# hpcde/spmv-acc

Hardware: AMD Instinct MI355X
Metric: CSR SpMV GFLOP/s (fp64, int32 indices; achieved HBM GB/s in roofline) (higher is better)
Workload: dtype f64

## Files before the change

include/spmv_acc.h:

```cpp
#ifndef SPMV_ACC_C_ABI_H
#define SPMV_ACC_C_ABI_H

#ifdef __cplusplus
extern "C" {
#endif

enum spmv_acc_strategy {
  SPMV_ACC_DEFAULT = 0,
  SPMV_ACC_ADAPTIVE = 1,
  SPMV_ACC_THREAD_ROW = 2,
  SPMV_ACC_WF_ROW = 3,
  SPMV_ACC_BLOCK_ROW_ORDINARY = 4,
  SPMV_ACC_LIGHT = 5,
  SPMV_ACC_VECTOR_ROW = 6,
  SPMV_ACC_LINE_ENHANCE = 7,
  SPMV_ACC_LINE = 8,
  SPMV_ACC_FLAT = 9,
  SPMV_ACC_ADAPTIVE_PLUS = 10
};
int spmv_acc_set_strategy(const char *name);
int spmv_acc_set_strategy_id(int strategy);
int spmv_acc_get_strategy(void);
const char *spmv_acc_strategy_name(int strategy);
int spmv_acc_parse_strategy(const char *name);
// ... 29 lines not shown

int spmv_acc_adaptive_plus_analyze(int m, int min_nnz_per_block, int threads_per_block, int vec_size,
                                   const int *h_rowptr, int *h_break_points, int bp_cap,
                                   int *h_first_block_of_row);
int spmv_acc_adaptive_plus_analyze_device(int m, int min_nnz_per_block, int threads_per_block, int vec_size,
                                          const int *d_rowptr, int *d_break_points, int bp_cap,
                                          int *d_first_block_of_row);
int spmv_acc_adaptive_plus_vec(int m, int nnz);

int spmv_acc_adaptive_branch(int m, int rp_quarter, int rp_half, int rp_three_quarter, int rp_last);

int spmv_acc_partition_rows(int m, int parts, int mode, const int *h_rowptr, int *row_begin);

int spmv_acc_sharded_spmv(void *nccl_comm, int strategy, double alpha, double beta, int m_local, int m_pad, int n, int nnz_local,
                          const int *h_rowptr, const int *d_rowptr, const int *d_colindex, const double *d_value, const double *dx,
                          double *dy_local, double *dy_full);

typedef struct spmv_acc_shard *spmv_acc_shard_t;
int spmv_acc_shard_create(spmv_acc_shard_t *out, void *nccl_comm, int strategy, int m_local, int m_pad, int n, int nnz_local,
                          const int *d_rowptr, const int *d_colindex, const double *d_value, int pipeline);
int spmv_acc_shard_step(spmv_acc_shard_t shard, double alpha, double beta, const double *dx, const double *dy_in_local,
                        double *dy_full);
int spmv_acc_shard_prepare(spmv_acc_shard_t shard, double beta, const double *dx);
int spmv_acc_shard_pipeline(spmv_acc_shard_t shard);
int spmv_acc_shard_destroy(spmv_acc_shard_t shard);
int spmv_acc_rccl_comm_init_all(void **comms, int ndev, const int *devices);
int spmv_acc_rccl_comm_destroy(void *comm);

int spmv_acc_stage_csr(int m, int n, int nnz, const int *h_rowptr, const int *h_colindex, const double *h_value,
                       const double *h_x, const double *h_y, int **d_rowptr, int **d_colindex, double **d_value,
                       double **d_x, double **d_y);
int spmv_acc_free_device(void *p);

int spmv_acc_prepare(int strategy, int m, int n, int nnz, const int *h_rowptr, const int *d_rowptr, const int *d_colindex,
                     const double *d_value, const double *dx, float *ms_out);
int spmv_acc_prepare_beta(int strategy, double beta, int m, int n, int nnz, const int *h_rowptr, const int *d_rowptr,
                          const int *d_colindex, const double *d_value, const double *dx, float *ms_out);

void spmv_acc_set_tune_cache(const char *path);

int spmv_acc_refresh_values(const int *d_rowptr);

double spmv_acc_last_prepare_us(void);

void spmv_acc_release_plans(const int *d_rowptr);
int spmv_acc_cached_plans(void);
int spmv_acc_check_plans(void);
int spmv_acc_query_plan(const int *d_rowptr, int m, int *out);
int spmv_acc_query_plan_beta0(const int *d_rowptr, int m);
int spmv_acc_query_plan_slab_passes(const int *d_rowptr, int m);
int spmv_acc_query_plan_settled(const int *d_rowptr, int m);
int spmv_acc_query_plan_col16(const int *d_rowptr, int m);
int spmv_acc_query_plan_col_bits(const int *d_rowptr, int m);
enum spmv_acc_kernel {
  SPMV_ACC_KERNEL_ROWBLOCK = 0,
  SPMV_ACC_KERNEL_ROWBLOCK_PLUS = 1,
  SPMV_ACC_KERNEL_FLAT_TILE = 2,
  SPMV_ACC_KERNEL_SLAB_PASSES = 3,
  SPMV_ACC_KERNEL_VECTOR_TILE = 4, SPMV_ACC_KERNEL_VECTOR_ROW = 5, SPMV_ACC_KERNEL_WAVE_ROW = 6, SPMV_ACC_KERNEL_LIGHT = 7,
  SPMV_ACC_KERNEL_BLOCK_ROW = 8, SPMV_ACC_KERNEL_COL_SLABS = 9, SPMV_ACC_KERNEL_SCALE_ONLY = 10
};
int spmv_acc_query_plan_last_kernel(const int *d_rowptr, int m);

void spmv_acc_set_stream(void *hip_stream);
void *spmv_acc_get_stream(void);

int spmv_acc_last_error(void);
const char *spmv_acc_last_error_string(void);
void spmv_acc_clear_error(void);
enum spmv_acc_error {
  SPMV_ACC_OK = 0,
  SPMV_ACC_ERR_UNSUPPORTED_TRANS = 1,
  SPMV_ACC_ERR_BAD_ARGUMENT = 2,
  SPMV_ACC_ERR_HIP = 3,
  SPMV_ACC_ERR_TOO_LARGE = 4,
  SPMV_ACC_ERR_UNKNOWN_STRATEGY = 5,
  SPMV_ACC_ERR_NO_DEVICE = 6
};

int spmv_acc_time_spmv(int strategy, int iters, double alpha, double beta, int m, int n, int nnz,
                       const int *h_rowptr, const int *d_rowptr, const int *d_colindex, const double *d_value,
                       const double *dx, double *dy, const double *d_y0, float *ms_out);

int spmv_acc_time_spmv_events(int strategy, int iters, double alpha, double beta, int m, int n, int nnz,
                              const int *h_rowptr, const int *d_rowptr, const int *d_colindex, const double *d_value,
                              const double *dx, double *dy, const double *d_y0, float *ms_out, unsigned event_flags);

int spmv_acc_time_spmv_cold(int strategy, int iters, double alpha, double beta, int m, int n, int nnz,
                            const int *h_rowptr, const int *d_rowptr, const int *d_colindex, const double *d_value,
                            const double *dx, double *dy, const double *d_y0, void *d_flush, long long flush_bytes, float *ms_out);

int spmv_acc_time_spmv_total(int strategy, int iters, double alpha, double beta, int m, int n, int nnz,
                             const int *h_rowptr, const int *d_rowptr, const int *d_colindex, const double *d_value,
                             const double *dx, double *dy, float *total_ms_out);
int spmv_acc_time_spmv_kernels(int strategy, int iters, double alpha, double beta, int m, int n, int nnz,
                               const int *h_rowptr, const int *d_rowptr, const int *d_colindex, const double *d_value,
                               const double *dx, double *dy, const double *d_y0, float *event_ms_out, float *kernel_ms_out, int *launches_out);
int spmv_acc_time_spmv_region(int strategy, int iters, double alpha, double beta, int m, int n, int nnz,
                              const int *h_rowptr, const int *d_rowptr, const int *d_colindex, const double *d_value,
                              const double *dx, double *dy, float *total_ms_out);
double spmv_acc_copy_ceiling_gbs(void *d_dst, const void *d_src, long long bytes, int reps);

int spmv_acc_set_tunable(const char *name, int value);
int spmv_acc_get_tunable(const char *name);
void spmv_acc_reset_tunables(void);

// ... 8 lines not shown
```

spmv_acc_amd/__init__.py:

```python
from __future__ import annotations

import ctypes
import os
from typing import Optional, Sequence

_HERE = os.path.dirname(os.path.abspath(__file__))
LIB_PATH = os.path.join(_HERE, "lib", "libspmv_acc.so")

STRATEGIES = (
    "default", "adaptive", "thread_row", "wf_row", "block_row_ordinary", "light",
    "vector_row", "line_enhance", "line", "flat", "adaptive_plus",
)
HOT_STRATEGIES = ("default", "adaptive", "flat", "line_enhance", "line", "vector_row", "adaptive_plus")

_c_int_p = ctypes.POINTER(ctypes.c_int)
_c_double_p = ctypes.POINTER(ctypes.c_double)

C_ABI_SYMBOLS = (
    "sparse_spmv", "spmv_acc_csr_spmv", "spmv_acc_csr_spmv_strategy", "spmv_acc_set_strategy",
    "spmv_acc_set_strategy_id", "spmv_acc_get_strategy", "spmv_acc_strategy_name", "spmv_acc_parse_strategy",
    "spmv_acc_break_points", "spmv_acc_break_points_len", "spmv_acc_adaptive_plus_analyze",
    "spmv_acc_adaptive_plus_vec", "spmv_acc_adaptive_branch", "spmv_acc_partition_rows", "spmv_acc_stage_csr",
    "spmv_acc_free_device", "spmv_acc_release_plans", "spmv_acc_cached_plans", "spmv_acc_query_plan",
    "spmv_acc_set_stream", "spmv_acc_get_stream", "spmv_acc_last_error", "spmv_acc_last_error_string",
    "spmv_acc_clear_error", "spmv_acc_time_spmv", "spmv_acc_version", "spmv_acc_set_tunable",
    "spmv_acc_get_tunable", "spmv_acc_reset_tunables", "spmv_acc_time_spmv_total", "spmv_acc_copy_ceiling_gbs", "spmv_acc_adaptive_plus_analyze_device", "spmv_acc_prepare",
    "spmv_acc_last_prepare_us", "spmv_acc_sharded_spmv", "spmv_acc_shard_prepare", "spmv_acc_csr_spmv_chunks", "spmv_acc_query_plan_settled", "spmv_acc_query_plan_col16", "spmv_acc_query_plan_col_bits", "spmv_acc_time_spmv_cold", "spmv_acc_csr_spmv_oop", "spmv_acc_check_plans",
    "spmv_acc_query_plan_beta0", "spmv_acc_query_plan_slab_passes", "spmv_acc_shard_create", "spmv_acc_shard_step", "spmv_acc_shard_pipeline",
    "spmv_acc_shard_destroy", "spmv_acc_rccl_comm_init_all", "spmv_acc_rccl_comm_destroy", "spmv_acc_set_tune_cache",
    "spmv_acc_prepare_beta", "spmv_acc_time_spmv_events", "spmv_acc_refresh_values", "spmv_acc_time_spmv_region", "spmv_acc_query_plan_last_kernel", "spmv_acc_time_spmv_kernels",
    "spmv_acc_csr_spmm",
)

_lib = None


class SpmvAccError(RuntimeError):
    pass


def load_library(path: Optional[str] = None) -> ctypes.CDLL:
    global _lib
    if _lib is not None and path is None:
        return _lib
    p = path or LIB_PATH
    if not os.path.exists(p):
        raise SpmvAccError(
            f"{p} not found: the HIP extension is not built. Run `python -c 'import __graft_entry__ as g; g.build()'` "
            "or `make -C spmv_acc_amd/csrc`. There is no CPU fallback."
        )
    try:
        import torch
    except ImportError:
        pass
    lib = ctypes.CDLL(p)
    vp, ci, cd = ctypes.c_void_p, ctypes.c_int, ctypes.c_double
    lib.sparse_spmv.argtypes = [ci, cd, cd, ci, ci, vp, vp, vp, vp, vp]
    lib.sparse_spmv.restype = None
    lib.spmv_acc_csr_spmv.argtypes = [ci, cd, cd, ci, ci, ci, vp, vp, vp, vp, vp, vp]
    lib.spmv_acc_csr_spmv.restype = None
    lib.spmv_acc_csr_spmv_strategy.argtypes = [ci, ci, cd, cd, ci, ci, ci, vp, vp, vp, vp, vp, vp]
    lib.spmv_acc_csr_spmv_strategy.restype = None
    lib.spmv_acc_set_strategy.argtypes = [ctypes.c_char_p]
    lib.spmv_acc_set_strategy_id.argtypes = [ci]
    lib.spmv_acc_strategy_name.argtypes = [ci]
    lib.spmv_acc_strategy_name.restype = ctypes.c_char_p
    lib.spmv_acc_parse_strategy.argtypes = [ctypes.c_char_p]
    lib.spmv_acc_break_points.argtypes = [vp, ci, ci, ci, vp, ci]
    lib.spmv_acc_break_points_len.argtypes = [ci, ci]
    lib.spmv_acc_adaptive_plus_analyze.argtypes = [ci, ci, ci, ci, vp, vp, ci, vp]
    lib.spmv_acc_adaptive_plus_vec.argtypes = [ci, ci]
    lib.spmv_acc_adaptive_plus_analyze_device.argtypes = [ci, ci, ci, ci, vp, vp, ci, vp]
    lib.spmv_acc_adaptive_branch.argtypes = [ci, ci, ci, ci, ci]
    lib.spmv_acc_partition_rows.argtypes = [ci, ci, ci, vp, vp]
    lib.spmv_acc_stage_csr.argtypes = [ci, ci, ci, vp, vp, vp, vp, vp] + [ctypes.POINTER(vp)] * 5
    lib.spmv_acc_free_device.argtypes = [vp]
    lib.spmv_acc_prepare.argtypes = [ci, ci, ci, ci, vp, vp, vp, vp, vp, ctypes.POINTER(ctypes.c_float)]
    lib.spmv_acc_release_plans.argtypes = [vp]
    lib.spmv_acc_release_plans.restype = None
    lib.spmv_acc_query_plan.argtypes = [vp, ci, vp]
    lib.spmv_acc_set_stream.argtypes = [vp]
    lib.spmv_acc_set_stream.restype = None
    lib.spmv_acc_get_stream.restype = vp
    lib.spmv_acc_last_error_string.restype = ctypes.c_char_p
    lib.spmv_acc_clear_error.restype = None
    lib.spmv_acc_time_spmv.argtypes = [ci, ci, cd, cd, ci, ci, ci, vp, vp, vp, vp, vp, vp, vp, vp]
    lib.spmv_acc_time_spmv_events.argtypes = [ci, ci, cd, cd, ci, ci, ci, vp, vp, vp, vp, vp, vp, vp, vp, ctypes.c_uint]
    lib.spmv_acc_time_spmv_cold.argtypes = [ci, ci, cd, cd, ci, ci, ci, vp, vp, vp, vp, vp, vp, vp, vp, ctypes.c_longlong, vp]
    lib.spmv_acc_version.restype = ctypes.c_char_p
    lib.spmv_acc_set_tunable.argtypes = [ctypes.c_char_p, ci]
    lib.spmv_acc_get_tunable.argtypes = [ctypes.c_char_p]
    lib.spmv_acc_reset_tunables.restype = None
    lib.spmv_acc_time_spmv_total.argtypes = [ci, ci, cd, cd, ci, ci, ci, vp, vp, vp, vp, vp, vp, vp]
    lib.spmv_acc_time_spmv_kernels.argtypes = [ci, ci, cd, cd, ci, ci, ci, vp, vp, vp, vp, vp, vp, vp, vp, vp, vp]
    lib.spmv_acc_time_spmv_region.argtypes = [ci, ci, cd, cd, ci, ci, ci, vp, vp, vp, vp, vp, vp, vp]
    lib.spmv_acc_copy_ceiling_gbs.argtypes = [vp, vp, ctypes.c_longlong, ci]
    lib.spmv_acc_copy_ceiling_gbs.restype = cd
    lib.spmv_acc_last_prepare_us.restype = cd
    lib.spmv_acc_sharded_spmv.argtypes = [vp, ci, cd, cd, ci, ci, ci, ci, vp, vp, vp, vp, vp, vp, vp]
    lib.spmv_acc_csr_spmv_oop.argtypes = [ci, ci, cd, cd, ci, ci, ci, vp, vp, vp, vp, vp, vp, vp]
    lib.spmv_acc_csr_spmv_oop.restype = None
    lib.spmv_acc_query_plan_beta0.argtypes = [vp, ci]
    lib.spmv_acc_query_plan_slab_passes.argtypes = [vp, ci]
    lib.spmv_acc_query_plan_settled.argtypes = [vp, ci]
    lib.spmv_acc_query_plan_col16.argtypes = [vp, ci]
    lib.spmv_acc_query_plan_col_bits.argtypes = [vp, ci]
    lib.spmv_acc_query_plan_last_kernel.argtypes = [vp, ci]
    lib.spmv_acc_shard_create.argtypes = [ctypes.POINTER(vp), vp, ci, ci, ci, ci, ci, vp, vp, vp, ci]
    lib.spmv_acc_shard_step.argtypes = [vp, cd, cd, vp, vp, vp]
    lib.spmv_acc_shard_pipeline.argtypes = [vp]
    lib.spmv_acc_shard_destroy.argtypes = [vp]
    lib.spmv_acc_rccl_comm_init_all.argtypes = [ctypes.POINTER(vp), ci, vp]
    lib.spmv_acc_rccl_comm_destroy.argtypes = [vp]
    lib.spmv_acc_set_tune_cache.argtypes = [ctypes.c_char_p]
    lib.spmv_acc_set_tune_cache.restype = None
    lib.spmv_acc_refresh_values.argtypes = [vp]
    lib.spmv_acc_prepare_beta.argtypes = [ci, cd, ci, ci, ci, vp, vp, vp, vp, vp, ctypes.POINTER(ctypes.c_float)]
    lib.spmv_acc_shard_prepare.argtypes = [vp, cd, vp]
    lib.spmv_acc_csr_spmv_chunks.argtypes = [ci, cd, cd, ci, ci, vp, vp, vp, vp, vp, vp, vp, vp, vp, vp]
    ll = ctypes.c_longlong
    lib.spmv_acc_csr_spmm.argtypes = [ci, ci, cd, cd, ci, ci, ci, vp, vp, vp, vp, vp, ll, vp, ll]
    lib.spmv_acc_csr_spmm.restype = ci
    if path is None:
        _lib = lib
    return lib


def strategy_id(name_or_id) -> int:
    if isinstance(name_or_id, int):
        return name_or_id
    s = load_library().spmv_acc_parse_strategy(str(name_or_id).encode())
    if s < 0:
        raise SpmvAccError(f"unknown KERNEL_STRATEGY {name_or_id!r}")
    return s


def _check(lib) -> None:
    code = lib.spmv_acc_last_error()
    if code not in (0, 1):
        msg = lib.spmv_acc_last_error_string().decode()
        lib.spmv_acc_clear_error()
        raise SpmvAccError(f"spmv_acc error {code}: {msg}")


def _ptr(t) -> int:
    if t is None:
        return 0
    if isinstance(t, int):
        return t
    if hasattr(t, "data_ptr"):
        return t.data_ptr()
    return t.ctypes.data


def _require_cuda(*tensors) -> None:
    for t in tensors:
        if t is not None and hasattr(t, "is_cuda") and not t.is_cuda:
            raise SpmvAccError("device pointers required: tensor is not on the GPU (no CPU fallback)")

# ... 241 lines not shown
    args = (strategy_id(strategy), iters, alpha, beta, m, n, nnz, None, _ptr(rowptr), _ptr(colindex), _ptr(value), _ptr(x), _ptr(y),
            ctypes.addressof(out))
    fn = lib.spmv_acc_time_spmv_region

    def run() -> float:
        rc = fn(*args)
        if rc != 0:
            raise SpmvAccError(f"time_spmv_region failed ({rc}): {lib.spmv_acc_last_error_string().decode()}")
        return float(out.value)

    return run


def copy_ceiling_gbs(dst, src, reps: int = 5) -> float:
    lib = load_library()
    _require_cuda(dst, src)
    nbytes = (src.numel() * src.element_size()) // 16 * 16
    return float(lib.spmv_acc_copy_ceiling_gbs(_ptr(dst), _ptr(src), nbytes, reps))


def release_plans(rowptr=None) -> None:
    load_library().spmv_acc_release_plans(_ptr(rowptr))


def set_tune_cache(path: Optional[str]) -> None:
    load_library().spmv_acc_set_tune_cache(path.encode() if path else None)


def refresh_values(rowptr) -> int:
    return int(load_library().spmv_acc_refresh_values(_ptr(rowptr)))


def check_plans() -> int:
    return int(load_library().spmv_acc_check_plans())


KERNEL_NAMES = {0: "rowblock", 1: "rowblock_plus", 2: "flat_tile", 3: "slab_passes", 4: "vector_tile", 5: "vector_row", 6: "wave_row", 7: "light",
                8: "block_row", 9: "col_slabs", 10: "scale_only"}


def query_plan(rowptr, m: int):
    import numpy as np

    out = np.zeros(9, dtype=np.int32)
    found = load_library().spmv_acc_query_plan(_ptr(rowptr), m, _ptr(out))
    if not found:
        return None
    keys = ("nnz", "adaptive_branch", "vec", "flat_tiles", "plus_blocks", "aligned16", "stream_policy", "flat_fixup", "adaptive_family")
    info = dict(zip(keys, (int(v) for v in out)))
    info["slab_passes"] = max(0, int(load_library().spmv_acc_query_plan_slab_passes(_ptr(rowptr), m)))
    info["settled"] = int(load_library().spmv_acc_query_plan_settled(_ptr(rowptr), m)) == 1
    info["col16"] = int(load_library().spmv_acc_query_plan_col16(_ptr(rowptr), m))
    info["col_bits"] = int(load_library().spmv_acc_query_plan_col_bits(_ptr(rowptr), m))
    info["last_kernel"] = KERNEL_NAMES.get(int(load_library().spmv_acc_query_plan_last_kernel(_ptr(rowptr), m)), "none")
    return info


def set_strategy(name: str) -> None:
    lib = load_library()
    if lib.spmv_acc_set_strategy(name.encode()) != 0:
        lib.spmv_acc_clear_error()
        raise SpmvAccError(f"unknown KERNEL_STRATEGY {name!r}")


def get_strategy() -> str:
    lib = load_library()
    return lib.spmv_acc_strategy_name(lib.spmv_acc_get_strategy()).decode()
```

spmv_acc_amd/csrc/c_api.cpp:

```cpp
#include <hip/hip_runtime.h>

#include <dlfcn.h>

#include <algorithm>
#include <cstdlib>
#include <cstring>
#include <mutex>
#include <vector>

#include "../../include/spmv_acc.h"
#include "engine.hpp"

#include <string>
#include <cstdint>

using namespace spmv_acc;

namespace {
struct PinTable {
  std::mutex mu;
  struct Range { uintptr_t lo, hi; int refs; };
  std::vector<Range> ranges;
  static constexpr uintptr_t kPage = 4096;
  bool pin(void *p, size_t bytes) {
// ... 306 lines not shown
  ok = ok && stage_one(st, h_value, static_cast<size_t>(nnz), d_value);
  ok = ok && stage_one(st, h_x, static_cast<size_t>(n), d_x);
  ok = ok && stage_one(st, h_y, static_cast<size_t>(m), d_y);
  ok = ok && hipStreamSynchronize(st.copy) == hipSuccess;
  if (!ok) {
    const hipError_t e = hipGetLastError();
    set_error(kErrHip, std::string("spmv_acc_stage_csr: ") + hipGetErrorString(e));
    return kErrHip;
  }
  return kOk;
}

int spmv_acc_free_device(void *p) {
  if (!p) return kOk;
  return hipFree(p) == hipSuccess ? kOk : kErrHip;
}

void spmv_acc_release_plans(const int *d_rowptr) { release_plans(d_rowptr); }
int spmv_acc_cached_plans(void) { return cached_plan_count(); }
int spmv_acc_check_plans(void) { return check_plans(); }
int spmv_acc_query_plan(const int *d_rowptr, int m, int *out) {
  PlanInfo info;
  if (!out || !query_plan(d_rowptr, m, &info)) return 0;
  out[0] = info.nnz;
  out[1] = info.adaptive_branch;
  out[2] = info.vec;
  out[3] = info.flat_tiles;
  out[4] = info.plus_blocks;
  out[5] = info.aligned16;
  out[6] = info.stream_policy;
  out[7] = info.flat_fixup;
  out[8] = info.adaptive_family;
  return 1;
}
int spmv_acc_query_plan_beta0(const int *d_rowptr, int m) {
  PlanInfo info;
  return query_plan(d_rowptr, m, &info) ? info.adaptive_family_beta0 : -2;
}
int spmv_acc_query_plan_slab_passes(const int *d_rowptr, int m) {
  PlanInfo info;
  return query_plan(d_rowptr, m, &info) ? info.slab_passes : -2;
}
int spmv_acc_query_plan_last_kernel(const int *d_rowptr, int m) {
  PlanInfo info;
  return query_plan(d_rowptr, m, &info) ? info.last_kernel : -2;
}
int spmv_acc_query_plan_col16(const int *d_rowptr, int m) {
  PlanInfo info;
  return query_plan(d_rowptr, m, &info) ? info.col16 : -2;
}
int spmv_acc_query_plan_col_bits(const int *d_rowptr, int m) {
  PlanInfo info;
  return query_plan(d_rowptr, m, &info) ? info.col_bits : -2;
}
int spmv_acc_query_plan_settled(const int *d_rowptr, int m) {
  PlanInfo info;
  return query_plan(d_rowptr, m, &info) ? info.settled : -2;
}

void spmv_acc_set_stream(void *hip_stream) { set_stream(static_cast<hipStream_t>(hip_stream)); }
void *spmv_acc_get_stream(void) { return static_cast<void *>(get_stream()); }

int spmv_acc_set_tunable(const char *name, int value) { return name ? set_tunable(name, value) : -1; }
int spmv_acc_get_tunable(const char *name) { return name ? get_tunable(name) : -1; }
void spmv_acc_reset_tunables(void) { reset_tunables(); }

double spmv_acc_last_prepare_us(void) { return last_prepare_us(); }

int spmv_acc_last_error(void) { return last_error(); }
const char *spmv_acc_last_error_string(void) { return last_error_string(); }
void spmv_acc_clear_error(void) { clear_error(); }

void spmv_acc_set_tune_cache(const char *path) { set_tune_cache(path); }
int spmv_acc_refresh_values(const int *d_rowptr) { return refresh_values(d_rowptr); }

int spmv_acc_prepare(int strategy, int m, int n, int nnz, const int *h_rowptr, const int *d_rowptr, const int *d_colindex,
                     const double *d_value, const double *dx, float *ms_out) {
  return spmv_acc_prepare_beta(strategy, 1.0, m, n, nnz, h_rowptr, d_rowptr, d_colindex, d_value, dx, ms_out);
}

int spmv_acc_prepare_beta(int strategy, double beta, int m, int n, int nnz, const int *h_rowptr, const int *d_rowptr,
                          const int *d_colindex, const double *d_value, const double *dx, float *ms_out) {
  if (m <= 0) return kOk;
  hipStream_t st = get_stream();
  double *scratch = nullptr;
  if (hipMalloc(reinterpret_cast<void **>(&scratch), sizeof(double) * static_cast<size_t>(m)) != hipSuccess) {
    set_error(kErrHip, "spmv_acc_prepare: hipMalloc failed");
    return kErrHip;
  }
  hipEvent_t e0 = nullptr, e1 = nullptr;
  const bool timed = ms_out && hipEventCreate(&e0) == hipSuccess && hipEventCreate(&e1) == hipSuccess;
  clear_error();
  if (timed) (void)hipEventRecord(e0, st);
  (void)hipMemsetAsync(scratch, 0, sizeof(double) * static_cast<size_t>(m), st);
  {
    UnboundedTuningScope unbounded;
    for (int round = 0; round < 6; ++round) {
      run_spmv(strategy, 0, 1.0, beta != 0.0 ? 1.0 : 0.0, m, n, nnz, h_rowptr, d_rowptr, d_colindex, d_value, dx, scratch);
      if (last_error() != kOk || last_prepare_us() <= 0.0) break;
    }
  }
  if (timed) (void)hipEventRecord(e1, st);
  int rc = hipStreamSynchronize(st) == hipSuccess ? kOk : kErrHip;
  if (timed && rc == kOk && hipEventElapsedTime(ms_out, e0, e1) != hipSuccess) rc = kErrHip;
  if (e0) (void)hipEventDestroy(e0);
  if (e1) (void)hipEventDestroy(e1);
// ... 256 lines not shown
```

spmv_acc_amd/csrc/dispatch.cpp:

```cpp
#include "engine_internal.hpp"

namespace spmv_acc {
using namespace detail;

namespace detail {

constexpr int kFlatMaxTileRows = 16384;

thread_local int t_strict_name = -1;

bool run_flat(hipStream_t st, Plan &p, double alpha, double beta, const double *x, double *y) {
  if (!ensure_flat(p, st)) return false;
  const bool strict = t_strict_name == kFlat;
  if (p.flat.max_tile_rows > kFlatMaxTileRows && tun(kT_rowblock_guard) && !strict) {
    return run_rowblock(st, p, nullptr, alpha, beta, x, y, false, 0);
  }
  p.A.cold = nullptr;
  p.flat.col16 = nullptr;
  if (!autotune_policy(p, kFamFlat, st, [&](int pol, double *ys) { launch_flat_with(st, p, pol, 1.0, trial_beta(), x, ys); })) return false;
  if (!autotune_flat_mode(p, st, x)) return false;
  if (!autotune_flat_geometry(p, st, x)) return false;
  if (!autotune_hint(p, kFamFlat, st, [&](double *ys) { launch_flat_with(st, p, policy_for(p, kFamFlat), 1.0, trial_beta(), x, ys); })) return false;
  const Col16 *c16 = nullptr;
  if (p.flat.stride == kThreads * kNnzPerThread && !flat_segment_sum() &&
      !autotune_col16(p, kFamFlat, st, [&](const Col16 *c, double *ys) {
        p.flat.col16 = c;
        launch_flat_with(st, p, policy_for(p, kFamFlat), 1.0, trial_beta(), x, ys);
      }, &c16))
    return false;
  p.flat.col16 = c16;
  const int rb_mode = tun(kT_flat_rowblock);
  const bool tile_pinned = tun(kT_flat_finish) >= 0 || tun(kT_flat_npt) >= 0 || tun(kT_flat_early) >= 0;
  if (rb_mode != 0 && (rb_mode > 0 || !tile_pinned) && !flat_segment_sum() && tun(kT_col16) <= 0 &&
      !t_coarse_tuning && !strict) {
    if (rb_mode > 0) {
      int vec = 1, rpb = kThreads;
      pick_rowblock_shape(p.A.m, p.A.count(), rowblock_target_for(p), &vec, &rpb);
      if (t_capturing ? (p.rowblock_ok == 1 && p.rowblock_rpb == rpb) : (probe_rowblock(p, rpb, st) && p.rowblock_ok == 1))
        return run_rowblock(st, p, nullptr, alpha, beta, x, y, false, 0);
    } else if (p.flat_rowblock_choice < 0 && !t_capturing && !by_rule()) {
      int vec = 1, rpb = kThreads;
      pick_rowblock_shape(p.A.m, p.A.count(), rowblock_target_for(p), &vec, &rpb);
      if (!probe_rowblock(p, rpb, st)) return false;
      p.flat_rowblock_choice = 0;
      if (p.rowblock_ok == 1) {
        TimingPhase ph(st, p.A.m);
        float ms2[2] = {0.f, 0.f};
        bool ok = ph.ok && run_rowblock(st, p, nullptr, 1.0, trial_beta(), x, ph.y, false);
        ok = ok && ph.in_turns(2, [&](int c) {
          if (c == 0) launch_flat_with(st, p, policy_for(p, kFamFlat), 1.0, trial_beta(), x, ph.y);
          else (void)run_rowblock(st, p, nullptr, 1.0, trial_beta(), x, ph.y, false);
        }, ranking_rounds(), ms2);
        if (!ok) return false;
        const float ms_flat = ms2[0], ms_rb = ms2[1];
        p.flat_rowblock_choice = ms_rb < 0.985f * ms_flat ? 1 : 0;
        tune_log("m %d nnz %d flat on balanced rows: tile kernel %.2f us, row blocks %.2f us -> %s", p.A.m, p.A.nnz, ms_flat * 1e3f, ms_rb * 1e3f,
                 p.flat_rowblock_choice ? "row blocks" : "tile kernel");
      }
    }
    if (rb_mode < 0 && p.flat_rowblock_choice == 1) return run_rowblock(st, p, nullptr, alpha, beta, x, y, false, 0);
  }
  launch_flat_with(st, p, policy_for(p, kFamFlat), alpha, beta, x, y);
  p.last_kernel = kKernelFlatTile;
  p.last_c16 = c16 && p.flat.stride == kThreads * kNnzPerThread && p.A.cold == nullptr ? c16->rec_ints : 0;
  p.last_col_bits = p.last_c16 > 0 ? c16->bits : 0;
  return true;
}

bool validate_plan(Plan &p, hipStream_t st) {
  if (p.invalid < 0) {
    if (!plan_work_allowed("validating the matrix")) return false;
    ++t_plan_work;
    int *d_flags = nullptr;
    int h = -1;
    if (!hip_ok(hipMalloc(reinterpret_cast<void **>(&d_flags), sizeof(int)), "hipMalloc validate")) return false;
    if (hip_ok(hipMemsetAsync(d_flags, 0, sizeof(int), st), "memset validate")) {
      launch_validate_csr(st, p.A, d_flags);
      if (!hip_ok(hipMemcpyAsync(&h, d_flags, sizeof(int), hipMemcpyDeviceToHost, st), "read validate") ||
          !hip_ok(hipStreamSynchronize(st), "sync validate"))
        h = -1;
    }
    (void)hipFree(d_flags);
    if (h < 0) return false;
    p.invalid = h;
  }
  if (p.invalid != 0) {
    std::string what = "matrix failed validation:";
    if (p.invalid & 1) what += " rowptr decreases or is negative;";
    if (p.invalid & 2) what += " rowptr[m] != nnz;";
    if (p.invalid & 4) what += " column index outside [0, n);";
    set_error(kErrBadArgument, what);
    return false;
  }
  return true;
}

bool launch_full_guard(Plan &p, hipStream_t st) {
  if (!p.A.guard || !p.A.stale) return true;
  if (!p.have_rp_digest) {
    if (!plan_work_allowed("the full row-pointer digest (guard_full)")) return false;
    ++t_plan_work;
    const size_t words = static_cast<size_t>(Plan::kDigestSlots) * kDigestMaxParts + 1;
    if (!p.d_digest_acc && !hip_ok(hipMalloc(reinterpret_cast<void **>(&p.d_digest_acc), sizeof(unsigned long long) * words), "hipMalloc digest"))
      return false;
    unsigned long long *out = p.d_digest_acc + words - 1;
    launch_rowptr_digest(st, p.A.rp, p.A.m, p.d_digest_acc);
    launch_rowptr_verdict(st, p.d_digest_acc, p.A.m, 0, nullptr, out);
    unsigned long long h = 0;
    if (!hip_ok(hipMemcpyAsync(&h, out, sizeof(h), hipMemcpyDeviceToHost, st), "read digest") || !hip_ok(hipStreamSynchronize(st), "sync digest"))
      return false;
    p.rp_digest = h;
    p.have_rp_digest = true;
  }
  unsigned long long *part = p.d_digest_acc + static_cast<size_t>(p.digest_turn++ % Plan::kDigestSlots) * kDigestMaxParts;
  launch_rowptr_digest(st, p.A.rp, p.A.m, part);
  launch_rowptr_verdict(st, part, p.A.m, p.rp_digest, p.A.stale, nullptr);
  return true;
}
// ... 96 lines not shown
      }))
    return false;
  if (tun(kT_rowblock_target) <= 0 && p.rb_target == 0 && p.stream_policy[kFamRowblock][t_beta_class] >= 0 && !t_capturing && !t_coarse_tuning &&
      !t_no_policy_timing && !by_rule()) {
    int v2[2], r2[2];
    const int cand[2] = {kRowblockTargetRule, kRowblockTargetAlt};
    for (int c = 0; c < 2; ++c) shape_for(cand[c], &v2[c], &r2[c]);
    if (v2[0] == v2[1] && r2[0] == r2[1]) {
      p.rb_target = cand[0];
    } else {
      TimingPhase ph(st, p.A.m);
      bool ok = ph.ok;
      bool skip[2] = {false, false};
      float ms[2] = {1e30f, 1e30f};
      const int pol = policy_for(p, kFamRowblock);
      for (int c = 0; ok && c < 2; ++c) {
        vec = v2[c];
        rpb = r2[c];
        if (tun(kT_rowblock_guard)) {
          ok = probe_rowblock(p, rpb, st);
          skip[c] = ok && p.rowblock_ok == 0;
        }
      }
      for (int round = 0; ok && round < ranking_rounds(); ++round) {
        for (int c = 0; ok && c < 2; ++c) {
          if (skip[c]) continue;
          vec = v2[c];
          rpb = r2[c];
          ok = setup();
          float t = 0.f;
          ok = ok && ph.time([&] {
            const int zz = next_reverse(p) ? 64 : 0;
            launch_rowblock_stream(st, p.A, vec, rpb, base_flags | (pol << 4) | zz, 1.0, trial_beta(), x, ph.y, dg, cache_ends);
          }, &t);
          if (ok && t < ms[c]) ms[c] = t;
        }
      }
      if (!ok) return false;
      p.rb_target = (!skip[1] && (skip[0] || ms[1] < 0.985f * ms[0])) ? cand[1] : cand[0];
      tune_log("m %d nnz %d row blocks: %d products per block %.2f us, %d products %.2f us -> %d", p.A.m, p.A.nnz, cand[0], ms[0] * 1e3f, cand[1], ms[1] * 1e3f,
               p.rb_target);
    }
    shape_for(rowblock_target_for(p), &vec, &rpb);
    if (tun(kT_rowblock_guard) && !probe_rowblock(p, rpb, st)) return false;
    if (!setup()) return false;
  }
  if (!autotune_hint(p, kFamRowblock, st, [&](double *ys) {
        const int zz = next_reverse(p) ? 64 : 0;
        launch_rowblock_stream(st, p.A, vec, rpb, base_flags | (policy_for(p, kFamRowblock) << 4) | zz, 1.0, trial_beta(), x, ys, dg, cache_ends);
      }))
    return false;
  const Col16 *c16 = nullptr;
  if (!autotune_col16(p, kFamRowblock, st, [&](const Col16 *c, double *ys) {
        const int zz = next_reverse(p) ? 64 : 0;
        launch_rowblock_stream(st, p.A, vec, rpb, base_flags | (policy_for(p, kFamRowblock) << 4) | zz, 1.0, trial_beta(), x, ys, dg, cache_ends, c);
      }, &c16))
    return false;
  const int zz = next_reverse(p) ? 64 : 0;
  launch_rowblock_stream(st, p.A, vec, rpb, base_flags | (policy_for(p, kFamRowblock) << 4) | zz, alpha, beta, x, y, dg, cache_ends, c16);
  p.last_kernel = kKernelRowblock;
  p.last_c16 = c16 && p.A.cold == nullptr ? c16->rec_ints : 0;
  p.last_col_bits = p.last_c16 > 0 ? c16->bits : 0;
  return true;
}

bool run_plus_prepare(Plan &p, const int *h_rowptr, hipStream_t st, const double *x) {
  auto launch = [&](int pol, double *ys) {
    launch_plus(st, p.A, p.d_pbp, p.d_pfbr, p.d_pblk, p.plus_blocks, p.plus_has_long, tun(kT_xcd_chunk), pol,
                p.d_ppartial, 1.0, trial_beta(), x, ys, next_reverse(p));
  };
  const int forced = tun(kT_plus_min_nnz);
  if (forced > 0) {
    return ensure_plus(p, h_rowptr, st, forced > 0 ? forced : kPlusMinNnz) && autotune_policy(p, kFamPlus, st, launch);
  }
  if (tun(kT_deterministic)) {
    int vec = 1, rpb = kThreads;
    pick_rowblock_shape(p.A.m, p.A.count(), rowblock_target_for(p), &vec, &rpb);
    return probe_rowblock(p, rpb, st) && ensure_plus(p, h_rowptr, st, p.rowblock_ok == 0 ? kPlusMinNnz : 1536);
  }
  if (p.plus_tuned_min > 0) return ensure_plus(p, h_rowptr, st, p.plus_tuned_min) && autotune_policy(p, kFamPlus, st, launch);
  if (t_capturing) return (p.plus_blocks >= 0 || ensure_plus(p, h_rowptr, st, 1536)) && autotune_policy(p, kFamPlus, st, launch);
  if (t_coarse_tuning || defer_tuning())
    return ensure_plus(p, h_rowptr, st, p.rowblock_ok == 0 ? kPlusMinNnz : 1536) && autotune_policy(p, kFamPlus, st, launch);
  if (!ensure_plus(p, h_rowptr, st, 1536) || !autotune_policy(p, kFamPlus, st, launch)) return false;
  TimingPhase ph(st, p.A.m);
  bool ok = ph.ok;
  const int candidates[3] = {1536, 1920, kPlusMinNnz};
  float best = 1e30f;
  int best_min = kPlusMinNnz;
  for (int c = 0; ok && c < 3; ++c) {
    ok = ensure_plus(p, h_rowptr, st, candidates[c]);
    if (!ok) break;
    float ms = 0.f;
    ok = ph.time([&] { launch(policy_for(p, kFamPlus), ph.y); }, &ms);
    if (ok) tune_log("m %d nnz %d beta class %d row-block-plus: MIN_NNZ_PER_BLOCK %d -> %.2f us (kept for both classes)", p.A.m, p.A.nnz, t_beta_class, candidates[c], ms * 1e3f);
    if (ok && ms < best) {
      best = ms;
      best_min = candidates[c];
    }
  }
  if (!ok) return false;
  p.plus_tuned_min = best_min;
  return ensure_plus(p, h_rowptr, st, best_min);
}

thread_local bool t_in_slab = false;
bool ensure_segments(Plan &p, int S, hipStream_t st);
thread_local bool t_in_segment_timing = false;
static bool decide_whole_pass_hint(hipStream_t st, Plan &p, const double *x) {
  const int s = p.seg_slabs - 1;
  if (p.seg_rest_below <= 0 || p.seg_entries[s] == 0 || tun(kT_gather_hint) == 0 || static_cast<long long>(p.A.n) * 8 >= (1LL << 32)) return true;
  if (p.hint_state < 0 && !t_capturing && !ensure_hint(p, st)) return false;
  if (p.hint_state != 1 || !p.d_cold) return true;
  if (p.seg_whole_hint >= 0 || t_capturing || by_rule()) return true;
  TimingPhase ph(st, p.A.m, false);
// ... 292 lines not shown
      return 0;
    }
  }
  *p.h_values_changed = 0;
  launch_value_samples(st, p.A.v, p.A.ci, p.A.nnz0, p.A.count() - 1, p.value_samples, p.d_value_samples, p.h_values_changed);
  if (!hip_ok(hipStreamSynchronize(st), "compare the value samples")) return 0;
  if (*p.h_values_changed & 2) {
    tune_log("m %d nnz %d: the caller's column indices changed under the slab-major copy: the copy is dropped, the run-list passes serve", p.A.m, p.A.nnz);
    p.free_slabs();
    p.slab_copy_choice = 0;
    return 0;
  }
  if (*p.h_values_changed) {
    launch_slab_scatter(st, p.A, p.slab_width, p.slab_count, p.d_slab_rp, p.d_slab_off, p.d_slab_ci, p.d_slab_v, true);
    launch_value_samples(st, p.A.v, p.A.ci, p.A.nnz0, p.A.count() - 1, p.value_samples, p.d_value_samples, nullptr);
    ++p.values_refreshed;
    tune_log("m %d nnz %d: the caller's values changed under the slab-major copy: refreshed (%u so far)", p.A.m, p.A.nnz, p.values_refreshed);
  }
  return S;
}

namespace {
thread_local bool t_early_clock = false;
thread_local std::chrono::steady_clock::time_point t_early_began;

void run_spmv_call(int strategy, int trans, double alpha, double beta, int m, int n, int nnz, const int *h_rowptr,
                   const int *d_rowptr, const int *d_colindex, const double *d_value, const double *dx, double *dy,
                   const double *dy_in);
}

void run_spmv(int strategy, int trans, double alpha, double beta, int m, int n, int nnz, const int *h_rowptr,
              const int *d_rowptr, const int *d_colindex, const double *d_value, const double *dx, double *dy,
              const double *dy_in) {
  apply_env_tunables();
  bool early = rule_until_settled() && !t_in_slab && !t_rule_twin && t_unbounded_tuning == 0 && m > 0 && d_rowptr && dy && strategy >= 0 &&
               strategy < kStrategyCount && strategy < 32 && tun(kT_col_slabs) < 2;
  const bool capturing = early && stream_capturing(t_stream);
  if (early) early = !plan_settled_for(d_rowptr, d_colindex, d_value, m, n, strategy, beta != 0.0 ? 1 : 0);
  if (!early) {
    run_spmv_call(strategy, trans, alpha, beta, m, n, nnz, h_rowptr, d_rowptr, d_colindex, d_value, dx, dy, dy_in);
    return;
  }
  if (capturing && !rule_twin_exists(d_rowptr, d_colindex, d_value, m, n)) {
    run_spmv_call(strategy, trans, alpha, beta, m, n, nnz, h_rowptr, d_rowptr, d_colindex, d_value, dx, dy, dy_in);
    return;
  }
  if (capturing) {
    ScopedSet twin(t_rule_twin, true);
    run_spmv_call(strategy, trans, alpha, beta, m, n, nnz, h_rowptr, d_rowptr, d_colindex, d_value, dx, dy, dy_in);
    return;
  }
  const auto began = std::chrono::steady_clock::now();
  const int err_before = last_error_code_only();
  int served_kernel = -1, served_c16 = 0, served_col_bits = 0;
  {
    ScopedSet twin(t_rule_twin, true);
    run_spmv_call(strategy, trans, alpha, beta, m, n, nnz, h_rowptr, d_rowptr, d_colindex, d_value, dx, dy, dy_in);
    if (const std::shared_ptr<Plan> tp = t_last_plan.lock()) {
      served_kernel = tp->last_kernel;
      served_c16 = tp->last_c16;
      served_col_bits = tp->last_col_bits;
    }
  }
  if (last_error_code_only() != err_before && last_error_code_only() != kOk && last_error_code_only() != kErrUnsupportedTrans) return;
  const double twin_prepare_us = t_last_prepare_us;
  double *scratch = tune_scratch(static_cast<size_t>(m));
  if (!scratch) {
    clear_error();
    return;
  }
  (void)hipMemsetAsync(scratch, 0, sizeof(double) * static_cast<size_t>(m), t_stream);
  t_early_began = began;
  {
    ScopedSet early_clock(t_early_clock, true);
    run_spmv_call(strategy, 0, alpha, beta, m, n, nnz, h_rowptr, d_rowptr, d_colindex, d_value, dx, scratch, nullptr);
  }
  t_last_prepare_us += twin_prepare_us;
  if (const std::shared_ptr<Plan> p = t_last_plan.lock()) {
    std::lock_guard<std::mutex> plan_lock(p->mu);
    const int cls = beta != 0.0 ? 1 : 0;
    if (!((p->settled_for[cls] >> strategy) & 1u)) {
      p->last_kernel = served_kernel;
      p->last_c16 = served_c16;
      p->last_col_bits = served_col_bits;
    }
  }
  if (plan_settled_for(d_rowptr, d_colindex, d_value, m, n, strategy, beta != 0.0 ? 1 : 0)) drop_rule_twin(d_rowptr, d_colindex, d_value, m, n);
}

namespace {
void run_spmv_call(int strategy, int trans, double alpha, double beta, int m, int n, int nnz, const int *h_rowptr,
                   const int *d_rowptr, const int *d_colindex, const double *d_value, const double *dx, double *dy,
                   const double *dy_in) {
  const int strategy_named = strategy;
  if (trans != 0) {
    set_error(kErrUnsupportedTrans, "only operation_none is supported; computed y = alpha*A*x + beta*y");
  }
  apply_env_tunables();
  if (m <= 0) return;
  if (m > INT_MAX - (1 << 16)) {
    set_error(kErrTooLarge, "row count does not leave room for block arithmetic in int32; shard the matrix");
    return;
  }
  if (!d_rowptr || !dy || (n > 0 && !dx)) {
    set_error(kErrBadArgument, "null rowptr / x / y");
    return;
  }
  if (dy_in == dy) dy_in = nullptr;
  if (dy_in && beta != 0.0) {
    const uintptr_t a = reinterpret_cast<uintptr_t>(dy_in), b = reinterpret_cast<uintptr_t>(dy), bytes = sizeof(double) * static_cast<uintptr_t>(m);
    if (a < b + bytes && b < a + bytes) {
      set_error(kErrBadArgument, "y_in and y_out overlap without being the same vector");
      return;
    }
  }
  hipStream_t st = t_stream;
  note_stream_use();
  t_capturing = stream_capturing(st);
  if (strategy < 0 || strategy >= kStrategyCount) {
    set_error(kErrUnknownStrategy, "unknown strategy id");
    return;
  }
  const std::shared_ptr<Plan> p = get_plan(m, n, nnz, h_rowptr, d_rowptr, d_colindex, d_value);
  if (!p) return;
  t_last_plan = p;
  struct ScratchScope {
    bool outer;
    ~ScratchScope() {
      if (outer) release_tune_scratch();
    }
  } scratch_scope{!t_in_slab};
  std::lock_guard<std::mutex> plan_lock(p->mu);
  t_beta_class = beta != 0.0 ? 1 : 0;
  struct BudgetScope {
    Plan &p;
    bool outer;
    int strategy, cls;
    ~BudgetScope() {
      if (!outer) return;
      if (t_first_trial_ms > 0.f) p.trial_ms = t_first_trial_ms;
      p.tuning_open = t_tuning_deferred;
      if (!t_tuning_deferred && strategy >= 0 && strategy < 32) p.settled_for[cls] |= 1u << strategy;
      t_budget_spmvs = 0.0;
      t_budget_ms = -1.0;
    }
  } budget_scope{*p, !t_in_slab, strategy_named, beta != 0.0 ? 1 : 0};
  if (!t_in_slab) {
    t_call_began = (t_early_clock && p->calls == 0) ? t_early_began : std::chrono::steady_clock::now();
    t_tuning_deferred = false;
    t_first_trial_ms = 0.f;
    const int allowance = p->calls == 0 ? tun(kT_first_call_budget) : tun(kT_later_call_budget);
    t_budget_spmvs = (t_unbounded_tuning > 0 || t_capturing || allowance <= 0) ? 0.0 : static_cast<double>(allowance);
    t_budget_ms = (t_budget_spmvs > 0.0 && p->trial_ms > 0.0) ? t_budget_spmvs * p->trial_ms : -1.0;
  }
  struct PrepareClock {
    unsigned work0;
    std::chrono::steady_clock::time_point t0;
    ~PrepareClock() {
      t_last_prepare_us =
          t_plan_work != work0 ? std::chrono::duration<double, std::micro>(std::chrono::steady_clock::now() - t0).count() : 0.0;
    }
  } prepare_clock{t_plan_work, std::chrono::steady_clock::now()};
  if (p->calls++ == 0) ++t_plan_work;
  (void)hipGetLastError();
  if (p->launched && p->last_stream != st && !t_capturing && !t_in_slab) {
    if (!p->order_event && hipEventCreateWithFlags(&p->order_event, hipEventDisableTiming) != hipSuccess) p->order_event = nullptr;
    if (p->order_event && hipEventRecord(p->order_event, p->last_stream) == hipSuccess) (void)hipStreamWaitEvent(st, p->order_event, 0);
    (void)hipGetLastError();
  }
  p->last_stream = st;
  p->launched = true;
  if (t_capturing) p->captured = true;
  struct YinScope {
    CsrDev &A;
    ~YinScope() { A.yin = nullptr; }
  } yin_scope{p->A};
  p->A.yin = beta != 0.0 ? dy_in : nullptr;
  p->last_c16 = 0;
  p->last_col_bits = 0;

  if (p->A.count() == 0) {
    launch_scale_y(st, m, beta, dy, p->A.yin);
    p->last_kernel = kKernelScaleOnly;
    return;
  }
  ScopedSet strict_scope(t_strict_name, t_in_slab ? t_strict_name : (tun(kT_strict_strategy) ? strategy : -1));
  if (!d_colindex || !d_value) {
    set_error(kErrBadArgument, "null colindex / value with nnz > 0");
    return;
  }
  if (tun(kT_validate) && !validate_plan(*p, st)) return;
  if (tun(kT_guard_full) && !t_in_slab && !launch_full_guard(*p, st)) return;

  int copy_slabs = (tun(kT_col_slabs) >= 2 && !t_in_slab) ? (tun(kT_col_slabs) > 64 ? 64 : tun(kT_col_slabs)) : 0;
  if (!copy_slabs && tun(kT_col_slabs) < 0 && !t_in_slab) copy_slabs = slab_copy_auto(*p, strategy, st, n, dx);
  if (copy_slabs) {
    if (!run_col_slabs(*p, copy_slabs, strategy, st, alpha, beta, m, n, dx, dy)) return;
    t_last_plan = p;
    t_beta_class = beta != 0.0 ? 1 : 0;
    if (t_plan_work != prepare_clock.work0 && p->tune_key) tune_store(*p);
    return;
  }

  if (tun(kT_slab_segments) >= 1 && !t_in_slab && !(t_strict_name == kLineEnhance || t_strict_name == kLine || t_strict_name == kFlat)) {
    const int S = tun(kT_slab_segments) == 1 ? seg_auto_slabs(n) : tun(kT_slab_segments) > 16 ? 16 : tun(kT_slab_segments);
    if (last_error_code_only() == kOk && !t_capturing && !ensure_segments(*p, S, st)) {
      (void)hipGetLastError();
      tune_log("m %d nnz %d: slab_segments: the run lists could not be built (%s), ordinary path", m, p->A.nnz, last_error_string());
      clear_error();
      p->free_segments();
      p->seg_state = 0;
    }
    if (p->seg_state == 1) {
      run_segments(st, *p, alpha, beta, dx, dy);
      if (t_plan_work != prepare_clock.work0 && p->tune_key) tune_store(*p);
      return;
    }
  }


  const long long avg = static_cast<long long>(p->A.count()) / m;
  auto resident_blocks = [&]() {
    int cus = 0;
    if (hipDeviceGetAttribute(&cus, hipDeviceAttributeMultiprocessorCount, p->device) != hipSuccess || cus <= 0) cus = 256;
    (void)hipGetLastError();
    return cus * 8;
  };
  if (strategy == kLight) {
    if (!p->d_light_counter) {
      if (!plan_work_allowed("LIGHT's row counter")) return;
      ++t_plan_work;
      if (!hip_ok(hipMalloc(reinterpret_cast<void **>(&p->d_light_counter), 2 * sizeof(unsigned)), "hipMalloc light counter") ||
// ... 103 lines not shown
```

spmv_acc_amd/csrc/engine.hpp:

```cpp
#pragma once

#include <hip/hip_runtime_api.h>

#include <string>
#include <vector>

#include "kernels.hpp"

namespace spmv_acc {

enum Strategy {
  kDefault = 0,
  kAdaptive = 1,
  kThreadRow = 2,
  kWfRow = 3,
  kBlockRowOrdinary = 4,
  kLight = 5,
  kVectorRow = 6,
  kLineEnhance = 7,
  kLine = 8,
  kFlat = 9,
  kAdaptivePlus = 10,
  kStrategyCount = 11
};
// ... 33 lines not shown
int active_strategy();
int set_active_strategy(int s);

struct FlatSegmentSumScope {
  FlatSegmentSumScope();
  ~FlatSegmentSumScope();
  bool prev;
};

struct RowptrSamples {
  int q1 = 0;
  int half = 0;
  int q3 = 0;
  int last = 0;
};

int adaptive_branch(int m, const RowptrSamples &s);

int plus_analyze_host(int m, int min_nnz_per_block, int threads_per_block, int vec_size, const int *host_row_ptr,
                      std::vector<int> &break_points, std::vector<int> &first_block_of_row);
int plus_analyze_device(int m, int min_nnz_per_block, int threads_per_block, int vec_size, const int *d_rowptr,
                        int *d_break_points, int bp_cap, int *d_first_block_of_row);
int plus_pick_vec(int m, int nnz);
int plus_pick_vec_tuned(int m, int nnz, int min_nnz);

void run_spmv(int strategy, int trans, double alpha, double beta, int m, int n, int nnz, const int *h_rowptr,
              const int *d_rowptr, const int *d_colindex, const double *d_value, const double *dx, double *dy,
              const double *dy_in = nullptr);

int run_spmm(int layout, int k, double alpha, double beta, int m, int n, int nnz, const int *h_rowptr, const int *d_rowptr, const int *d_colindex,
             const double *d_value, const double *dX, long long ldx, double *dY, long long ldy);
void release_plans(const int *d_rowptr, int m_only = -1);
void kernel_clock_begin();
void kernel_clock_set(bool on);
void kernel_clock_release();
size_t kernel_clock_used();
bool kernel_clock_failed();
hipEvent_t kernel_clock_event(size_t i);

struct PlanInfo {
  int nnz = 0;
  int adaptive_branch = 0;
  int vec = 0;
  int flat_tiles = 0;
  int plus_blocks = 0;
  int aligned16 = 0;
  int stream_policy = -1;
  int flat_fixup = -1;
  int adaptive_family = -1;
  int adaptive_family_beta0 = -1;
  int slab_passes = 0;
  int last_kernel = -1;
  int col16 = -1;
  int col_bits = -1;
  int settled = 0;
};
bool query_plan(const int *d_rowptr, int m, PlanInfo *out);
unsigned plan_work_count();
int cached_plan_count();
void set_tune_cache(const char *path);
int refresh_values(const int *d_rowptr);
int check_plans();

}
```

spmv_acc_amd/csrc/engine_internal.hpp:

```cpp
#pragma once

#include "engine.hpp"

#include <hip/hip_runtime.h>

#include <algorithm>
#include <atomic>
#include <chrono>
#include <climits>
#include <cstdarg>
#include <cstdio>
#include <cstdint>
#include <cstdlib>
#include <cstring>
#include <deque>
#include <map>
#include <memory>
#include <mutex>
#include <string>
#include <tuple>

#include <vector>

#include "kernels.hpp"
// ... 16 lines not shown
  return capturing;
}
template <typename T> struct ScopedSet {
  T &ref;
  const T old;
  ScopedSet(T &r, T value) : ref(r), old(r) { ref = value; }
  ~ScopedSet() { ref = old; }
  ScopedSet(const ScopedSet &) = delete;
  ScopedSet &operator=(const ScopedSet &) = delete;
};
struct Tunable {
  const char *name;
  int def;
  int val;
};
enum TunableId {
  kT_xcd_chunk, kT_rowblock_vec, kT_rowblock_target, kT_stream_plain, 
  kT_rowblock_guard, kT_adaptive_timed, kT_adaptive_split, 
  kT_plus_min_nnz, kT_plus_host_analysis, kT_flat_finish, kT_flat_npt, kT_validate, kT_rowlen, kT_flat_early, kT_vector_tile, kT_col16, kT_vector_width, kT_zigzag, kT_cache_ends_mb, kT_flat_reduce, kT_gather_hint, kT_hint_budget_kb, kT_deterministic, kT_col_slabs, kT_flat_rowblock, kT_guard_full, kT_slab_segments, kT_first_call_budget, kT_later_call_budget, kT_slab_whole_below, kT_strict_strategy, kT_slab_kb, kT_hint_min_x_mb, kT_max_grid_blocks, kT_flat_small_nnz_k, kTunableCount
};
extern Tunable g_tunables[];
void apply_env_tunables();
extern thread_local bool t_rule_twin;
inline int tun(TunableId id) {
  if (id == kT_deterministic) return (t_rule_twin || g_tunables[id].val > 0) ? 1 : 0;
  return g_tunables[id].val;
}
inline bool rule_until_settled() { return g_tunables[kT_deterministic].val == 0; }
bool quarters_uneven(const RowptrSamples &s);
int classic_vec(long long avg);
int tile_vec(long long avg);

int guard_acquire(int device, const int **d_guard, int **h_flag);
void guard_release(int device, int slot, bool launched, hipStream_t last_stream);
enum Family { kFamRowblock = 0, kFamPlus = 1, kFamFlat = 2, kFamVector = 3, kFamilyCount = 4 };
enum LastKernel { kKernelRowblock = 0, kKernelPlus = 1, kKernelFlatTile = 2, kKernelSlabPasses = 3, kKernelVectorTile = 4, kKernelVectorRow = 5,
                  kKernelWaveRow = 6, kKernelLight = 7, kKernelBlockRow = 8, kKernelColSlabs = 9, kKernelScaleOnly = 10 };
extern thread_local int t_strict_name;

typedef std::tuple<int, const void *, const void *, const void *, int, int, int> PlanKey;

struct Plan {
  int device = 0;
  PlanKey key;
  hipStream_t last_stream = nullptr;
  hipEvent_t order_event = nullptr;
  bool launched = false;
  unsigned long long last_use = 0;
  std::mutex mu;
  unsigned long long calls = 0;
  unsigned launches = 0;
  double trial_ms = 0.0;
  int last_c16 = -1;
  int last_col_bits = -1;
  int last_kernel = -1;
  bool tuning_open = true;
  bool captured = false;
  unsigned settled_for[2] = {0, 0};
  CsrDev A;
  int guard_slot = -1;
  bool have_samples = false;
  RowptrSamples samples;
  int stream_policy[kFamilyCount][2] = {{-1, -1}, {-1, -1}, {-1, -1}, {-1, -1}};
  int invalid = -1;
  int rowblock_ok = -1;
  int rowblock_rpb = 0;
  int rb_target = 0;
  int max_block_nnz = 0;
  bool rowblock_uneven = false;
  int adaptive_family[2] = {-1, -1};
  float adaptive_ms[2][3] = {{1e30f, 1e30f, 1e30f}, {1e30f, 1e30f, 1e30f}};
  bool adaptive_provisional[2] = {false, false};
  bool adaptive_skipped[2][3] = {{false, false, false}, {false, false, false}};
  RowDigest digest;
  int flat_tiles = -1;
  FlatPlan flat;
  Col16 col16;
  int c16_use[kFamilyCount] = {-1, -1, -1, -1};
  int flat_npt_choice = 0;
  bool flat_geometry_tuned = false;
  int flat_rowblock_choice = -1;
  bool flat_early_choice = false;
  int flat_mode_choice[2] = {-1, -1};
  unsigned long long tune_key = 0;
  unsigned *d_light_counter = nullptr;
  static constexpr int kDigestSlots = 8;
  bool have_rp_digest = false;
  unsigned long long rp_digest = 0;
  unsigned long long *d_digest_acc = nullptr;
  unsigned digest_turn = 0;
  int slab_count = 0;
  int slab_width = 0;
  int slab_copy_choice = -1;
  unsigned long long *d_value_samples = nullptr;
  int *h_values_changed = nullptr;
  int value_samples = 0;
  unsigned values_refreshed = 0;
  long long *d_slab_off = nullptr;
  std::vector<int *> slab_rowid, slab_crp;
  std::vector<int> slab_rows;
  double *d_slab_ys = nullptr;
  int *d_slab_rp = nullptr;
  int *d_slab_ci = nullptr;
  double *d_slab_v = nullptr;
  std::vector<long long> slab_off;
  int plus_blocks = -1;
  int plus_vec = 0;
  int plus_min = 0;
  int plus_tuned_min = 0;
  bool plus_has_long = false;
  int hint_state = -1;
  unsigned char *d_cold = nullptr;
  double hint_hot_share = 0.0;
  int hint_use[kFamilyCount] = {-1, -1, -1, -1};
  int *d_pbp = nullptr;
  int *d_pfbr = nullptr;
  double *d_ppartial = nullptr;
  void *d_pblk = nullptr;
  int spmm_state = -1;
  SpmmLong spmm;
  void free_spmm() {
    for (void *q : {static_cast<void *>(spmm.rows), static_cast<void *>(spmm.first), static_cast<void *>(spmm.piece), static_cast<void *>(spmm.partial)})
      if (q) (void)hipFree(q);
    spmm = SpmmLong();
    spmm_state = -1;
  }

  ~Plan() {
    free_device();
    guard_release(device, guard_slot, launched, last_stream);
  }
  bool is_stale() const { return A.stale && __atomic_load_n(A.stale, __ATOMIC_RELAXED) != 0; }
  void free_col16() {
    if (col16.d16) (void)hipFree(col16.d16);
    if (col16.d8) (void)hipFree(col16.d8);
    if (col16.rec) (void)hipFree(col16.rec);
    if (col16.ovf) (void)hipFree(col16.ovf);
    if (col16.ci_guard) (void)hipFree(col16.ci_guard);
    col16 = Col16();
  }
  void free_digest() {
    if (digest.lens) (void)hipFree(digest.lens);
    if (digest.base) (void)hipFree(digest.base);
    digest = RowDigest();
  }
  void free_slabs();
  int seg_state = -1, seg_slabs = 0;
  int seg_choice = -1;
  bool seg_early_tried = false;
  std::vector<int *> seg_row, seg_begin, seg_vptr, seg_blk, seg_cut;
  std::vector<int> seg_entries, seg_blocks, seg_pieces;
  double *d_seg_ys = nullptr;
  int seg_rest_below = 0;
  int seg_whole_hint = -1;
  void free_segments() {
    seg_rest_below = 0;
    seg_whole_hint = -1;
    for (auto *list : {&seg_row, &seg_begin, &seg_vptr, &seg_blk, &seg_cut}) {
      for (int *q : *list)
        if (q) (void)hipFree(q);
      list->clear();
    }
    seg_entries.clear();
    seg_blocks.clear();
    seg_pieces.clear();
    if (d_seg_ys) (void)hipFree(d_seg_ys);
    d_seg_ys = nullptr;
    seg_state = -1;
    seg_slabs = 0;
  }
  void free_device() {
    if (order_event) (void)hipEventDestroy(order_event);
    order_event = nullptr;
    free_slabs();
    free_segments();
    if (d_light_counter) (void)hipFree(d_light_counter);
    d_light_counter = nullptr;
    if (d_digest_acc) (void)hipFree(d_digest_acc);
    d_digest_acc = nullptr;
    if (d_cold) (void)hipFree(d_cold);
    d_cold = nullptr;
    hint_state = -1;
    free_flat();
    free_digest();
    free_col16();
    free_spmm();
    if (d_pbp) (void)hipFree(d_pbp);
    if (d_pfbr) (void)hipFree(d_pfbr);
    if (d_ppartial) (void)hipFree(d_ppartial);
    if (d_pblk) (void)hipFree(d_pblk);
    d_pblk = nullptr;
    d_ppartial = nullptr;
    d_pbp = d_pfbr = nullptr;
  }
  static void free_flat_plan(FlatPlan &F) {
    if (F.bp) (void)hipFree(F.bp);
    if (F.head) (void)hipFree(F.head);
    if (F.tail) (void)hipFree(F.tail);
    if (F.tail_row) (void)hipFree(F.tail_row);
    if (F.tail_end) (void)hipFree(F.tail_end);
    if (F.digest) (void)hipFree(F.digest);
    F = FlatPlan();
  }
  void free_flat() {
    free_flat_plan(flat);
    flat_tiles = -1;
  }
};

struct TuneRecord {
  int v[26];
  bool operator==(const TuneRecord &o) const { return std::memcmp(v, o.v, sizeof(v)) == 0; }
};
constexpr int kTuneFields = 26;
bool tune_cache_enabled();
void tune_adopt(Plan &p);
void tune_store(const Plan &p);
extern std::map<PlanKey, std::shared_ptr<Plan>> g_plans;
extern thread_local std::weak_ptr<Plan> t_last_plan;
extern thread_local bool t_capturing;
bool plan_work_allowed(const char *what);
bool plan_settled_for(const int *rp, const int *ci, const double *v, int m, int n, int strategy, int cls);
void drop_rule_twin(const int *rp, const int *ci, const double *v, int m, int n);
bool rule_twin_exists(const int *rp, const int *ci, const double *v, int m, int n);
const int *host_view(const int *h);
bool fetch_samples(Plan &p, const int *h_rowptr);
std::shared_ptr<Plan> get_plan(int m, int n, int nnz, const int *h_rowptr, const int *rp, const int *ci, const double *v);
bool report_stale_last_plan();
void drain_deferred_locked();

extern thread_local bool t_flat_segment_sum;
inline bool flat_segment_sum() { return (t_flat_segment_sum || tun(kT_flat_reduce) == 1) && tun(kT_col16) <= 0; }
extern thread_local int t_beta_class;
inline double trial_beta() { return t_beta_class ? 1.0 : 0.0; }
extern thread_local bool t_coarse_tuning;
extern thread_local bool t_no_policy_timing;
extern thread_local bool t_in_slab;
inline bool next_reverse(Plan &p) { return tun(kT_zigzag) && (p.launches++ & 1u); }
constexpr int kRowblockTargetRule = 1800, kRowblockTargetAlt = 1500;
inline int rowblock_target_for(const Plan &p) { return tun(kT_rowblock_target) > 0 ? tun(kT_rowblock_target) : (p.rb_target > 0 ? p.rb_target : kRowblockTargetRule); }
constexpr int kFlatSmallNnz = 24 << 20;
inline long long flat_small_nnz() { return static_cast<long long>(tun(kT_flat_small_nnz_k)) << 10; }
int policy_for(const Plan &p, int fam);
bool tune_log_enabled();
void tune_log(const char *fmt, ...);
double *tune_scratch(size_t len);
void release_tune_scratch();
bool build_flat_plan(const CsrDev &A, int stride, hipStream_t stream, FlatPlan &F);
int flat_stride_for(const Plan &p);
bool ensure_flat(Plan &p, hipStream_t stream);
int analyze_on_device(hipStream_t st, const int *d_rowptr, int m, int min_nnz, int threads, int vec, int **d_bp, int **d_fbr);
bool ensure_plus(Plan &p, const int *h_rowptr, hipStream_t stream, int min_nnz);
bool ensure_col16(Plan &p, hipStream_t st);
bool ensure_hint(Plan &p, hipStream_t st);
bool ensure_slabs(Plan &p, int S, hipStream_t st);
bool ensure_segments(Plan &p, int S_cols, hipStream_t st);
void launch_flat_plan(hipStream_t st, const CsrDev &A, FlatPlan &F, int policy, double alpha, double beta, const double *x, double *y, bool reverse);
void launch_flat_with(hipStream_t st, Plan &p, int policy, double alpha, double beta, const double *x, double *y);
bool autotune_flat_mode(Plan &p, hipStream_t st, const double *x);
bool autotune_flat_geometry(Plan &p, hipStream_t st, const double *x);

extern thread_local std::chrono::steady_clock::time_point t_call_began;
extern thread_local double t_budget_spmvs;
extern thread_local double t_budget_ms;
extern thread_local bool t_tuning_deferred;
extern thread_local float t_first_trial_ms;
extern thread_local int t_unbounded_tuning;
inline bool defer_tuning() {
  if (t_budget_spmvs <= 0.0 || t_budget_ms < 0.0) return false;
  const double spent = std::chrono::duration<double, std::milli>(std::chrono::steady_clock::now() - t_call_began).count();
  if (spent < 0.5 * t_budget_ms) return false;
  t_tuning_deferred = true;
  return true;
}
inline bool by_rule() { return tun(kT_deterministic) != 0 || defer_tuning(); }
inline double budget_spent_fraction() {
  if (t_budget_spmvs <= 0.0 || t_budget_ms <= 0.0) return 0.0;
  return std::chrono::duration<double, std::milli>(std::chrono::steady_clock::now() - t_call_began).count() / t_budget_ms;
}

struct TuneTimer {
  static constexpr int kMaxTimed = 5;
  hipEvent_t e0 = nullptr, e1 = nullptr;
  hipEvent_t per[2 * kMaxTimed] = {};
  void *reset_ptr = nullptr;
  size_t reset_bytes = 0;
  bool ok = false;
  TuneTimer() {
    ok = hip_ok(hipEventCreate(&e0), "event") && hip_ok(hipEventCreate(&e1), "event");
    for (auto &e : per) ok = ok && hip_ok(hipEventCreate(&e), "event");
  }
  ~TuneTimer() {
    if (e0) (void)hipEventDestroy(e0);
    if (e1) (void)hipEventDestroy(e1);
    for (auto &e : per)
      if (e) (void)hipEventDestroy(e);
  }
  template <typename F> bool time(hipStream_t st, F &&fn, float *ms_per_launch, int at_least = 1) {
    if (!ok) return false;
    float first = 0.f;
    (void)hipEventRecord(e0, st);
    fn();
    (void)hipEventRecord(e1, st);
    if (!hip_ok(hipEventSynchronize(e1), "sync tune") || !hip_ok(hipEventElapsedTime(&first, e0, e1), "elapsed tune")) return false;
    if (t_first_trial_ms <= 0.f) t_first_trial_ms = first;
    if (t_budget_spmvs > 0.0 && t_budget_ms < 0.0) t_budget_ms = t_budget_spmvs * static_cast<double>(first);
// ... 88 lines not shown
      if (p.stream_policy[f][cls] >= 0) return true;
  }
  TimingPhase ph(st, p.A.m);
  bool ok = ph.ok;
  const int candidates[3] = {kStreamPolicyNt, kStreamPolicyDefault, kStreamPolicyValueDefault};
  float best = 1e30f;
  int best_policy = kStreamPolicyNt;
  for (int c = 0; ok && c < 3; ++c) {
    float ms = 0.f;
    ok = ph.time([&] { launch(candidates[c], ph.y); }, &ms);
    if (ok) tune_log("m %d nnz %d family %d beta class %d: stream policy %d -> %.2f us", p.A.m, p.A.nnz, fam, cls, candidates[c], ms * 1e3f);
    if (ok && ms < best) {
      best = ms;
      best_policy = candidates[c];
    }
  }
  if (ok) tune_log("m %d nnz %d family %d: keeps stream policy %d", p.A.m, p.A.nnz, fam, best_policy);
  if (ok) p.stream_policy[fam][cls] = best_policy;
  return ok;
}

template <class Launch> bool autotune_hint(Plan &p, int fam, hipStream_t st, Launch launch) {
  p.A.cold = nullptr;
  const int mode = tun(kT_gather_hint);
  if (mode == 0) return true;
  if ((p.hint_state < 0 || (mode < 0 && p.hint_state == 1 && p.hint_use[fam] < 0)) && stream_capturing(st)) return true;
  if (!ensure_hint(p, st)) return false;
  if (p.hint_state != 1) return true;
  if (mode > 0 || tun(kT_deterministic)) {
    p.A.cold = p.d_cold;
    return true;
  }
  if (p.hint_use[fam] < 0 && defer_tuning()) return true;
  if (p.hint_use[fam] < 0) {
    TimingPhase ph(st, p.A.m);
    bool ok = ph.ok;
    float ms[2] = {0.f, 0.f};
    for (int h = 0; ok && h < 2; ++h) {
      p.A.cold = h ? p.d_cold : nullptr;
      ok = ph.time([&] { launch(ph.y); }, &ms[h]);
    }
    p.A.cold = nullptr;
    if (!ok) return false;
    p.hint_use[fam] = ms[1] < 0.98f * ms[0] ? 1 : 0;
    tune_log("m %d nnz %d family %d beta class %d gather hints: plain %.2f us, hinted %.2f us -> %s (kept for both classes)", p.A.m, p.A.nnz, fam,
             t_beta_class, ms[0] * 1e3f, ms[1] * 1e3f, p.hint_use[fam] ? "hinted" : "plain");
  }
  p.A.cold = p.hint_use[fam] == 1 ? p.d_cold : nullptr;
  return true;
}

template <class Launch> bool autotune_col16(Plan &p, int fam, hipStream_t st, Launch launch, const Col16 **out) {
  *out = nullptr;
  const int mode = tun(kT_col16);
  if (mode == 0 || p.A.cold != nullptr || p.col16.state == 0) return true;
  if (mode < 0 && (tun(kT_deterministic) || p.c16_use[fam] == 0)) return true;
  const bool undecided = p.col16.state < 0 || (mode < 0 && p.c16_use[fam] < 0);
  if (undecided) {
    if (t_capturing || (mode < 0 && (t_coarse_tuning || t_no_policy_timing || defer_tuning())) || stream_capturing(st)) return true;
  }
  if (!ensure_col16(p, st)) return false;
  if (p.col16.state != 1) return true;
  if (mode < 0 && p.c16_use[fam] < 0) {
    TimingPhase ph(st, p.A.m);
    float ms[2] = {0.f, 0.f};
    if (!ph.ok || !ph.in_turns(2, [&](int c) { launch(c ? &p.col16 : nullptr, ph.y); }, ranking_rounds(), ms)) return false;
    p.c16_use[fam] = ms[1] < 0.985f * ms[0] ? 1 : 0;
    tune_log("m %d nnz %d family %d beta class %d 16-bit columns (%d ints per chunk record, %lld escapes, %lld in overflow): colindex %.2f us, encoding %.2f us -> %s",
             p.A.m, p.A.nnz, fam, t_beta_class, p.col16.rec_ints, p.col16.escapes, p.col16.overflow, ms[0] * 1e3f, ms[1] * 1e3f,
             p.c16_use[fam] ? "encoding" : "colindex");
  }
  if (mode > 0 || p.c16_use[fam] == 1) *out = &p.col16;
  return true;
}

bool validate_plan(Plan &p, hipStream_t st);
bool launch_full_guard(Plan &p, hipStream_t st);
bool probe_rowblock(Plan &p, int rpb, hipStream_t st);
bool ensure_digest(Plan &p, int rpb, hipStream_t st);
bool run_flat(hipStream_t st, Plan &p, double alpha, double beta, const double *x, double *y);
bool run_rowblock(hipStream_t st, Plan &p, const int *h_rowptr, double alpha, double beta, const double *x, double *y,
                  bool allow_uneven_switch = false, int lanes_per_row = 0);
bool run_plus(hipStream_t st, Plan &p, const int *h_rowptr, double alpha, double beta, const double *x, double *y);
void run_segments(hipStream_t st, Plan &p, double alpha, double beta, const double *x, double *y);
int seg_auto_slabs(int n);

}
}
```

spmv_acc_amd/csrc/k_col16.hip:

```cpp
#include <climits>

#include <rocprim/device/device_scan.hpp>

#include "device_utils.hpp"
#include "kernels.hpp"

namespace spmv_acc {
namespace {

using namespace dev;

constexpr int kChunk = kCol16Chunk;

template <int BITS> struct CodeWidth;
template <> struct CodeWidth<16> {
  typedef unsigned short T;
  static constexpr int half = 32767;
};
template <> struct CodeWidth<8> {
  typedef unsigned char T;
  static constexpr int half = 127;
};

template <int BITS>
// ... 19 lines not shown
    if (esc > 0) atomicAdd(stats, static_cast<unsigned long long>(esc));
    if (esc > 12) atomicAdd(stats + 1, 1ull);
    if (esc > 28) atomicAdd(stats + 2, 1ull);
    if (esc > 60) atomicAdd(stats + 3, 1ull);
  }
}

__device__ __forceinline__ void chunk_stats(const int *__restrict__ ci, int nnz, int chunk0, int nchunks, int c, int *__restrict__ base,
                                            int *__restrict__ esc_count, unsigned long long *stats) {
  const int lane = threadIdx.x & (kWave - 1);
  const long long j0 = (static_cast<long long>(chunk0) + c) * kChunk + 4 * lane;
  int col[4];
#pragma unroll
  for (int e = 0; e < 4; ++e) col[e] = (j0 + e < nnz) ? ci[j0 + e] : INT_MAX;
  int lo0 = col[0] < col[1] ? col[0] : col[1], hi0 = col[0] < col[1] ? col[1] : col[0];
  int lo1 = col[2] < col[3] ? col[2] : col[3], hi1 = col[2] < col[3] ? col[3] : col[2];
  const int smallest = lo0 < lo1 ? lo0 : lo1;
  int second = lo0 < lo1 ? (hi0 < lo1 ? hi0 : lo1) : (hi1 < lo0 ? hi1 : lo0);
  const int mine = second != INT_MAX ? second : smallest;
  int rank = 0;
  for (int l = 0; l < kWave; ++l) {
    const int other = __shfl(mine, l, kWave);
    rank += (other < mine || (other == mine && l < lane)) ? 1 : 0;
  }
  const int valid = __popcll(__ballot(mine != INT_MAX));
  const int want = valid > 0 ? (valid - 1) / 2 : 0;
  const unsigned long long holder = __ballot(rank == want);
  const int src = holder ? __ffsll(static_cast<long long>(holder)) - 1 : 0;
  const int median = __shfl(mine, src, kWave);
  chunk_base<16>(col, median, valid == 0, lane, c, base, esc_count, stats);
  chunk_base<8>(col, median, valid == 0, lane, c, base + nchunks + 1, esc_count + nchunks + 1, stats + 4);
}

__global__ __launch_bounds__(kThreads) void col16_base_kernel(const int *__restrict__ ci, int nnz, int chunk0, int nchunks,
                                                              int *__restrict__ base, int *__restrict__ esc_count,
                                                              unsigned long long *__restrict__ stats) {
  __shared__ unsigned long long tally[8];
  if (threadIdx.x < 8) tally[threadIdx.x] = 0;
  __syncthreads();
  const long long c_ll = static_cast<long long>(blockIdx.x) * (kThreads / kWave) + threadIdx.x / kWave;
  if (c_ll < nchunks) chunk_stats(ci, nnz, chunk0, nchunks, static_cast<int>(c_ll), base, esc_count, tally);
  __syncthreads();
  if (threadIdx.x < 8 && tally[threadIdx.x] != 0) atomicAdd(stats + threadIdx.x, tally[threadIdx.x]);
}

__global__ __launch_bounds__(kThreads) void col16_overflow_kernel(int *__restrict__ cnt, int nchunks, int E) {
  const long long c = static_cast<long long>(blockIdx.x) * kThreads + threadIdx.x;
  if (c < nchunks) {
    const int over = cnt[c] - E;
    cnt[c] = over > 0 ? over : 0;
  }
}

template <int BITS>
__global__ __launch_bounds__(kThreads) void col16_encode_kernel(const int *__restrict__ ci, int nnz, int chunk0, int nchunks,
                                                                const int *__restrict__ base, const int *__restrict__ ovf_start,
                                                                int R, typename CodeWidth<BITS>::T *__restrict__ codes,
                                                                int *__restrict__ rec, int *__restrict__ ovf) {
  typedef typename CodeWidth<BITS>::T Code;
  constexpr int ESC = 2 * CodeWidth<BITS>::half + 1;
  const int lane = threadIdx.x & (kWave - 1);
  const long long c_ll = static_cast<long long>(blockIdx.x) * (kThreads / kWave) + threadIdx.x / kWave;
  if (c_ll >= nchunks) return;
  const int c = static_cast<int>(c_ll);
  const long long j0 = (static_cast<long long>(chunk0) + c) * kChunk + 4 * lane;
  const int bs = base[c];
  const int E = R - 4;
  int col[4];
  bool is_esc[4];
  int mine = 0;
#pragma unroll
  for (int e = 0; e < 4; ++e) {
    col[e] = (j0 + e < nnz) ? ci[j0 + e] : bs;
    const long long d = static_cast<long long>(col[e]) - bs;
    is_esc[e] = d < 0 || d >= ESC;
    mine += is_esc[e] ? 1 : 0;
  }
  int incl = mine;
#pragma unroll
  for (int o = 1; o < kWave; o <<= 1) {
    const int up = __shfl_up(incl, o, kWave);
    if (lane >= o) incl += up;
  }
  const int total = __shfl(incl, kWave - 1, kWave);
  int pos = incl - mine;
  int *r = rec + static_cast<size_t>(c) * R;
  const int o0 = ovf_start[c];
  Code out[4];
#pragma unroll
  for (int e = 0; e < 4; ++e) {
    out[e] = static_cast<Code>(ESC);
    if (is_esc[e]) {
      if (pos < E) r[4 + pos] = col[e];
      else ovf[o0 + pos - E] = col[e];
      ++pos;
    } else {
      out[e] = static_cast<Code>(col[e] - bs);
    }
  }
  Code *dst = codes + static_cast<size_t>(c) * kChunk + 4 * lane;
#pragma unroll
  for (int e = 0; e < 4; ++e) dst[e] = out[e];
  if (lane == 0) {
    r[0] = bs;
    r[1] = total;
    r[2] = o0;
  }
}

__global__ __launch_bounds__(kWave) void col16_guard_kernel(const int *__restrict__ ci, int lo, int span, int *__restrict__ out) {
  out[threadIdx.x] = ci[lo + static_cast<int>(static_cast<long long>(threadIdx.x) * span / (kWave - 1))];
}

}

size_t col16_scan_bytes(int nchunks) {
  size_t bytes = 0;
  (void)rocprim::exclusive_scan(nullptr, bytes, static_cast<int *>(nullptr), static_cast<int *>(nullptr), 0,
                                static_cast<size_t>(nchunks) + 1, rocprim::plus<int>());
  return bytes;
}

void launch_col16_base(hipStream_t stream, const int *ci, int nnz, int chunk0, int nchunks, int *base, int *esc_count,
                       unsigned long long *stats) {
  if (nchunks <= 0) return;
  const int waves_per_block = kThreads / kWave;
  SPMV_ACC_LAUNCH(col16_base_kernel, dim3((nchunks + waves_per_block - 1) / waves_per_block), dim3(kThreads), 0, stream, ci, nnz,
                     chunk0, nchunks, base, esc_count, stats);
}

void launch_col16_overflow(hipStream_t stream, int *cnt, int nchunks, int E) {
  if (nchunks <= 0) return;
  SPMV_ACC_LAUNCH(col16_overflow_kernel, dim3((nchunks + kThreads - 1) / kThreads), dim3(kThreads), 0, stream, cnt, nchunks, E);
}

bool launch_col16_scan(hipStream_t stream, int nchunks, const int *esc_count, int *esc_start, void *tmp, size_t tmp_bytes) {
  return rocprim::exclusive_scan(tmp, tmp_bytes, esc_count, esc_start, 0, static_cast<size_t>(nchunks) + 1, rocprim::plus<int>(),
                                 stream) == hipSuccess;
}

void launch_col16_encode(hipStream_t stream, const int *ci, int nnz, int chunk0, int nchunks, const int *base, const int *ovf_start,
                         int R, int bits, void *codes, int *rec, int *ovf) {
  if (nchunks <= 0) return;
  const int waves_per_block = kThreads / kWave;
  const dim3 grid((nchunks + waves_per_block - 1) / waves_per_block);
  if (bits == 8)
    SPMV_ACC_LAUNCH(col16_encode_kernel<8>, grid, dim3(kThreads), 0, stream, ci, nnz, chunk0, nchunks, base, ovf_start, R,
                       static_cast<unsigned char *>(codes), rec, ovf);
  else
    SPMV_ACC_LAUNCH(col16_encode_kernel<16>, grid, dim3(kThreads), 0, stream, ci, nnz, chunk0, nchunks, base, ovf_start, R,
                       static_cast<unsigned short *>(codes), rec, ovf);
}

void launch_col16_guard(hipStream_t stream, const int *ci, int lo, int span, int *out) {
  SPMV_ACC_LAUNCH(col16_guard_kernel, dim3(1), dim3(kWave), 0, stream, ci, lo, span, out);
}

}
```

spmv_acc_amd/csrc/k_flat.hip:

```cpp
#include "device_utils.hpp"
#include "kernels.hpp"
#include "tile_stage.hpp"

namespace spmv_acc {
namespace {

using namespace dev;

__global__ __launch_bounds__(256) void break_points_kernel(const int *__restrict__ rp, int m, int nnz, int stride, int tile0,
                                                           int *__restrict__ bp, int bp_len) {
  const int j = blockIdx.x * 256 + threadIdx.x;
  if (j >= bp_len) return;
  const long long target = (static_cast<long long>(j) + tile0) * stride;
  int out = 0;
  if (j > 0 && target <= nnz) {
    int lo = 0, hi = m;
    while (lo < hi) {
      const int mid = lo + (hi - lo) / 2;
      if (rp[mid] < target) lo = mid + 1; else hi = mid;
    }
    out = (rp[lo] == target) ? lo : (lo > 0 ? lo - 1 : 0);
  }
  bp[j] = out;
}

__device__ __forceinline__ int tile_end_excl(const int *__restrict__ rp, const int *__restrict__ bp, int t, int ntiles,
                                             int m, int t1) {
  if (t == ntiles - 1) return m;
  int e = bp[t + 1];
  e = e < m ? e : m;
  return (e < m && rp[e] < t1) ? e + 1 : e;
}

template <int NPT, bool NTC, bool NTV, bool EARLY, bool C16 = false, bool SEGSUM = false, bool HINT = false>
__global__ __launch_bounds__(kThreads) __attribute__((amdgpu_waves_per_eu(EARLY || NPT > 8 ? 1 : 7, 8))) void flat_tile_kernel(int m, int nnz, int ntiles, double alpha, double beta,
                                                             const int *__restrict__ rp, const int *__restrict__ bp,
                                                             const int *__restrict__ ci,
                                                             const double *__restrict__ v,
                                                             const double *__restrict__ x, double *y, const double *yin,
                                                             double *__restrict__ head, double *__restrict__ tail,
                                                             int *__restrict__ tail_row, int *__restrict__ tail_end,
                                                             int xcd_chunk, int reach, int tile0,
                                                             const int *__restrict__ guard, int *__restrict__ stale,
                                                             Col16Dev c16, int reverse, int cache_ends,
                                                             const int4v *__restrict__ dig, const unsigned char *__restrict__ cold) {
  check_plan_guard(rp, m, guard, stale);
  constexpr int STRIDE = kThreads * NPT;
  static_assert(STRIDE / 64 <= kTileSpans, "TileSpans must hold every >= 64-product span of one tile");
  __shared__ __attribute__((aligned(16))) double lds[STRIDE];
  __shared__ double sh_tail_sum, sh_tail_yold;
  __shared__ int sh_tail_row;
  __shared__ TileSpans spans;
  if (threadIdx.x == 0) {
    sh_tail_row = -1;
    spans.n = 0;
  }
  int t = (reverse & 1) ? zigzag_block(blockIdx.x, ntiles) : static_cast<int>(blockIdx.x);
  if (xcd_chunk > 0) t = xcd_chunked_block(t, ntiles, xcd_chunk);
  const int t0 = (t + tile0) * STRIDE;
  const int t1 = (nnz - t0 > STRIDE) ? t0 + STRIDE : nnz;

  StreamRegs<EARLY ? NPT : 4> early_regs;
  const bool early = EARLY && xcd_chunk >= 0 && stage_fast_ok(t1, nnz);
  if (EARLY && early) stage_issue<kThreads, EARLY ? NPT : 4, NTC, NTV>(early_regs, t0, t1, ci, v);

  const int4v rec = dig[t];
  const int first = rec.x;
  const int end_excl = rec.y;
  const int nrows = end_excl - first;
  int w = 1;
  while (!SEGSUM && w < 64 && nrows * (w * 2) <= kThreads) w <<= 1;
  const int lane = threadIdx.x & (w - 1);
  const int vec_id = threadIdx.x / w;
  const int vecs = kThreads / w;
  const bool live0 = vec_id < nrows;
  int a0 = 0, b0 = 0;
  if (live0) {
    a0 = rp[first + vec_id];
    b0 = rp[first + vec_id + 1];
  }
  const bool early_y = beta != 0.0;
  double y_old0 = 0.0;
  if (early_y && live0 && lane == 0) y_old0 = yin[first + vec_id];

  constexpr int FIN_STEPS = kFlatFinish / kWave;
  int fin_c[FIN_STEPS];
  double fin_v[FIN_STEPS];
  bool fin = false;
  if (reach > 0 && nrows > 0 && t < ntiles - 1 && threadIdx.x < kWave) {
    const int la = rec.z, lb = rec.w;
    fin = la >= t0 && lb > t1 && lb - t1 <= reach;
    if (fin) {
#pragma unroll
      for (int k = 0; k < FIN_STEPS; ++k) {
        const int j = t1 + static_cast<int>(threadIdx.x) + k * kWave;
        fin_c[k] = j < lb ? load_stream(ci + j) : -1;
        fin_v[k] = j < lb ? load_stream(v + j) : 0.0;
      }
    }
  }

  if (C16) check_ci_guard(ci, c16, stale);
  if (C16 && stage_fast_ok(t1, nnz))
    stage_products_c16<kThreads, NPT, NTC, NTV>(lds, t0, t0, t1, c16, v, x);
  else if (EARLY && early) stage_finish<kThreads, EARLY ? NPT : 4>(lds, early_regs, x);
  else if (NTC && NTV && cache_ends > 0 && (t < cache_ends || t >= ntiles - cache_ends))
    stage_products<kThreads, NPT, false, false, HINT>(lds, t0, t1, nnz, ci, v, x, xcd_chunk >= 0, cold, (reverse & 2) != 0);
  else stage_products<kThreads, NPT, NTC, NTV, HINT>(lds, t0, t1, nnz, ci, v, x, xcd_chunk >= 0, cold, (reverse & 2) != 0);

  double fin_extra = 0.0;
  if (fin) {
#pragma unroll
    for (int k = 0; k < FIN_STEPS; ++k)
      if (fin_c[k] >= 0) fin_extra += fin_v[k] * x[fin_c[k]];
  }

  __shared__ unsigned char seg_head[SEGSUM ? STRIDE : 1];
  __shared__ double seg_wave_sum[kThreads / kWave];
  __shared__ int seg_wave_flag[kThreads / kWave];
  if (SEGSUM) {
#pragma unroll
    for (int e = 0; e < NPT; ++e) seg_head[NPT * threadIdx.x + e] = 0;
  }

  __syncthreads();

  if (SEGSUM) {
    if (threadIdx.x == 0) seg_head[0] = 1;
    for (int base = 0; base < nrows; base += kThreads) {
      const int i = base + static_cast<int>(threadIdx.x);
      if (i < nrows) {
        const int a = (base == 0) ? a0 : rp[first + i];
        const int b = (base == 0) ? b0 : rp[first + i + 1];
        if (a >= t0 && a < t1 && b > a) seg_head[a - t0] = 1;
      }
    }
    __syncthreads();
    const int c0 = NPT * static_cast<int>(threadIdx.x);
    double run = 0.0;
    int first_head = NPT;
#pragma unroll
    for (int e = 0; e < NPT; ++e) {
      if (seg_head[c0 + e]) {
        run = 0.0;
        first_head = first_head == NPT ? e : first_head;
      }
      run += lds[c0 + e];
      lds[c0 + e] = run;
    }
    double sv = run;
    int sf = first_head < NPT ? 1 : 0;
    const int wl = threadIdx.x & (kWave - 1);
#pragma unroll
    for (int d = 1; d < kWave; d <<= 1) {
      const double pv = __shfl_up(sv, d, kWave);
      const int pf = __shfl_up(sf, d, kWave);
      if (wl >= d && !sf) {
// ... 95 lines not shown
  if (t >= ntiles) return;
  const int t0 = (t + tile0) * stride;
  const int t1 = (nnz - t0 > stride) ? t0 + stride : nnz;
  int first = bp[t];
  first = first < m ? first : m;
  const int end_excl = tile_end_excl(rp, bp, t, ntiles, m, t1);
  if (end_excl <= first) return;
  atomicMax(flag + 1, end_excl - first);
  if (t == ntiles - 1) return;
  const int r = end_excl - 1;
  if (rp[r] >= t0 && rp[r + 1] - t1 > kFlatFinish) *flag = 1;
}

__global__ __launch_bounds__(256) void flat_fixup_kernel(int ntiles, int stride, int tile0, double alpha, double beta,
                                                         const double *__restrict__ head,
                                                         const double *__restrict__ tail,
                                                         const int *__restrict__ tail_row,
                                                         const int *__restrict__ tail_end, double *y, const double *yin) {
  const int t = blockIdx.x * 256 + threadIdx.x;
  int r = -1;
  if (t < ntiles - 1) r = tail_row[t];
  int k0 = 0, k1 = 0;
  double s = 0.0;
  if (r >= 0) {
    const long long b = tail_end[t];
    k0 = t + 1;
    k1 = static_cast<int>((b + stride - 1) / stride) - tile0;
    k1 = k1 < ntiles ? k1 : ntiles;
    s = tail[t];
  }
  s += wave_range_sum(head, k0, k1);
  if (r >= 0) store_y(y, yin, r, alpha, beta, s);
}

}

void launch_break_points_from(hipStream_t stream, const int *rp, int m, int nnz, int stride, int tile0, int *bp, int bp_len) {
  if (bp_len <= 0) return;
  SPMV_ACC_LAUNCH(break_points_kernel, dim3((bp_len + 255) / 256), dim3(256), 0, stream, rp, m, nnz, stride, tile0, bp,
                     bp_len);
}
void launch_break_points(hipStream_t stream, const int *rp, int m, int nnz, int stride, int *bp, int bp_len) {
  launch_break_points_from(stream, rp, m, nnz, stride, 0, bp, bp_len);
}

namespace {
template <int NPT, bool NTC, bool NTV>
void launch_flat_variant(hipStream_t stream, const CsrDev &A, const FlatPlan &P, double alpha, double beta, const double *x,
                         double *y) {
  const Col16Dev none = {};
  if (P.early_stream)
    SPMV_ACC_LAUNCH((flat_tile_kernel<NPT, NTC, NTV, true>), dim3(P.ntiles), dim3(kThreads), 0, stream, A.m, A.nnz,
                       P.ntiles, alpha, beta, A.rp, P.bp, A.ci, A.v, x, y, A.yin ? A.yin : y, P.head, P.tail, P.tail_row, P.tail_end,
                       P.xcd_chunk, P.needs_fixup ? 0 : kFlatFinish, P.tile0, A.guard, A.stale, none, (P.reverse ? 1 : 0) | (x32_ok(A) ? 2 : 0), P.cache_ends, static_cast<const int4v *>(P.digest), nullptr);
  else
    SPMV_ACC_LAUNCH((flat_tile_kernel<NPT, NTC, NTV, false>), dim3(P.ntiles), dim3(kThreads), 0, stream, A.m, A.nnz,
                       P.ntiles, alpha, beta, A.rp, P.bp, A.ci, A.v, x, y, A.yin ? A.yin : y, P.head, P.tail, P.tail_row, P.tail_end,
                       P.xcd_chunk, P.needs_fixup ? 0 : kFlatFinish, P.tile0, A.guard, A.stale, none, (P.reverse ? 1 : 0) | (x32_ok(A) ? 2 : 0), P.cache_ends, static_cast<const int4v *>(P.digest), nullptr);
}
template <bool NTC, bool NTV>
void launch_flat_segsum(hipStream_t stream, const CsrDev &A, const FlatPlan &P, double alpha, double beta, const double *x,
                        double *y) {
  const Col16Dev none = {};
  SPMV_ACC_LAUNCH((flat_tile_kernel<kNnzPerThread, NTC, NTV, false, false, true>), dim3(P.ntiles), dim3(kThreads), 0, stream, A.m,
                     A.nnz, P.ntiles, alpha, beta, A.rp, P.bp, A.ci, A.v, x, y, A.yin ? A.yin : y, P.head, P.tail, P.tail_row, P.tail_end,
                     P.xcd_chunk, P.needs_fixup ? 0 : kFlatFinish, P.tile0, A.guard, A.stale, none, (P.reverse ? 1 : 0) | (x32_ok(A) ? 2 : 0), P.cache_ends,
                     static_cast<const int4v *>(P.digest), nullptr);
}
template <bool NTC, bool NTV>
void launch_flat_hint(hipStream_t stream, const CsrDev &A, const FlatPlan &P, double alpha, double beta, const double *x, double *y) {
  const Col16Dev none = {};
  SPMV_ACC_LAUNCH((flat_tile_kernel<kNnzPerThread, NTC, NTV, false, false, false, true>), dim3(P.ntiles), dim3(kThreads), 0, stream, A.m,
                     A.nnz, P.ntiles, alpha, beta, A.rp, P.bp, A.ci, A.v, x, y, A.yin ? A.yin : y, P.head, P.tail, P.tail_row, P.tail_end,
                     P.xcd_chunk, P.needs_fixup ? 0 : kFlatFinish, P.tile0, A.guard, A.stale, none, (P.reverse ? 1 : 0) | (x32_ok(A) ? 2 : 0), P.cache_ends,
                     static_cast<const int4v *>(P.digest), A.cold);
}
template <bool NTC, bool NTV>
void launch_flat_col16(hipStream_t stream, const CsrDev &A, const FlatPlan &P, double alpha, double beta, const double *x,
                       double *y) {
  const Col16Dev c = col16_dev(*P.col16, A);
  SPMV_ACC_LAUNCH((flat_tile_kernel<kNnzPerThread, NTC, NTV, false, true>), dim3(P.ntiles), dim3(kThreads), 0, stream, A.m,
                     A.nnz, P.ntiles, alpha, beta, A.rp, P.bp, A.ci, A.v, x, y, A.yin ? A.yin : y, P.head, P.tail, P.tail_row, P.tail_end,
                     P.xcd_chunk, P.needs_fixup ? 0 : kFlatFinish, P.tile0, A.guard, A.stale, c, (P.reverse ? 1 : 0) | 2, P.cache_ends, static_cast<const int4v *>(P.digest), nullptr);
}
template <int NPT>
void launch_flat_policy(hipStream_t stream, const CsrDev &A, const FlatPlan &P, double alpha, double beta, const double *x,
                        double *y) {
  switch (P.stream_policy & 3) {
  case 1: launch_flat_variant<NPT, false, false>(stream, A, P, alpha, beta, x, y); break;
  case 2: launch_flat_variant<NPT, false, true>(stream, A, P, alpha, beta, x, y); break;
  case 3: launch_flat_variant<NPT, true, false>(stream, A, P, alpha, beta, x, y); break;
  default: launch_flat_variant<NPT, true, true>(stream, A, P, alpha, beta, x, y); break;
  }
}
}

void launch_flat_digest(hipStream_t stream, const CsrDev &A, const FlatPlan &P) {
  if (P.ntiles <= 0) return;
  SPMV_ACC_LAUNCH(flat_digest_kernel, dim3((P.ntiles + 255) / 256), dim3(256), 0, stream, A.rp, P.bp, P.ntiles, A.m, A.nnz, P.stride,
                     P.tile0, static_cast<int4v *>(P.digest));
}

void launch_flat_needs_fixup(hipStream_t stream, const CsrDev &A, const FlatPlan &P, int *d_flag) {
  if (P.ntiles <= 0) return;
  SPMV_ACC_LAUNCH(flat_needs_fixup_kernel, dim3((P.ntiles + 255) / 256), dim3(256), 0, stream, A.rp, P.bp, P.ntiles,
                     A.m, A.nnz, P.stride, P.tile0, d_flag);
}

void launch_flat(hipStream_t stream, const CsrDev &A, const FlatPlan &P, double alpha, double beta, const double *x,
                 double *y) {
  if (P.ntiles <= 0) return;
  const int npt = P.stride / kThreads;
  if (P.segment_sum && npt == kNnzPerThread) {
    switch (P.stream_policy & 3) {
    case 1: launch_flat_segsum<false, false>(stream, A, P, alpha, beta, x, y); break;
    case 2: launch_flat_segsum<false, true>(stream, A, P, alpha, beta, x, y); break;
    case 3: launch_flat_segsum<true, false>(stream, A, P, alpha, beta, x, y); break;
    default: launch_flat_segsum<true, true>(stream, A, P, alpha, beta, x, y); break;
    }
  } else if (A.cold != nullptr && !P.col16 && !P.early_stream && npt == kNnzPerThread) {
    switch (P.stream_policy & 3) {
    case 1: launch_flat_hint<false, false>(stream, A, P, alpha, beta, x, y); break;
    case 2: launch_flat_hint<false, true>(stream, A, P, alpha, beta, x, y); break;
    case 3: launch_flat_hint<true, false>(stream, A, P, alpha, beta, x, y); break;
    default: launch_flat_hint<true, true>(stream, A, P, alpha, beta, x, y); break;
    }
  } else if (P.col16 && P.col16->state == 1 && x32_ok(A) && npt == kNnzPerThread) {
    switch (P.stream_policy & 3) {
    case 1: launch_flat_col16<false, false>(stream, A, P, alpha, beta, x, y); break;
    case 2: launch_flat_col16<false, true>(stream, A, P, alpha, beta, x, y); break;
    case 3: launch_flat_col16<true, false>(stream, A, P, alpha, beta, x, y); break;
    default: launch_flat_col16<true, true>(stream, A, P, alpha, beta, x, y); break;
    }
  } else if (npt == 4) launch_flat_policy<4>(stream, A, P, alpha, beta, x, y);
  else if (npt == 16) launch_flat_policy<16>(stream, A, P, alpha, beta, x, y);
  else launch_flat_policy<8>(stream, A, P, alpha, beta, x, y);
// ... 8 lines not shown
```

spmv_acc_amd/csrc/k_rowblock.hip:

```cpp
#include "device_utils.hpp"
#include "kernels.hpp"
#include "tile_stage.hpp"

namespace spmv_acc {
namespace {

using namespace dev;

template <int CTRL> __device__ __forceinline__ int dpp_shr_or_zero(int v) {
  return __builtin_amdgcn_update_dpp(0, v, CTRL, 0xF, 0xF, false);
}
__device__ __forceinline__ int wave_inclusive_scan(int v) {
  v += dpp_shr_or_zero<0x111>(v);
  v += dpp_shr_or_zero<0x112>(v);
  v += dpp_shr_or_zero<0x114>(v);
  v += dpp_shr_or_zero<0x118>(v);
  const int t0 = __builtin_amdgcn_readlane(v, 15), t1 = __builtin_amdgcn_readlane(v, 31), t2 = __builtin_amdgcn_readlane(v, 47);
  const int r = (threadIdx.x & (kWave - 1)) >> 4;
  return v + (r > 0 ? t0 : 0) + (r > 1 ? t1 : 0) + (r > 2 ? t2 : 0);
}

template <int VEC, bool NTC, bool NTV, bool LENS, bool HINT = false, bool C16 = false>
__global__ __launch_bounds__(kThreads) void rowblock_stream_kernel(int m, int nnz, int nblocks, int rpb, int flags,
                                                                   double alpha, double beta,
                                                                   const int *__restrict__ rp,
                                                                   const int *__restrict__ ci,
                                                                   const double *__restrict__ v,
                                                                   const double *__restrict__ x,
                                                                   double *y, const double *yin,
                                                                   const int *__restrict__ guard,
                                                                   int *__restrict__ stale,
                                                                   const unsigned char *__restrict__ lens,
                                                                   const int *__restrict__ base, int cache_ends,
                                                                   const unsigned char *__restrict__ cold, Col16Dev c16) {
  check_plan_guard(rp, m, guard, stale);
  if (C16) check_ci_guard(ci, c16, stale);
  __shared__ int wave_tot[kThreads / kWave];
  __shared__ __attribute__((aligned(16))) double lds[kTile];
  __shared__ TileSpans2K spans;
  if (threadIdx.x == 0) spans.n = 0;

  int b = blockIdx.x;
  if (flags & 64) b = zigzag_block(b, nblocks);
  if (flags & 4) b = xcd_chunked_block(b, nblocks, flags >> 8);

  const long long base_ll = static_cast<long long>(b) * rpb;
  const int row_base = static_cast<int>(base_ll);
  const int row_end = (base_ll + rpb < m) ? row_base + rpb : m;
  int s0, s1;
  bool from_lens = false;
  if (LENS) {
    const int b0 = base[b];
    s0 = b0 & 0x7fffffff;
    s1 = base[b + 1] & 0x7fffffff;
    from_lens = b0 >= 0;
  } else {
    s0 = rp[row_base];
    s1 = rp[row_end];
  }

  const int lane = threadIdx.x % VEC;
  const int row = row_base + threadIdx.x / VEC;
  const bool live = row < row_end;
  int r0 = 0, r1 = 0, len = 0;
  if (LENS && from_lens) {
    if (live) len = lens[row];
  } else if (live) {
    r0 = rp[row];
    r1 = rp[row + 1];
  }
  const bool writer = live && lane == 0;
  double y_old = 0.0;
  if (beta != 0.0 && writer) y_old = yin[row];

  double acc = 0.0;
  int incl = 0;
  const int lo4 = s0 & ~3;
  const int off0 = (C16 && lo4 < s1) ? (s0 & ~(kCol16Chunk - 1)) : lo4;
  const bool c16_ok = C16 && stage_fast_ok(s1, nnz);
  for (int off = off0; off < s1; off += kTile) {
    const bool cached_end = NTC && NTV && cache_ends > 0 && (b < cache_ends || b >= nblocks - cache_ends);
    if (C16 && c16_ok) {
      if (cached_end) stage_products_c16<kThreads, kNnzPerThread, false, false>(lds, off, lo4 > off ? lo4 : off, s1, c16, v, x);
      else stage_products_c16<kThreads, kNnzPerThread, NTC, NTV>(lds, off, lo4 > off ? lo4 : off, s1, c16, v, x);
    } else if (cached_end)
      stage_products<kThreads, kNnzPerThread, false, false, HINT>(lds, off, s1, nnz, ci, v, x, true, cold, (flags & 128) != 0);
    else
      stage_products<kThreads, kNnzPerThread, NTC, NTV, HINT>(lds, off, s1, nnz, ci, v, x, true, cold, (flags & 128) != 0);
    if (LENS && from_lens && off == off0) {
      incl = wave_inclusive_scan(lane == 0 ? len : 0);
      if ((threadIdx.x & (kWave - 1)) == kWave - 1) wave_tot[threadIdx.x / kWave] = incl;
    }
    __syncthreads();
    if (LENS && from_lens && off == off0) {
      const int w = threadIdx.x / kWave;
      int before = s0;
#pragma unroll
      for (int k = 0; k < kThreads / kWave - 1; ++k) before += (k < w) ? wave_tot[k] : 0;
      r1 = before + incl;
      r0 = r1 - len;
    }
    const int lo = (r0 > off ? r0 : off) - off;
    const int hi = (r1 < off + kTile ? r1 : off + kTile) - off;
    acc += tile_row_sum<kThreads>(lds, spans, lo, hi > lo ? hi : lo, lane, VEC);
    if (off + kTile < s1) __syncthreads();
  }
  acc = group_sum<VEC>(acc);
  if (writer) {
    __builtin_nontemporal_store(beta == 0.0 ? alpha * acc : alpha * acc + beta * y_old, y + row);
  }
}

__global__ __launch_bounds__(256) void max_block_nnz_kernel(const int *__restrict__ rp, int m, int rpb, int nblocks,
                                                            int avg_block, int *__restrict__ out) {
  const int b = blockIdx.x * 256 + threadIdx.x;
  int v = 0;
  bool off = false;
  if (b < nblocks) {
    const long long lo = static_cast<long long>(b) * rpb;
    const long long hi = lo + rpb < m ? lo + rpb : m;
    v = rp[hi] - rp[lo];
    const long long d = static_cast<long long>(v) - avg_block;
    off = hi - lo == rpb && (20 * (d < 0 ? -d : d) > 7LL * avg_block || v > kTile);
  }
  const unsigned long long votes = __ballot(off);
#pragma unroll
  for (int o = 32; o > 0; o >>= 1) {
    const int other = __shfl_xor(v, o, 64);
    v = other > v ? other : v;
  }
  if ((threadIdx.x & 63) == 0) {
    if (v > 0) atomicMax(out, v);
    if (votes) atomicAdd(out + 1, __popcll(votes));
  }
}

__global__ __launch_bounds__(256) void row_digest_base_kernel(const int *__restrict__ rp, int m, int rpb, int nblocks,
                                                              int *__restrict__ base) {
  const int b = blockIdx.x * 256 + threadIdx.x;
  if (b > nblocks) return;
  const long long r = static_cast<long long>(b) * rpb;
  base[b] = rp[r < m ? r : m];
}
__global__ __launch_bounds__(256) void row_digest_lens_kernel(const int *__restrict__ rp, int m, int rpb,
                                                              unsigned char *__restrict__ lens, int *__restrict__ base) {
  const long long r = static_cast<long long>(blockIdx.x) * 256 + threadIdx.x;
  if (r >= m) return;
  const int len = rp[r + 1] - rp[r];
  lens[r] = static_cast<unsigned char>(len < 255 ? (len > 0 ? len : 0) : 255);
  if (len > 255 || len < 0) atomicOr(base + r / rpb, static_cast<int>(0x80000000u));
}

template <int VEC, bool NC, bool NV, bool LN, bool H, bool C>
void launch_rb_instance(hipStream_t stream, const CsrDev &A, const RowDigest *D, const Col16Dev &c16, int nblocks, int rpb, int flags,
                        double alpha, double beta, const double *x, double *y, int cache_ends) {
  SPMV_ACC_LAUNCH((rowblock_stream_kernel<VEC, NC, NV, LN, H, C>), dim3(nblocks), dim3(kThreads), 0, stream, A.m, A.nnz, nblocks, rpb, flags,
                     alpha, beta, A.rp, A.ci, A.v, x, y, A.yin ? A.yin : y, A.guard, A.stale,
                     LN ? D->lens : static_cast<const unsigned char *>(nullptr), LN ? D->base : static_cast<const int *>(nullptr), cache_ends,
                     H ? A.cold : static_cast<const unsigned char *>(nullptr), c16);
}

template <int VEC, bool NC, bool NV>
void launch_policy(hipStream_t stream, const CsrDev &A, const RowDigest *D, const Col16 *C, int nblocks, int rpb, int flags, double alpha,
                   double beta, const double *x, double *y, int cache_ends) {
  const bool lens = VEC <= 2 && D && D->lens;
  const bool c16 = C && C->state == 1 && A.cold == nullptr && x32_ok(A);
  const Col16Dev cd = c16 ? col16_dev(*C, A) : Col16Dev{};
#define SPMV_ACC_RB(LN, H, CC) launch_rb_instance<VEC, NC, NV, LN, H, CC>(stream, A, D, cd, nblocks, rpb, flags, alpha, beta, x, y, cache_ends)
  if constexpr (VEC <= 2) {
    if (lens) {
      if (c16) SPMV_ACC_RB(true, false, true);
      else if (A.cold) SPMV_ACC_RB(true, true, false);
      else SPMV_ACC_RB(true, false, false);
      return;
    }
  }
  if (c16) SPMV_ACC_RB(false, false, true);
  else if (A.cold) SPMV_ACC_RB(false, true, false);
  else SPMV_ACC_RB(false, false, false);
#undef SPMV_ACC_RB
}

template <int VEC>
void launch_vec(hipStream_t stream, const CsrDev &A, const RowDigest *D, const Col16 *C, int rpb, int xcd, double alpha, double beta,
                const double *x, double *y, int cache_ends) {
  if (rpb < 1 || rpb > kThreads / VEC) rpb = kThreads / VEC;
  if (D && D->rpb != rpb) D = nullptr;
  const int nblocks = static_cast<int>((static_cast<long long>(A.m) + rpb - 1) / rpb);
  if (nblocks == 0) return;
  const int remap = (xcd & ~0xb) | (x32_ok(A) ? 128 : 0);
  switch ((xcd >> 4) & 3) {
  case 1: launch_policy<VEC, false, false>(stream, A, D, C, nblocks, rpb, remap, alpha, beta, x, y, cache_ends); break;
  case 2: launch_policy<VEC, false, true>(stream, A, D, C, nblocks, rpb, remap, alpha, beta, x, y, cache_ends); break;
  case 3: launch_policy<VEC, true, false>(stream, A, D, C, nblocks, rpb, remap, alpha, beta, x, y, cache_ends); break;
  default: launch_policy<VEC, true, true>(stream, A, D, C, nblocks, rpb, remap, alpha, beta, x, y, cache_ends); break;
  }
}

}

void launch_max_block_nnz(hipStream_t stream, const int *rp, int m, int rows_per_block, int avg_block, int *d_out) {
  const int nblocks = static_cast<int>((static_cast<long long>(m) + rows_per_block - 1) / rows_per_block);
  if (nblocks <= 0) return;
  SPMV_ACC_LAUNCH(max_block_nnz_kernel, dim3((nblocks + 255) / 256), dim3(256), 0, stream, rp, m, rows_per_block,
                     nblocks, avg_block, d_out);
}

void launch_row_digest(hipStream_t stream, const int *rp, int m, int rows_per_block, unsigned char *lens, int *base) {
  if (m <= 0 || rows_per_block <= 0) return;
  const int nblocks = static_cast<int>((static_cast<long long>(m) + rows_per_block - 1) / rows_per_block);
  SPMV_ACC_LAUNCH(row_digest_base_kernel, dim3((nblocks + 1 + 255) / 256), dim3(256), 0, stream, rp, m, rows_per_block, nblocks,
                     base);
  SPMV_ACC_LAUNCH(row_digest_lens_kernel, dim3(static_cast<unsigned>((static_cast<long long>(m) + 255) / 256)), dim3(256), 0,
                     stream, rp, m, rows_per_block, lens, base);
}

void launch_rowblock_stream(hipStream_t stream, const CsrDev &A, int vec, int rows_per_block, int xcd_remap,
                            double alpha, double beta, const double *x, double *y, const RowDigest *digest, int cache_ends,
                            const Col16 *col16) {
  switch (vec) {
// ... 23 lines not shown
```

spmv_acc_amd/csrc/kernels.hpp:

```cpp
#pragma once

#include <hip/hip_runtime_api.h>
#include <hip/hip_ext.h>

namespace spmv_acc {

bool kernel_clock_next(hipEvent_t *start, hipEvent_t *stop);
#define SPMV_ACC_LAUNCH(kernel, grid, block, shmem, stream, ...)                                                                  \
  do {                                                                                                                           \
    hipEvent_t kc_e0_ = nullptr, kc_e1_ = nullptr;                                                                               \
    if (::spmv_acc::kernel_clock_next(&kc_e0_, &kc_e1_))                                                                         \
      hipExtLaunchKernelGGL(kernel, grid, block, shmem, stream, kc_e0_, kc_e1_, 0, __VA_ARGS__);                                 \
    else                                                                                                                         \
      hipLaunchKernelGGL(kernel, grid, block, shmem, stream, __VA_ARGS__);                                                       \
  } while (0)

struct CsrDev {
  int m = 0;
  int n = 0;
  int nnz = 0;
  int nnz0 = 0;
  int count() const { return nnz - nnz0; }
  const int *rp = nullptr;
  const int *ci = nullptr;
// ... 37 lines not shown

constexpr int kThreads = 256;
constexpr int kMaxGridBlocks = 8388593;
int max_grid_blocks();
constexpr int kNnzPerThread = 8;
constexpr int kTile = kThreads * kNnzPerThread;
constexpr int kVectorTarget = 1900;
constexpr int kPlusThreads = 256;
constexpr int kPlusR = 2;
constexpr int kPlusMinNnz = 2 * kPlusR * kPlusThreads;
constexpr int kPlusLongChunk = 2 * kPlusMinNnz;

void launch_vector_row(hipStream_t stream, const CsrDev &A, int row_split, int w0, int w1, double alpha, double beta,
                       const double *x, double *y, bool single_row_groups = false);

void launch_vector_tile(hipStream_t stream, const CsrDev &A, int row_split, int w0, int w1, double avg0, double avg1,
                        int target_products, int xcd_chunk, int stream_policy, double alpha, double beta, const double *x,
                        double *y, bool reverse = false);

void launch_light(hipStream_t stream, const CsrDev &A, int w, int grid_blocks, unsigned *counter, double alpha, double beta, const double *x,
                  double *y);
void launch_block_row(hipStream_t stream, const CsrDev &A, int grid_blocks, double alpha, double beta, const double *x, double *y);

void launch_wave_row(hipStream_t stream, const CsrDev &A, double alpha, double beta, const double *x, double *y);

struct RowDigest {
  int rpb = 0;
  unsigned char *lens = nullptr;
  int *base = nullptr;
};
struct Col16;
void launch_rowblock_stream(hipStream_t stream, const CsrDev &A, int vec, int rows_per_block, int flags,
                            double alpha, double beta, const double *x, double *y, const RowDigest *digest = nullptr,
                            int cache_ends = 0, const Col16 *col16 = nullptr);
void launch_row_digest(hipStream_t stream, const int *rp, int m, int rows_per_block, unsigned char *lens, int *base);
void pick_rowblock_shape(int m, int nnz, int target_products, int *vec, int *rows_per_block);

void launch_max_block_nnz(hipStream_t stream, const int *rp, int m, int rows_per_block, int avg_block, int *d_out);
constexpr int kRowblockMaxRounds = 8;

void launch_break_points(hipStream_t stream, const int *rp, int m, int nnz, int stride, int *bp, int bp_len);

constexpr int kCol16Chunk = 256;
struct Col16 {
  int state = -1;
  int chunk0 = 0;
  int nchunks = 0;
  int rec_ints = 0;
  int bits = 0;
  unsigned short *d16 = nullptr;
  unsigned char *d8 = nullptr;
  int *rec = nullptr;
  int *ovf = nullptr;
  int *ci_guard = nullptr;
  long long escapes = 0;
  long long overflow = 0;
  size_t bytes = 0;
};
struct Col16Dev {
  const unsigned short *d16;
  const unsigned char *d8;
  const int *rec;
  const int *ovf;
  const int *ci_guard;
  int rec_ints;
  int guard_lo, guard_span;
};
inline Col16Dev col16_dev(const Col16 &C, const CsrDev &A) {
  Col16Dev d;
  d.d16 = C.d16 ? C.d16 - static_cast<long long>(C.chunk0) * kCol16Chunk : nullptr;
  d.d8 = C.d8 ? C.d8 - static_cast<long long>(C.chunk0) * kCol16Chunk : nullptr;
  d.rec = C.rec - static_cast<long long>(C.chunk0) * C.rec_ints;
  d.ovf = C.ovf;
  d.ci_guard = C.ci_guard;
  d.rec_ints = C.rec_ints;
  d.guard_lo = A.nnz0;
  d.guard_span = A.count() > 0 ? A.count() - 1 : 0;
  return d;
}
constexpr int kHintLineShift = 4;
constexpr int kHintBins = 4096;
constexpr int kHintSamples = 8 << 20;
void launch_hint_census(hipStream_t stream, const int *ci, int nnz, int ncols, int stride, int samples, unsigned *counts);
void launch_hint_hist(hipStream_t stream, const unsigned *counts, int nlines, unsigned *hist_lines, unsigned long long *hist_hits);
void launch_hint_bits(hipStream_t stream, const int *ci, int nnz, int ncols, const unsigned *counts, unsigned threshold, unsigned char *bits);

size_t col16_scan_bytes(int nchunks);
void launch_col16_base(hipStream_t stream, const int *ci, int nnz, int chunk0, int nchunks, int *base, int *esc_count, unsigned long long *stats);
void launch_col16_overflow(hipStream_t stream, int *cnt, int nchunks, int E);
bool launch_col16_scan(hipStream_t stream, int nchunks, const int *esc_count, int *esc_start, void *tmp, size_t tmp_bytes);
void launch_col16_encode(hipStream_t stream, const int *ci, int nnz, int chunk0, int nchunks, const int *base, const int *ovf_start, int R,
                         int bits, void *codes, int *rec, int *ovf);
void launch_col16_guard(hipStream_t stream, const int *ci, int lo, int span, int *out);

struct FlatPlan {
  int stride = 0;
  int ntiles = 0;
  int tile0 = 0;
  int *bp = nullptr;
  double *head = nullptr;
  double *tail = nullptr;
  int *tail_row = nullptr;
  int *tail_end = nullptr;
  void *digest = nullptr;
  int xcd_chunk = 0;
  int stream_policy = 0;
  bool can_finish = false;
  bool needs_fixup = true;
  int max_tile_rows = 0;
  bool early_stream = false;
  bool reverse = false;
  int cache_ends = 0;
  bool segment_sum = false;
  const Col16 *col16 = nullptr;
  bool mode_tuned[2] = {false, false};
  bool tuned_fixup[2] = {true, true};
};
constexpr int kFlatFinish = 128;
void launch_break_points_from(hipStream_t stream, const int *rp, int m, int nnz, int stride, int tile0, int *bp, int bp_len);
void launch_flat_digest(hipStream_t stream, const CsrDev &A, const FlatPlan &P);
void launch_flat_needs_fixup(hipStream_t stream, const CsrDev &A, const FlatPlan &P, int *d_flag);
void launch_flat(hipStream_t stream, const CsrDev &A, const FlatPlan &P, double alpha, double beta, const double *x,
                 double *y);

void launch_plus_digest(hipStream_t stream, const CsrDev &A, const int *bp, const int *fbr, int nblocks, int long_chunk, void *blk,
                        int *d_has_long);
void launch_plus(hipStream_t stream, const CsrDev &A, const int *bp, const int *fbr, const void *blk, int nblocks,
                 bool has_long_rows, int xcd_chunk, int stream_policy, double *partial, double alpha, double beta,
                 const double *x, double *y, bool reverse = false);

size_t plus_analyze_device_workspace_bytes(int m);
bool plus_analyze_device_count(hipStream_t stream, const int *rp, int m, int min_nnz, int threads_per_block,
                               int vec_size, void *workspace, int *d_total);
void plus_analyze_device_emit(hipStream_t stream, const int *rp, int m, int min_nnz, const void *workspace, int *d_bp,
                              int *d_fbr);

void launch_slab_count(hipStream_t stream, const CsrDev &A, int width, int S, int *cnt);
void launch_slab_scatter(hipStream_t stream, const CsrDev &A, int width, int S, const int *rps, const long long *off, int *ci_out,
                         double *v_out, bool values_only = false);
void launch_slab_flags(hipStream_t stream, const int *rps, int m, int *flags);
void launch_slab_compact(hipStream_t stream, const int *rps, const int *pos, int m, int *rowid, int *crp);
void launch_slab_merge(hipStream_t stream, int ms, const int *rowid, const double *ys, double *y);
void launch_value_samples(hipStream_t stream, const double *v, const int *ci, long long lo, long long span, int count, unsigned long long *saved, int *changed);
constexpr int kValueSamples = 65536;
constexpr int kSlabCopyAfterCalls = 32;
// ... 23 lines not shown
```

spmv_acc_amd/csrc/plan.cpp:

```cpp
#include "engine_internal.hpp"

namespace spmv_acc {
using namespace detail;

namespace detail {

constexpr int kGuardSlots = 4096;
struct GuardPool {
  int *d_guard = nullptr;
  int *h_flags = nullptr;
  std::deque<std::pair<int, hipEvent_t>> free_slots;
  bool failed = false;
};
std::mutex g_guard_mu;
std::map<int, GuardPool> g_guard_pools;

int guard_acquire(int device, const int **d_guard, int **h_flag) {
  std::lock_guard<std::mutex> lk(g_guard_mu);
  GuardPool &P = g_guard_pools[device];
  if (P.failed) return -1;
  if (!P.d_guard) {
    if (hipMalloc(reinterpret_cast<void **>(&P.d_guard), sizeof(int) * kGuardSlots * kGuardSamples) != hipSuccess ||
        hipHostMalloc(reinterpret_cast<void **>(&P.h_flags), sizeof(int) * kGuardSlots,
                      hipHostMallocCoherent | hipHostMallocMapped | hipHostMallocPortable) != hipSuccess) {
// ... 428 lines not shown
  std::vector<PlanKey> gone;
  for (auto &kv : g_plans) {
    if (!kv.second->is_stale()) continue;
    PlanKey k = kv.first;
    std::get<6>(k) = 0;
    if (std::find(gone.begin(), gone.end(), k) == gone.end()) gone.push_back(k);
  }
  for (const PlanKey &k : gone) {
    erase_with_sibling_locked(k);
    ++dropped;
  }
  if (dropped) set_error(kErrBadArgument, kStaleText);
  return dropped;
}


void release_plans(const int *d_rowptr, int m_only) {
  std::lock_guard<std::mutex> lk(g_mu);
  for (auto it = g_plans.begin(); it != g_plans.end();) {
    if (!d_rowptr || (std::get<1>(it->first) == d_rowptr && (m_only < 0 || std::get<4>(it->first) == m_only))) {
      it = g_plans.erase(it);
    } else {
      ++it;
    }
  }
  drain_deferred_locked();
}

bool query_plan(const int *d_rowptr, int m, PlanInfo *out) {
  std::lock_guard<std::mutex> lk(g_mu);
  for (auto &kv : g_plans) {
    if (std::get<1>(kv.first) == d_rowptr && std::get<4>(kv.first) == m && std::get<6>(kv.first) == 0) {
      const Plan &p = *kv.second;
      out->nnz = p.A.nnz;
      out->adaptive_branch = p.have_samples ? adaptive_branch(m, p.samples) : 0;
      int rb_vec = 1, rb_rows = kThreads;
      pick_rowblock_shape(m, p.A.count(), rowblock_target_for(p), &rb_vec, &rb_rows);
      out->vec = rb_vec;
      out->flat_tiles = p.flat_tiles;
      out->plus_blocks = p.plus_blocks;
      out->aligned16 = p.A.aligned16 ? 1 : 0;
      const int afam = p.adaptive_family[1] >= 0 ? p.adaptive_family[1] : p.adaptive_family[0];
      int fam = afam;
      for (int f = 0; fam < 0 && f < kFamilyCount; ++f)
        if (p.stream_policy[f][1] >= 0 || p.stream_policy[f][0] >= 0) fam = f;
      out->stream_policy = fam < 0 ? -1 : (p.stream_policy[fam][1] >= 0 ? p.stream_policy[fam][1] : p.stream_policy[fam][0]);
      out->flat_fixup = p.flat_tiles > 0 ? (p.flat.needs_fixup ? 1 : 0) : -1;
      out->adaptive_family = afam;
      out->adaptive_family_beta0 = p.adaptive_family[0];
      out->settled = p.calls > 0 && !p.tuning_open ? 1 : 0;
      out->last_kernel = p.last_kernel;
      out->col16 = p.last_c16;
      out->col_bits = p.last_col_bits;
      out->slab_passes = p.seg_state == 1 && (tun(kT_slab_segments) >= 1 || (tun(kT_slab_segments) < 0 && p.seg_choice == 1)) ? p.seg_slabs - (p.seg_rest_below > 0 ? 1 : 0) : 0;
      return true;
    }
  }
  return false;
}

int cached_plan_count() {
  std::lock_guard<std::mutex> lk(g_mu);
  int n = 0;
  for (auto &kv : g_plans) n += std::get<6>(kv.first) == 0 ? 1 : 0;
  return n;
}

namespace detail {
bool plan_settled_for(const int *rp, const int *ci, const double *v, int m, int n, int strategy, int cls) {
  int dev = 0;
  if (hipGetDevice(&dev) != hipSuccess) return true;
  std::lock_guard<std::mutex> lk(g_mu);
  auto it = g_plans.find(PlanKey(dev, rp, ci, v, m, n, 0));
  if (it == g_plans.end()) return false;
  const Plan &p = *it->second;
  return strategy >= 0 && strategy < 32 && ((p.settled_for[cls & 1] >> strategy) & 1u);
}

bool rule_twin_exists(const int *rp, const int *ci, const double *v, int m, int n) {
  int dev = 0;
  if (hipGetDevice(&dev) != hipSuccess) return false;
  std::lock_guard<std::mutex> lk(g_mu);
  return g_plans.find(PlanKey(dev, rp, ci, v, m, n, 1)) != g_plans.end();
}

void drop_rule_twin(const int *rp, const int *ci, const double *v, int m, int n) {
  int dev = 0;
  if (hipGetDevice(&dev) != hipSuccess) return;
  std::lock_guard<std::mutex> lk(g_mu);
  auto it = g_plans.find(PlanKey(dev, rp, ci, v, m, n, 1));
  if (it != g_plans.end() && !it->second->captured) g_plans.erase(it);
}
}

}
```

spmv_acc_amd/csrc/tile_stage.hpp:

```cpp
#pragma once

#include "device_utils.hpp"
#include "kernels.hpp"

namespace spmv_acc {
namespace dev {

template <int THREADS, int NPT, bool NTC, bool NTV, bool HINT>
__device__ __forceinline__ void stage_products_all(double *__restrict__ lds, int a0, int hi, const int *__restrict__ ci,
                                                   const double *__restrict__ v, const double *__restrict__ x,
                                                   const unsigned char *__restrict__ cold) {
  constexpr int K = NPT / 4;
  int4v c[K];
  double2v va[K], vb[K];
  unsigned nib[K];
#pragma unroll
  for (int k = 0; k < K; ++k) {
    const int j = a0 + 4 * (threadIdx.x + k * THREADS);
    const int jc = (j < hi) ? j : a0;
    c[k] = load_stream_i4<NTC>(ci + jc);
    va[k] = load_stream_d2<NTV>(v + jc);
    vb[k] = load_stream_d2<NTV>(v + jc + 2);
    if (HINT) nib[k] = static_cast<unsigned>(cold[jc >> 3]) >> (jc & 4);
  }
// ... 137 lines not shown
      xg[k][0] = x[R.c[k].x];
      xg[k][1] = x[R.c[k].y];
      xg[k][2] = x[R.c[k].z];
      xg[k][3] = x[R.c[k].w];
    }
  }
#pragma unroll
  for (int k = 0; k < K; ++k) {
    if (R.has[k]) {
      const int g = threadIdx.x + k * THREADS;
      double2v p0, p1;
      p0.x = R.va[k].x * xg[k][0];
      p0.y = R.va[k].y * xg[k][1];
      p1.x = R.vb[k].x * xg[k][2];
      p1.y = R.vb[k].y * xg[k][3];
      double2v *dst = reinterpret_cast<double2v *>(lds + 4 * g);
      dst[0] = p0;
      dst[1] = p1;
    }
  }
}

typedef unsigned int uint2v __attribute__((ext_vector_type(2)));
typedef uint2v uint2v_a2 __attribute__((aligned(2)));

template <int BITS> struct Codes4;
template <> struct Codes4<16> {
  static constexpr int escape = 0xFFFF;
  uint2v d;
  template <bool NT> __device__ __forceinline__ void load(const Col16Dev &C, int j) {
    const uint2v_a2 *p = reinterpret_cast<const uint2v_a2 *>(C.d16 + j);
    d = NT ? __builtin_nontemporal_load(p) : *p;
  }
  __device__ __forceinline__ void split(int (&dq)[4]) const {
    dq[0] = static_cast<int>(d.x & 0xFFFFu);
    dq[1] = static_cast<int>(d.x >> 16);
    dq[2] = static_cast<int>(d.y & 0xFFFFu);
    dq[3] = static_cast<int>(d.y >> 16);
  }
};
template <> struct Codes4<8> {
  static constexpr int escape = 0xFF;
  unsigned d;
  template <bool NT> __device__ __forceinline__ void load(const Col16Dev &C, int j) {
    const unsigned *p = reinterpret_cast<const unsigned *>(C.d8 + j);
    d = NT ? __builtin_nontemporal_load(p) : *p;
  }
  __device__ __forceinline__ void split(int (&dq)[4]) const {
#pragma unroll
    for (int q = 0; q < 4; ++q) dq[q] = static_cast<int>((d >> (8 * q)) & 0xFFu);
  }
};

template <int BITS>
__device__ __forceinline__ void c16_decode(int (&c)[4], const Codes4<BITS> &d, int rv, int R, int lane, const int *__restrict__ ovf) {
  constexpr int ESC = Codes4<BITS>::escape;
  const int bs = __builtin_amdgcn_readlane(rv, 0);
  const int nesc = __builtin_amdgcn_readlane(rv, 1);
  int dq[4];
  d.split(dq);
#pragma unroll
  for (int q = 0; q < 4; ++q) c[q] = bs + dq[q];
  if (nesc > 0) {
    const int E = R - 4;
    const unsigned long long lt = (1ull << lane) - 1ull;
    const bool e[4] = {dq[0] == ESC, dq[1] == ESC, dq[2] == ESC, dq[3] == ESC};
    const unsigned long long slot[4] = {__ballot(e[0]), __ballot(e[1]), __ballot(e[2]), __ballot(e[3])};
    int r = __popcll(slot[0] & lt) + __popcll(slot[1] & lt) + __popcll(slot[2] & lt) + __popcll(slot[3] & lt);
#pragma unroll
    for (int q = 0; q < 4; ++q) {
      if (slot[q]) {
        const int got = __shfl(rv, (4 + r) & (kWave - 1), kWave);
        if (e[q]) c[q] = r < E ? got : ovf[__builtin_amdgcn_readlane(rv, 2) + r - E];
      }
      r += e[q] ? 1 : 0;
    }
  }
}

template <int THREADS, int NPT, bool NTC, bool NTV, int BITS>
__device__ __forceinline__ void stage_products_c16_all(double *__restrict__ lds, int a0, int lo4, int hi, const Col16Dev &C,
                                                       const double *__restrict__ v, const double *__restrict__ x) {
  constexpr int K = NPT / 4;
  Codes4<BITS> d[K];
  double2v va[K], vb[K];
  int rv[K];
  const int lane = threadIdx.x & (kWave - 1);
  const int R = C.rec_ints;
  const int rl = lane < R ? lane : 0;
#pragma unroll
  for (int k = 0; k < K; ++k) {
    const int wave_j = __builtin_amdgcn_readfirstlane(a0 + 4 * ((threadIdx.x & ~(kWave - 1)) + k * THREADS));
    rv[k] = C.rec[static_cast<long long>(wave_j >> 8) * R + rl];
  }
#pragma unroll
  for (int k = 0; k < K; ++k) d[k].template load<NTC>(C, a0 + 4 * (threadIdx.x + k * THREADS));
#pragma unroll
  for (int k = 0; k < K; ++k) {
    const int j = a0 + 4 * (threadIdx.x + k * THREADS);
    const int jv = (j >= lo4 && j < hi) ? j : lo4;
    va[k] = load_stream_d2<NTV>(v + jv);
    vb[k] = load_stream_d2<NTV>(v + jv + 2);
  }
  double xg[K][4];
#pragma unroll
  for (int k = 0; k < K; ++k) {
    const int j = a0 + 4 * (threadIdx.x + k * THREADS);
    int c[4];
    c16_decode(c, d[k], rv[k], R, lane, C.ovf);
    const bool mine = j >= lo4 && j < hi;
    const int bs = __builtin_amdgcn_readlane(rv[k], 0);
#pragma unroll
    for (int q = 0; q < 4; ++q) xg[k][q] = gather_u32(x, mine ? c[q] : bs);
  }
#pragma unroll
  for (int k = 0; k < K; ++k) {
    const int g = threadIdx.x + k * THREADS;
    double2v p0, p1;
    p0.x = va[k].x * xg[k][0];
    p0.y = va[k].y * xg[k][1];
    p1.x = vb[k].x * xg[k][2];
    p1.y = vb[k].y * xg[k][3];
    double2v *dst = reinterpret_cast<double2v *>(lds + 4 * g);
    dst[0] = p0;
    dst[1] = p1;
  }
}

template <int THREADS, int NPT, bool NTC, bool NTV, int BITS>
__device__ __forceinline__ void stage_products_c16_tail(double *__restrict__ lds, int a0, int lo4, int hi, const Col16Dev &C,
                                                        const double *__restrict__ v, const double *__restrict__ x) {
  const int lane = threadIdx.x & (kWave - 1);
  const int R = C.rec_ints;
  const int rl = lane < R ? lane : 0;
#pragma nounroll
  for (int k = 0; k < NPT / 4 - 1; ++k) {
    const int wave_j = __builtin_amdgcn_readfirstlane(a0 + 4 * ((threadIdx.x & ~(kWave - 1)) + k * THREADS));
    if (wave_j >= hi) break;
    const int g = threadIdx.x + k * THREADS;
    const int j = a0 + 4 * g;
    const int rv = C.rec[static_cast<long long>(wave_j >> 8) * R + rl];
    Codes4<BITS> d;
    d.template load<NTC>(C, j);
    const int jv = (j >= lo4 && j < hi) ? j : lo4;
    const double2v va = load_stream_d2<NTV>(v + jv), vb = load_stream_d2<NTV>(v + jv + 2);
    int c[4];
    c16_decode(c, d, rv, R, lane, C.ovf);
    const bool mine = j >= lo4 && j < hi;
    const int bs = __builtin_amdgcn_readlane(rv, 0);
    double xg[4];
#pragma unroll
    for (int q = 0; q < 4; ++q) xg[q] = gather_u32(x, mine ? c[q] : bs);
    double2v p0, p1;
    p0.x = va.x * xg[0];
    p0.y = va.y * xg[1];
    p1.x = vb.x * xg[2];
    p1.y = vb.y * xg[3];
    double2v *dst = reinterpret_cast<double2v *>(lds + 4 * g);
    dst[0] = p0;
    dst[1] = p1;
  }
}

template <int THREADS, int NPT, bool NTC, bool NTV>
__device__ __forceinline__ void stage_products_c16(double *__restrict__ lds, int a0, int lo4, int hi, const Col16Dev &C,
                                                   const double *__restrict__ v, const double *__restrict__ x) {
  const int last_j = __builtin_amdgcn_readfirstlane(a0 + 4 * ((threadIdx.x & ~(kWave - 1)) + (NPT / 4 - 1) * THREADS));
  if (C.d8 != nullptr) {
    if (last_j < hi) stage_products_c16_all<THREADS, NPT, NTC, NTV, 8>(lds, a0, lo4, hi, C, v, x);
    else stage_products_c16_tail<THREADS, NPT, NTC, NTV, 8>(lds, a0, lo4, hi, C, v, x);
  } else {
    if (last_j < hi) stage_products_c16_all<THREADS, NPT, NTC, NTV, 16>(lds, a0, lo4, hi, C, v, x);
    else stage_products_c16_tail<THREADS, NPT, NTC, NTV, 16>(lds, a0, lo4, hi, C, v, x);
  }
}

__device__ __forceinline__ void check_ci_guard(const int *__restrict__ ci, const Col16Dev &C, int *__restrict__ stale) {
  if (C.ci_guard != nullptr && stale != nullptr && blockIdx.x == 0 && threadIdx.x < kWave) {
    const int idx = C.guard_lo + static_cast<int>(static_cast<long long>(threadIdx.x) * C.guard_span / (kWave - 1));
    if (ci[idx] != C.ci_guard[threadIdx.x]) __hip_atomic_store(stale, 1, __ATOMIC_RELAXED, __HIP_MEMORY_SCOPE_SYSTEM);
  }
}

constexpr int kTileSpans = 64;
template <int N> struct TileSpansN {
  int n;
  int lo[N], hi[N];
  double sum[N];
};
typedef TileSpansN<kTileSpans> TileSpans;
typedef TileSpansN<32> TileSpans2K;

template <int THREADS, class Spans>
__device__ __forceinline__ double tile_row_sum(const double *__restrict__ lds, Spans &sh, int lo, int hi, int lane, int w) {
  const int span = hi - lo;
  const bool posted = w < kWave && span >= 64 && span > 16 * w;
  int slot = -1;
  double s = 0.0;
  if (posted) {
    if (lane == 0) {
      slot = atomicAdd(&sh.n, 1);
      sh.lo[slot] = lo;
      sh.hi[slot] = hi;
    }
  } else {
    int j = lo + lane;
    for (; j + 3 * w < hi; j += 4 * w) {
      const double a = lds[j], b = lds[j + w], c = lds[j + 2 * w], d = lds[j + 3 * w];
      s += a;
      s += b;
      s += c;
      s += d;
    }
    for (; j < hi; j += w) s += lds[j];
  }
  const int n = __syncthreads_count(posted && lane == 0);
  if (n > 0) {
    const int wave = threadIdx.x / kWave, l = threadIdx.x & (kWave - 1);
    for (int e = wave; e < n; e += THREADS / kWave) {
      double t = 0.0;
      const int b = sh.hi[e];
      for (int j = sh.lo[e] + l; j < b; j += kWave) t += lds[j];
      t = group_sum<64>(t);
      if (l == 0) sh.sum[e] = t;
    }
    __syncthreads();
// ... 52 lines not shown
```

spmv_acc_amd/csrc/tuner.cpp:

```cpp
#include "engine_internal.hpp"

namespace spmv_acc {
using namespace detail;

namespace detail {

bool build_flat_plan(const CsrDev &A, int stride, hipStream_t stream, FlatPlan &F) {
  if (!plan_work_allowed("flat: break points and tile digests")) return false;
  ++t_plan_work;
  Plan::free_flat_plan(F);
  const int nnz = A.nnz;
  const int tile0 = A.nnz0 / stride;
  const int tiles = nnz / stride + (nnz % stride ? 1 : 0) - tile0;
  const size_t n1 = static_cast<size_t>(tiles) + 1;
  if (!hip_ok(hipMalloc(reinterpret_cast<void **>(&F.bp), sizeof(int) * n1), "hipMalloc break points") ||
      !hip_ok(hipMalloc(reinterpret_cast<void **>(&F.head), sizeof(double) * n1), "hipMalloc head carries") ||
      !hip_ok(hipMalloc(reinterpret_cast<void **>(&F.tail), sizeof(double) * n1), "hipMalloc tail carries") ||
      !hip_ok(hipMalloc(reinterpret_cast<void **>(&F.tail_row), sizeof(int) * n1), "hipMalloc tail rows") ||
      !hip_ok(hipMalloc(reinterpret_cast<void **>(&F.tail_end), sizeof(int) * n1), "hipMalloc tail ends") ||
      !hip_ok(hipMalloc(&F.digest, 16 * n1), "hipMalloc tile digest")) {
    Plan::free_flat_plan(F);
    return false;
  }
  F.stride = stride;
  F.ntiles = tiles;
  F.tile0 = tile0;
  launch_break_points_from(stream, A.rp, A.m, nnz, stride, tile0, F.bp, static_cast<int>(n1));
  launch_flat_digest(stream, A, F);
  int *d_flag = nullptr;
  int h_flag[2] = {1, 0};
  if (!hip_ok(hipMalloc(reinterpret_cast<void **>(&d_flag), 2 * sizeof(int)), "hipMalloc flat flag")) {
    Plan::free_flat_plan(F);
    return false;
  }
  bool probed = hip_ok(hipMemsetAsync(d_flag, 0, 2 * sizeof(int), stream), "memset flat flag");
  if (probed) {
    launch_flat_needs_fixup(stream, A, F, d_flag);
    probed = hip_ok(hipMemcpyAsync(h_flag, d_flag, 2 * sizeof(int), hipMemcpyDeviceToHost, stream), "read flat flag") &&
             hip_ok(hipStreamSynchronize(stream), "sync flat flag");
  }
  (void)hipFree(d_flag);
  if (!probed) {
    Plan::free_flat_plan(F);
    return false;
  }
  F.max_tile_rows = h_flag[1];
  F.can_finish = h_flag[0] == 0;
  F.needs_fixup = true;
  F.mode_tuned[0] = F.mode_tuned[1] = false;
  return true;
}


thread_local bool t_flat_segment_sum = false;

int flat_stride_for(const Plan &p) {
  if (flat_segment_sum()) return kThreads * kNnzPerThread;
  if (tun(kT_col16) > 0) return kThreads * kNnzPerThread;
  int npt = tun(kT_flat_npt);
  if (npt < 0) npt = p.flat_npt_choice > 0 ? p.flat_npt_choice : kNnzPerThread;
  return kThreads * ((npt == 4 || npt == 16) ? npt : kNnzPerThread);
}

bool ensure_flat(Plan &p, hipStream_t stream) {
  const int stride = flat_stride_for(p);
  if (p.flat_tiles >= 0 && p.flat.stride == stride) return true;
  p.flat_tiles = -1;
  if (!build_flat_plan(p.A, stride, stream, p.flat)) return false;
  p.flat_tiles = p.flat.ntiles;
  if (p.flat_geometry_tuned) p.flat.early_stream = p.flat_early_choice && stride != kThreads * 16;
  for (int c = 0; c < 2; ++c) {
    if (p.flat_mode_choice[c] < 0) continue;
    p.flat.mode_tuned[c] = true;
    p.flat.tuned_fixup[c] = p.flat_mode_choice[c] == 1 || !p.flat.can_finish;
  }
  return true;
}

int analyze_on_device(hipStream_t stream, const int *d_rp, int m, int min_nnz, int threads, int vec, int **d_bp_out,
                      int **d_fbr_out) {
  void *ws = nullptr;
  int *d_total = nullptr;
  int blocks = -1;
  *d_bp_out = *d_fbr_out = nullptr;
  if (!hip_ok(hipMalloc(&ws, plus_analyze_device_workspace_bytes(m)), "hipMalloc analysis workspace")) return -1;
  if (hip_ok(hipMalloc(reinterpret_cast<void **>(&d_total), sizeof(int)), "hipMalloc analysis total")) {
    if (!plus_analyze_device_count(stream, d_rp, m, min_nnz, threads, vec, ws, d_total)) {
      set_error(kErrHip, "device row-block analysis: scan failed");
    } else {
      int total = 0;
      if (hip_ok(hipMemcpyAsync(&total, d_total, sizeof(int), hipMemcpyDeviceToHost, stream), "read block count") &&
          hip_ok(hipStreamSynchronize(stream), "sync analysis") &&
          hip_ok(hipMalloc(reinterpret_cast<void **>(d_bp_out), sizeof(int) * (static_cast<size_t>(total) + 1)),
                 "hipMalloc plus bp") &&
          hip_ok(hipMalloc(reinterpret_cast<void **>(d_fbr_out), sizeof(int) * (static_cast<size_t>(m) + 1)),
                 "hipMalloc plus fbr")) {
        plus_analyze_device_emit(stream, d_rp, m, min_nnz, ws, *d_bp_out, *d_fbr_out);
        if (hip_ok(hipStreamSynchronize(stream), "sync analysis emit")) blocks = total;
      }
    }
    (void)hipFree(d_total);
  }
  (void)hipFree(ws);
  if (blocks < 0) {
    if (*d_bp_out) (void)hipFree(*d_bp_out);
    if (*d_fbr_out) (void)hipFree(*d_fbr_out);
    *d_bp_out = *d_fbr_out = nullptr;
  }
  return blocks;
}

// ... 113 lines not shown


bool tune_log_enabled() {
  static const bool on = [] {
    const char *e = std::getenv("SPMV_ACC_TUNE_LOG");
    return e && *e && *e != '0';
  }();
  return on;
}
void tune_log(const char *fmt, ...) {
  if (!tune_log_enabled()) return;
  va_list ap;
  va_start(ap, fmt);
  std::fputs("[spmv_acc tune] ", stderr);
  std::vfprintf(stderr, fmt, ap);
  std::fputc('\n', stderr);
  va_end(ap);
}

thread_local double *t_scratch = nullptr;
thread_local size_t t_scratch_len = 0;
double *tune_scratch(size_t len) {
  if (t_scratch && t_scratch_len >= len) return t_scratch;
  if (t_scratch) (void)hipFree(t_scratch);
  t_scratch = nullptr;
  t_scratch_len = 0;
  if (!hip_ok(hipMalloc(reinterpret_cast<void **>(&t_scratch), sizeof(double) * (len ? len : 1)), "hipMalloc tune y")) {
    t_scratch = nullptr;
    return nullptr;
  }
  t_scratch_len = len;
  return t_scratch;
}
void release_tune_scratch() {
  if (t_scratch) (void)hipFree(t_scratch);
  t_scratch = nullptr;
  t_scratch_len = 0;
}



bool ensure_col16(Plan &p, hipStream_t st) {
  Col16 &C = p.col16;
  if (C.state >= 0) return true;
  if (!plan_work_allowed("the 16-bit column encoding")) return false;
  const CsrDev &A = p.A;
  const int chunk0 = A.nnz0 / (kThreads * kNnzPerThread) * (kThreads * kNnzPerThread / kCol16Chunk);
  const int nchunks = (A.nnz + kCol16Chunk - 1) / kCol16Chunk - chunk0;
  if (!x32_ok(A) || nchunks < 64) {
    C.state = 0;
    return true;
  }
  ++t_plan_work;
  int *base = nullptr, *cnt = nullptr, *ovf_start = nullptr;
  unsigned long long *stats = nullptr;
  void *tmp = nullptr;
  const size_t tmp_bytes = col16_scan_bytes(nchunks);
  const size_t n1 = static_cast<size_t>(nchunks) + 1;
  bool ok = hip_ok(hipMalloc(reinterpret_cast<void **>(&base), sizeof(int) * 2 * n1), "hipMalloc col16 bases") &&
            hip_ok(hipMalloc(reinterpret_cast<void **>(&cnt), sizeof(int) * 2 * n1), "hipMalloc col16 escape counts") &&
            hip_ok(hipMalloc(reinterpret_cast<void **>(&ovf_start), sizeof(int) * n1), "hipMalloc col16 overflow offsets") &&
            hip_ok(hipMalloc(reinterpret_cast<void **>(&stats), sizeof(unsigned long long) * 8), "hipMalloc col16 statistics") &&
            hip_ok(hipMalloc(&tmp, tmp_bytes > 0 ? tmp_bytes : 16), "hipMalloc col16 scan workspace") &&
            hip_ok(hipMemsetAsync(cnt + nchunks, 0, sizeof(int), st), "memset col16") &&
            hip_ok(hipMemsetAsync(cnt + n1 + nchunks, 0, sizeof(int), st), "memset col16") &&
            hip_ok(hipMemsetAsync(stats, 0, sizeof(unsigned long long) * 8, st), "memset col16 statistics");
  unsigned long long h_stats[8] = {0, 0, 0, 0, 0, 0, 0, 0};
  int R = 0, total = 0, bits = 16;
  if (ok) {
    launch_col16_base(st, A.ci, A.nnz, chunk0, nchunks, base, cnt, stats);
    ok = hip_ok(hipMemcpyAsync(h_stats, stats, sizeof(h_stats), hipMemcpyDeviceToHost, st), "read col16 statistics") &&
         hip_ok(hipStreamSynchronize(st), "sync col16 statistics");
  }
  if (ok) {
    const unsigned long long limit = static_cast<unsigned long long>(nchunks) / 100;
    R = h_stats[1] <= limit ? 16 : (h_stats[2] <= limit ? 32 : (h_stats[3] <= limit ? 64 : 0));
    const int R8 = h_stats[5] <= limit ? 16 : (h_stats[6] <= limit ? 32 : (h_stats[7] <= limit ? 64 : 0));
    const long long extra8 = static_cast<long long>(h_stats[4]) - static_cast<long long>(h_stats[0]);
    const int mode = tun(kT_col16);
    bits = mode == 8 || (mode != 2 && R > 0 && R8 > 0 && R8 <= R && 200 * extra8 <= static_cast<long long>(A.count())) ? 8 : 16;
    if (bits == 8) R = R8;
    const int forced = tun(kT_col16) > 1 ? tun(kT_col16) : 0;
    if (forced == 16 || forced == 32 || forced == 64) R = forced;
    tune_log("m %d nnz %d 16-bit columns: %llu escapes in %d chunks, %llu / %llu / %llu chunks above 12 / 28 / 60 -> %s", A.m, A.nnz, h_stats[0], nchunks,
             h_stats[1], h_stats[2], h_stats[3], R ? (R == 16 ? "16-int records" : (R == 32 ? "32-int records" : "64-int records")) : "not encoded");
    tune_log("m %d nnz %d 8-bit columns: %llu escapes (%+lld), %llu / %llu / %llu chunks above 12 / 28 / 60 -> %d-bit codes", A.m, A.nnz, h_stats[4], extra8,
             h_stats[5], h_stats[6], h_stats[7], bits);
  }
  if (ok && R > 0) {
    const size_t cofs = bits == 8 ? n1 : 0;
    launch_col16_overflow(st, cnt + cofs, nchunks, R - 4);
    ok = launch_col16_scan(st, nchunks, cnt + cofs, ovf_start, tmp, tmp_bytes) &&
         hip_ok(hipMemcpyAsync(&total, ovf_start + nchunks, sizeof(int), hipMemcpyDeviceToHost, st), "read col16 overflow total") &&
         hip_ok(hipStreamSynchronize(st), "sync col16");
    const size_t code_bytes = static_cast<size_t>(bits / 8) * static_cast<size_t>(nchunks) * kCol16Chunk;
    const size_t rec_bytes = sizeof(int) * static_cast<size_t>(nchunks) * R;
    const size_t ovf_bytes = sizeof(int) * (static_cast<size_t>(total) + 64);
    void *codes = nullptr;
    ok = ok && hip_ok(hipMalloc(&codes, code_bytes), "hipMalloc col16 offsets") &&
         hip_ok(hipMalloc(reinterpret_cast<void **>(&C.rec), rec_bytes), "hipMalloc col16 records") &&
         hip_ok(hipMalloc(reinterpret_cast<void **>(&C.ovf), ovf_bytes), "hipMalloc col16 overflow list") &&
         hip_ok(hipMalloc(reinterpret_cast<void **>(&C.ci_guard), sizeof(int) * kGuardSamples), "hipMalloc col16 guard") &&
         hip_ok(hipMemsetAsync(C.rec, 0, rec_bytes, st), "memset col16 records") && hip_ok(hipMemsetAsync(C.ovf, 0, ovf_bytes, st), "memset col16 overflow");
    if (bits == 8) C.d8 = static_cast<unsigned char *>(codes);
    else C.d16 = static_cast<unsigned short *>(codes);
    if (ok) {
      launch_col16_encode(st, A.ci, A.nnz, chunk0, nchunks, base + cofs, ovf_start, R, bits, codes, C.rec, C.ovf);
      launch_col16_guard(st, A.ci, A.nnz0, A.count() > 0 ? A.count() - 1 : 0, C.ci_guard);
      ok = hip_ok(hipStreamSynchronize(st), "sync col16 encode");
    }
    C.bytes = code_bytes + rec_bytes + ovf_bytes;
  }
  for (void *q : {static_cast<void *>(base), static_cast<void *>(cnt), static_cast<void *>(ovf_start), static_cast<void *>(stats), tmp})
    if (q) (void)hipFree(q);
  if (!ok) {
    p.free_col16();
    return false;
  }
  if (R == 0) {
    p.free_col16();
    C.state = 0;
    return true;
  }
  C.state = 1;
  C.chunk0 = chunk0;
  C.nchunks = nchunks;
  C.rec_ints = R;
  C.bits = bits;
  C.escapes = static_cast<long long>(h_stats[bits == 8 ? 4 : 0]);
  C.overflow = total;
  return true;
}


void launch_flat_plan(hipStream_t st, const CsrDev &A, FlatPlan &F, int policy, double alpha, double beta, const double *x,
                      double *y, bool reverse) {
  F.xcd_chunk = tun(kT_xcd_chunk);
  F.stream_policy = policy;
  const int early = tun(kT_flat_early);
  if (early >= 0) F.early_stream = early != 0;
  F.reverse = reverse;
  F.cache_ends = tun(kT_cache_ends_mb) > 0 && tun(kT_zigzag) ? static_cast<int>(tun(kT_cache_ends_mb) * 1048576.0 / (12.0 * F.stride)) : 0;
  launch_flat(st, A, F, alpha, beta, x, y);
}
void launch_flat_with(hipStream_t st, Plan &p, int policy, double alpha, double beta, const double *x, double *y) {
  p.flat.segment_sum = flat_segment_sum();
  launch_flat_plan(st, p.A, p.flat, policy, alpha, beta, x, y, next_reverse(p));
}

bool autotune_flat_mode(Plan &p, hipStream_t st, const double *x) {
  FlatPlan &F = p.flat;
  const int forced = tun(kT_flat_finish);
  if (!F.can_finish || F.ntiles <= 1) {
    F.needs_fixup = !F.can_finish;
    return true;
  }
  if (forced >= 0) {
    F.needs_fixup = forced == 0;
    return true;
  }
  if (tun(kT_deterministic)) {
    F.needs_fixup = false;
    return true;
  }
  const int cls = t_beta_class;
  if (F.mode_tuned[cls]) {
    F.needs_fixup = F.tuned_fixup[cls];
    return true;
  }
  if (!t_capturing && defer_tuning()) {
    F.needs_fixup = false;
    return true;
  }
  if (t_capturing) {
    F.needs_fixup = F.mode_tuned[cls ^ 1] ? F.tuned_fixup[cls ^ 1] : false;
    return true;
  }
  if (t_coarse_tuning && p.A.count() >= flat_small_nnz()) {
    F.needs_fixup = true;
    return true;
  }
  TimingPhase ph(st, p.A.m);
  bool ok = ph.ok;
  float ms[2] = {0.f, 0.f};
  for (int mode = 0; ok && mode < 2; ++mode) {
    F.needs_fixup = mode == 0;
    ok = ph.time([&] { launch_flat_with(st, p, policy_for(p, kFamFlat), 1.0, trial_beta(), x, ph.y); }, &ms[mode]);
  }
  F.tuned_fixup[cls] = F.needs_fixup = !(ok && ms[1] < ms[0]);
  F.mode_tuned[cls] = ok;
  if (ok) p.flat_mode_choice[cls] = F.tuned_fixup[cls] ? 1 : 0;
  if (ok) tune_log("m %d nnz %d beta class %d flat cut rows: carries + fix-up %.2f us, finished in the tile %.2f us", p.A.m, p.A.nnz, cls, ms[0] * 1e3f, ms[1] * 1e3f);
  return ok;
}

bool autotune_flat_geometry(Plan &p, hipStream_t st, const double *x) {
  if (p.flat_geometry_tuned || tun(kT_col16) > 0 || flat_segment_sum() || t_capturing || by_rule()) return true;
  if (p.A.count() >= flat_small_nnz() || p.flat.ntiles <= 1) {
    p.flat_geometry_tuned = true;
    return true;
  }
  const bool time_npt = tun(kT_flat_npt) < 0, time_early = tun(kT_flat_early) < 0;
  if (!time_npt && !time_early) return true;
  TimingPhase ph(st, p.A.m);
  bool ok = ph.ok;
  const int pol = policy_for(p, kFamFlat);
  FlatPlan alt;
  FlatPlan *plans[2] = {&p.flat, nullptr};
  if (ok && time_npt) {
    const int other = p.flat.stride == kThreads * 4 ? kThreads * kNnzPerThread : kThreads * 4;
    ok = build_flat_plan(p.A, other, st, alt);
    if (ok) {
      alt.needs_fixup = alt.tuned_fixup[0] = alt.tuned_fixup[1] = !alt.can_finish;
      alt.mode_tuned[0] = alt.mode_tuned[1] = true;
      plans[1] = &alt;
    }
  }
  float best = 1e30f;
  int best_plan = 0;
  bool best_early = false;
  for (int k = 0; ok && k < 2; ++k) {
    if (!plans[k]) continue;
    for (int e = 0; ok && e < (time_early ? 2 : 1); ++e) {
      plans[k]->early_stream = time_early ? e != 0 : plans[k]->early_stream;
      float ms = 0.f;
      ok = ph.time([&] { launch_flat_plan(st, p.A, *plans[k], pol, 1.0, trial_beta(), x, ph.y, next_reverse(p)); }, &ms);
      if (ok) tune_log("m %d nnz %d flat geometry: %d non-zeros per tile, stream-first %d -> %.2f us", p.A.m, p.A.nnz, plans[k]->stride,
                       plans[k]->early_stream ? 1 : 0, ms * 1e3f);
      if (ok && ms < best) {
        best = ms;
        best_plan = k;
        best_early = plans[k]->early_stream;
      }
    }
  }
  if (ok) {
    if (best_plan == 1) {
      Plan::free_flat_plan(p.flat);
      p.flat = alt;
      alt = FlatPlan();
      p.flat_tiles = p.flat.ntiles;
    }
    p.flat.early_stream = p.flat_early_choice = best_early;
    p.flat_npt_choice = p.flat.stride / kThreads;
    p.flat_geometry_tuned = true;
    for (int c = 0; c < 2; ++c) p.flat_mode_choice[c] = p.flat.mode_tuned[c] ? (p.flat.tuned_fixup[c] ? 1 : 0) : -1;
  }
  Plan::free_flat_plan(alt);
  return ok;
}
// ... 296 lines not shown
```

Before: 570.0.

## Pack col16 chunk records into variable-size granules with window descriptors

Replaces the fixed-size per-chunk escape records of the compressed 16/8-bit column encoding with variable-length 64-byte granules sized by each chunk's escape count. Per-chunk and per-rowblock window descriptors locate the records. The aim is to cut the bytes read for column metadata when records would otherwise be padded to 32 or 64 ints. The cost is an extra descriptor load per tile or block, added setup kernels, and more complex indexing in the kernels.

```diff
diff --git a/include/spmv_acc.h b/include/spmv_acc.h
--- a/include/spmv_acc.h
+++ b/include/spmv_acc.h
@@ -105,6 +105,7 @@
 int spmv_acc_query_plan_settled(const int *d_rowptr, int m);
 int spmv_acc_query_plan_col16(const int *d_rowptr, int m);
 int spmv_acc_query_plan_col_bits(const int *d_rowptr, int m);
+int spmv_acc_query_plan_col_packed(const int *d_rowptr, int m);
 enum spmv_acc_kernel {
   SPMV_ACC_KERNEL_ROWBLOCK = 0,
   SPMV_ACC_KERNEL_ROWBLOCK_PLUS = 1,
diff --git a/spmv_acc_amd/__init__.py b/spmv_acc_amd/__init__.py
--- a/spmv_acc_amd/__init__.py
+++ b/spmv_acc_amd/__init__.py
@@ -25,7 +25,7 @@
     "spmv_acc_set_stream", "spmv_acc_get_stream", "spmv_acc_last_error", "spmv_acc_last_error_string",
     "spmv_acc_clear_error", "spmv_acc_time_spmv", "spmv_acc_version", "spmv_acc_set_tunable",
     "spmv_acc_get_tunable", "spmv_acc_reset_tunables", "spmv_acc_time_spmv_total", "spmv_acc_copy_ceiling_gbs", "spmv_acc_adaptive_plus_analyze_device", "spmv_acc_prepare",
-    "spmv_acc_last_prepare_us", "spmv_acc_sharded_spmv", "spmv_acc_shard_prepare", "spmv_acc_csr_spmv_chunks", "spmv_acc_query_plan_settled", "spmv_acc_query_plan_col16", "spmv_acc_query_plan_col_bits", "spmv_acc_time_spmv_cold", "spmv_acc_csr_spmv_oop", "spmv_acc_check_plans",
+    "spmv_acc_last_prepare_us", "spmv_acc_sharded_spmv", "spmv_acc_shard_prepare", "spmv_acc_csr_spmv_chunks", "spmv_acc_query_plan_settled", "spmv_acc_query_plan_col16", "spmv_acc_query_plan_col_bits", "spmv_acc_query_plan_col_packed", "spmv_acc_time_spmv_cold", "spmv_acc_csr_spmv_oop", "spmv_acc_check_plans",
     "spmv_acc_query_plan_beta0", "spmv_acc_query_plan_slab_passes", "spmv_acc_shard_create", "spmv_acc_shard_step", "spmv_acc_shard_pipeline",
     "spmv_acc_shard_destroy", "spmv_acc_rccl_comm_init_all", "spmv_acc_rccl_comm_destroy", "spmv_acc_set_tune_cache",
     "spmv_acc_prepare_beta", "spmv_acc_time_spmv_events", "spmv_acc_refresh_values", "spmv_acc_time_spmv_region", "spmv_acc_query_plan_last_kernel", "spmv_acc_time_spmv_kernels",
@@ -105,6 +105,7 @@
     lib.spmv_acc_query_plan_settled.argtypes = [vp, ci]
     lib.spmv_acc_query_plan_col16.argtypes = [vp, ci]
     lib.spmv_acc_query_plan_col_bits.argtypes = [vp, ci]
+    lib.spmv_acc_query_plan_col_packed.argtypes = [vp, ci]
     lib.spmv_acc_query_plan_last_kernel.argtypes = [vp, ci]
     lib.spmv_acc_shard_create.argtypes = [ctypes.POINTER(vp), vp, ci, ci, ci, ci, ci, vp, vp, vp, ci]
     lib.spmv_acc_shard_step.argtypes = [vp, cd, cd, vp, vp, vp]
@@ -452,6 +453,7 @@
     info["settled"] = int(load_library().spmv_acc_query_plan_settled(_ptr(rowptr), m)) == 1
     info["col16"] = int(load_library().spmv_acc_query_plan_col16(_ptr(rowptr), m))
     info["col_bits"] = int(load_library().spmv_acc_query_plan_col_bits(_ptr(rowptr), m))
+    info["col_packed"] = int(load_library().spmv_acc_query_plan_col_packed(_ptr(rowptr), m))
     info["last_kernel"] = KERNEL_NAMES.get(int(load_library().spmv_acc_query_plan_last_kernel(_ptr(rowptr), m)), "none")
     return info
 
diff --git a/spmv_acc_amd/csrc/c_api.cpp b/spmv_acc_amd/csrc/c_api.cpp
--- a/spmv_acc_amd/csrc/c_api.cpp
+++ b/spmv_acc_amd/csrc/c_api.cpp
@@ -382,6 +382,10 @@
 int spmv_acc_query_plan_col_bits(const int *d_rowptr, int m) {
   PlanInfo info;
   return query_plan(d_rowptr, m, &info) ? info.col_bits : -2;
+}
+int spmv_acc_query_plan_col_packed(const int *d_rowptr, int m) {
+  PlanInfo info;
+  return query_plan(d_rowptr, m, &info) ? info.col_packed : -2;
 }
 int spmv_acc_query_plan_settled(const int *d_rowptr, int m) {
   PlanInfo info;
diff --git a/spmv_acc_amd/csrc/dispatch.cpp b/spmv_acc_amd/csrc/dispatch.cpp
--- a/spmv_acc_amd/csrc/dispatch.cpp
+++ b/spmv_acc_amd/csrc/dispatch.cpp
@@ -31,7 +31,7 @@
   p.flat.col16 = c16;
   const int rb_mode = tun(kT_flat_rowblock);
   const bool tile_pinned = tun(kT_flat_finish) >= 0 || tun(kT_flat_npt) >= 0 || tun(kT_flat_early) >= 0;
-  if (rb_mode != 0 && (rb_mode > 0 || !tile_pinned) && !flat_segment_sum() && tun(kT_col16) <= 0 &&
+  if (rb_mode != 0 && (rb_mode > 0 || !tile_pinned) && !flat_segment_sum() && col16_mode() <= 0 &&
       !t_coarse_tuning && !strict) {
     if (rb_mode > 0) {
       int vec = 1, rpb = kThreads;
@@ -64,6 +64,7 @@
   p.last_kernel = kKernelFlatTile;
   p.last_c16 = c16 && p.flat.stride == kThreads * kNnzPerThread && p.A.cold == nullptr ? c16->rec_ints : 0;
   p.last_col_bits = p.last_c16 > 0 ? c16->bits : 0;
+  p.last_col_packed = p.last_c16 > 0 && c16->packed ? 1 : 0;
   return true;
 }
 
@@ -266,15 +267,19 @@
     return false;
   const Col16 *c16 = nullptr;
   if (!autotune_col16(p, kFamRowblock, st, [&](const Col16 *c, double *ys) {
+        if (c) (void)ensure_col16_blocks(p, rpb, st);
         const int zz = next_reverse(p) ? 64 : 0;
         launch_rowblock_stream(st, p.A, vec, rpb, base_flags | (policy_for(p, kFamRowblock) << 4) | zz, 1.0, trial_beta(), x, ys, dg, cache_ends, c);
       }, &c16))
     return false;
+  if (c16 && !ensure_col16_blocks(p, rpb, st)) return false;
+  if (c16 && c16->packed && !(c16->blk && c16->blk_rpb == rpb)) c16 = nullptr;
   const int zz = next_reverse(p) ? 64 : 0;
   launch_rowblock_stream(st, p.A, vec, rpb, base_flags | (policy_for(p, kFamRowblock) << 4) | zz, alpha, beta, x, y, dg, cache_ends, c16);
   p.last_kernel = kKernelRowblock;
   p.last_c16 = c16 && p.A.cold == nullptr ? c16->rec_ints : 0;
   p.last_col_bits = p.last_c16 > 0 ? c16->bits : 0;
+  p.last_col_packed = p.last_c16 > 0 && c16->packed ? 1 : 0;
   return true;
 }
 
@@ -673,7 +678,7 @@
   }
   const auto began = std::chrono::steady_clock::now();
   const int err_before = last_error_code_only();
-  int served_kernel = -1, served_c16 = 0, served_col_bits = 0;
+  int served_kernel = -1, served_c16 = 0, served_col_bits = 0, served_col_packed = 0;
   {
     ScopedSet twin(t_rule_twin, true);
     run_spmv_call(strategy, trans, alpha, beta, m, n, nnz, h_rowptr, d_rowptr, d_colindex, d_value, dx, dy, dy_in);
@@ -681,6 +686,7 @@
       served_kernel = tp->last_kernel;
       served_c16 = tp->last_c16;
       served_col_bits = tp->last_col_bits;
+      served_col_packed = tp->last_col_packed;
     }
   }
   if (last_error_code_only() != err_before && last_error_code_only() != kOk && last_error_code_only() != kErrUnsupportedTrans) return;
@@ -704,6 +710,7 @@
       p->last_kernel = served_kernel;
       p->last_c16 = served_c16;
       p->last_col_bits = served_col_bits;
+      p->last_col_packed = served_col_packed;
     }
   }
   if (plan_settled_for(d_rowptr, d_colindex, d_value, m, n, strategy, beta != 0.0 ? 1 : 0)) drop_rule_twin(d_rowptr, d_colindex, d_value, m, n);
@@ -799,6 +806,7 @@
   p->A.yin = beta != 0.0 ? dy_in : nullptr;
   p->last_c16 = 0;
   p->last_col_bits = 0;
+  p->last_col_packed = 0;
 
   if (p->A.count() == 0) {
     launch_scale_y(st, m, beta, dy, p->A.yin);
diff --git a/spmv_acc_amd/csrc/engine.hpp b/spmv_acc_amd/csrc/engine.hpp
--- a/spmv_acc_amd/csrc/engine.hpp
+++ b/spmv_acc_amd/csrc/engine.hpp
@@ -109,6 +109,7 @@
   int slab_passes = 0;
   int last_kernel = -1;
   int col16 = -1;
+  int col_packed = -1;
   int col_bits = -1;
   int settled = 0;
 };
diff --git a/spmv_acc_amd/csrc/engine_internal.hpp b/spmv_acc_amd/csrc/engine_internal.hpp
--- a/spmv_acc_amd/csrc/engine_internal.hpp
+++ b/spmv_acc_amd/csrc/engine_internal.hpp
@@ -92,6 +92,7 @@
   unsigned launches = 0;
   double trial_ms = 0.0;
   int last_c16 = -1;
+  int last_col_packed = -1;
   int last_col_bits = -1;
   int last_kernel = -1;
   bool tuning_open = true;
@@ -177,6 +178,8 @@
     if (col16.rec) (void)hipFree(col16.rec);
     if (col16.ovf) (void)hipFree(col16.ovf);
     if (col16.ci_guard) (void)hipFree(col16.ci_guard);
+    if (col16.win) (void)hipFree(col16.win);
+    if (col16.blk) (void)hipFree(col16.blk);
     col16 = Col16();
   }
   void free_digest() {
@@ -270,7 +273,9 @@
 void drain_deferred_locked();
 
 extern thread_local bool t_flat_segment_sum;
-inline bool flat_segment_sum() { return (t_flat_segment_sum || tun(kT_flat_reduce) == 1) && tun(kT_col16) <= 0; }
+inline int col16_mode() { return tun(kT_col16) >= 100 ? tun(kT_col16) % 100 : tun(kT_col16); }
+inline int col16_pack_mode() { return tun(kT_col16) >= 200 ? 0 : (tun(kT_col16) >= 100 ? 1 : -1); }
+inline bool flat_segment_sum() { return (t_flat_segment_sum || tun(kT_flat_reduce) == 1) && col16_mode() <= 0; }
 extern thread_local int t_beta_class;
 inline double trial_beta() { return t_beta_class ? 1.0 : 0.0; }
 extern thread_local bool t_coarse_tuning;
@@ -292,6 +297,7 @@
 int analyze_on_device(hipStream_t st, const int *d_rowptr, int m, int min_nnz, int threads, int vec, int **d_bp, int **d_fbr);
 bool ensure_plus(Plan &p, const int *h_rowptr, hipStream_t stream, int min_nnz);
 bool ensure_col16(Plan &p, hipStream_t st);
+bool ensure_col16_blocks(Plan &p, int rpb, hipStream_t st);
 bool ensure_hint(Plan &p, hipStream_t st);
 bool ensure_slabs(Plan &p, int S, hipStream_t st);
 bool ensure_segments(Plan &p, int S_cols, hipStream_t st);
@@ -486,7 +492,7 @@
 
 template <class Launch> bool autotune_col16(Plan &p, int fam, hipStream_t st, Launch launch, const Col16 **out) {
   *out = nullptr;
-  const int mode = tun(kT_col16);
+  const int mode = col16_mode();
   if (mode == 0 || p.A.cold != nullptr || p.col16.state == 0) return true;
   if (mode < 0 && (tun(kT_deterministic) || p.c16_use[fam] == 0)) return true;
   const bool undecided = p.col16.state < 0 || (mode < 0 && p.c16_use[fam] < 0);
diff --git a/spmv_acc_amd/csrc/k_col16.hip b/spmv_acc_amd/csrc/k_col16.hip
--- a/spmv_acc_amd/csrc/k_col16.hip
+++ b/spmv_acc_amd/csrc/k_col16.hip
@@ -95,11 +95,39 @@
   }
 }
 
+__global__ __launch_bounds__(kThreads) void col16_granules_kernel(const int *__restrict__ esc_count, int nchunks, int fixed, int *__restrict__ granules) {
+  const long long c = static_cast<long long>(blockIdx.x) * kThreads + threadIdx.x;
+  if (c < nchunks) {
+    const int e = esc_count[c] < 60 ? esc_count[c] : 60;
+    granules[c] = fixed > 0 ? fixed : (4 + e + 15) / 16;
+  }
+}
+
+__global__ __launch_bounds__(kThreads) void col16_windows_kernel(const int *__restrict__ start, int nchunks, int *__restrict__ win) {
+  const long long c = static_cast<long long>(blockIdx.x) * kThreads + threadIdx.x;
+  if (c >= nchunks) return;
+  unsigned cls = 0;
+  for (int q = 0; q < 8 && c + q < nchunks; ++q) cls |= static_cast<unsigned>(start[c + q + 1] - start[c + q] - 1) << (2 * q);
+  win[2 * c] = start[c];
+  win[2 * c + 1] = static_cast<int>(cls);
+}
+
+__global__ __launch_bounds__(kThreads) void col16_blocks_kernel(const int *__restrict__ rp, int m, int rpb, int nblocks, const int *__restrict__ win,
+                                                                int *__restrict__ blk) {
+  const long long b = static_cast<long long>(blockIdx.x) * kThreads + threadIdx.x;
+  if (b >= nblocks) return;
+  const long long r = b * rpb;
+  const long long c = rp[r < m ? r : m] >> 8;
+  blk[2 * b] = win[2 * c];
+  blk[2 * b + 1] = win[2 * c + 1];
+}
+
 template <int BITS>
 __global__ __launch_bounds__(kThreads) void col16_encode_kernel(const int *__restrict__ ci, int nnz, int chunk0, int nchunks,
                                                                 const int *__restrict__ base, const int *__restrict__ ovf_start,
                                                                 int R, typename CodeWidth<BITS>::T *__restrict__ codes,
-                                                                int *__restrict__ rec, int *__restrict__ ovf) {
+                                                                int *__restrict__ rec, int *__restrict__ ovf,
+                                                                const int *__restrict__ rec_start) {
   typedef typename CodeWidth<BITS>::T Code;
   constexpr int ESC = 2 * CodeWidth<BITS>::half + 1;
   const int lane = threadIdx.x & (kWave - 1);
@@ -127,7 +155,7 @@
   }
   const int total = __shfl(incl, kWave - 1, kWave);
   int pos = incl - mine;
-  int *r = rec + static_cast<size_t>(c) * R;
+  int *r = rec + static_cast<size_t>(rec_start[c]) * 16;
   const int o0 = ovf_start[c];
   Code out[4];
 #pragma unroll
@@ -177,22 +205,37 @@
   SPMV_ACC_LAUNCH(col16_overflow_kernel, dim3((nchunks + kThreads - 1) / kThreads), dim3(kThreads), 0, stream, cnt, nchunks, E);
 }
 
+void launch_col16_granules(hipStream_t stream, const int *esc_count, int nchunks, int fixed_granules, int *granules) {
+  if (nchunks <= 0) return;
+  SPMV_ACC_LAUNCH(col16_granules_kernel, dim3((nchunks + kThreads - 1) / kThreads), dim3(kThreads), 0, stream, esc_count, nchunks, fixed_granules, granules);
+}
+
+void launch_col16_windows(hipStream_t stream, const int *start, int nchunks, int *win) {
+  if (nchunks <= 0) return;
+  SPMV_ACC_LAUNCH(col16_windows_kernel, dim3((nchunks + kThreads - 1) / kThreads), dim3(kThreads), 0, stream, start, nchunks, win);
+}
+
+void launch_col16_blocks(hipStream_t stream, const int *rp, int m, int rpb, int nblocks, const int *win, int *blk) {
+  if (nblocks <= 0) return;
+  SPMV_ACC_LAUNCH(col16_blocks_kernel, dim3((nblocks + kThreads - 1) / kThreads), dim3(kThreads), 0, stream, rp, m, rpb, nblocks, win, blk);
+}
+
 bool launch_col16_scan(hipStream_t stream, int nchunks, const int *esc_count, int *esc_start, void *tmp, size_t tmp_bytes) {
   return rocprim::exclusive_scan(tmp, tmp_bytes, esc_count, esc_start, 0, static_cast<size_t>(nchunks) + 1, rocprim::plus<int>(),
                                  stream) == hipSuccess;
 }
 
 void launch_col16_encode(hipStream_t stream, const int *ci, int nnz, int chunk0, int nchunks, const int *base, const int *ovf_start,
-                         int R, int bits, void *codes, int *rec, int *ovf) {
+                         int R, int bits, void *codes, int *rec, int *ovf, const int *rec_start) {
   if (nchunks <= 0) return;
   const int waves_per_block = kThreads / kWave;
   const dim3 grid((nchunks + waves_per_block - 1) / waves_per_block);
   if (bits == 8)
     SPMV_ACC_LAUNCH(col16_encode_kernel<8>, grid, dim3(kThreads), 0, stream, ci, nnz, chunk0, nchunks, base, ovf_start, R,
-                       static_cast<unsigned char *>(codes), rec, ovf);
+                       static_cast<unsigned char *>(codes), rec, ovf, rec_start);
   else
     SPMV_ACC_LAUNCH(col16_encode_kernel<16>, grid, dim3(kThreads), 0, stream, ci, nnz, chunk0, nchunks, base, ovf_start, R,
-                       static_cast<unsigned short *>(codes), rec, ovf);
+                       static_cast<unsigned short *>(codes), rec, ovf, rec_start);
 }
 
 void launch_col16_guard(hipStream_t stream, const int *ci, int lo, int span, int *out) {
diff --git a/spmv_acc_amd/csrc/k_flat.hip b/spmv_acc_amd/csrc/k_flat.hip
--- a/spmv_acc_amd/csrc/k_flat.hip
+++ b/spmv_acc_amd/csrc/k_flat.hip
@@ -43,9 +43,11 @@
                                                              int xcd_chunk, int reach, int tile0,
                                                              const int *__restrict__ guard, int *__restrict__ stale,
                                                              Col16Dev c16, int reverse, int cache_ends,
-                                                             const int4v *__restrict__ dig, const unsigned char *__restrict__ cold) {
+                                                             const int4v *__restrict__ dig, const unsigned char *__restrict__ cold,
+                                                             const int *__restrict__ c16_win) {
   check_plan_guard(rp, m, guard, stale);
   constexpr int STRIDE = kThreads * NPT;
+  static_assert(!C16 || STRIDE <= 8 * kCol16Chunk, "a packed-record window descriptor names 8 chunks");
   static_assert(STRIDE / 64 <= kTileSpans, "TileSpans must hold every >= 64-product span of one tile");
   __shared__ __attribute__((aligned(16))) double lds[STRIDE];
   __shared__ double sh_tail_sum, sh_tail_yold;
@@ -65,6 +67,7 @@
   if (EARLY && early) stage_issue<kThreads, EARLY ? NPT : 4, NTC, NTV>(early_regs, t0, t1, ci, v);
 
   const int4v rec = dig[t];
+  const C16Window cw = (C16 && c16_win != nullptr) ? c16_window_load(c16_win, (static_cast<long long>(t) + tile0) * (STRIDE / kCol16Chunk)) : c16_window_fixed(t0, c16.rec_ints);
   const int first = rec.x;
   const int end_excl = rec.y;
   const int nrows = end_excl - first;
@@ -102,7 +105,7 @@
 
   if (C16) check_ci_guard(ci, c16, stale);
   if (C16 && stage_fast_ok(t1, nnz))
-    stage_products_c16<kThreads, NPT, NTC, NTV>(lds, t0, t0, t1, c16, v, x);
+    stage_products_c16<kThreads, NPT, NTC, NTV>(lds, t0, t0, t1, c16, cw, v, x);
   else if (EARLY && early) stage_finish<kThreads, EARLY ? NPT : 4>(lds, early_regs, x);
   else if (NTC && NTV && cache_ends > 0 && (t < cache_ends || t >= ntiles - cache_ends))
     stage_products<kThreads, NPT, false, false, HINT>(lds, t0, t1, nnz, ci, v, x, xcd_chunk >= 0, cold, (reverse & 2) != 0);
@@ -304,11 +307,11 @@
   if (P.early_stream)
     SPMV_ACC_LAUNCH((flat_tile_kernel<NPT, NTC, NTV, true>), dim3(P.ntiles), dim3(kThreads), 0, stream, A.m, A.nnz,
                        P.ntiles, alpha, beta, A.rp, P.bp, A.ci, A.v, x, y, A.yin ? A.yin : y, P.head, P.tail, P.tail_row, P.tail_end,
-                       P.xcd_chunk, P.needs_fixup ? 0 : kFlatFinish, P.tile0, A.guard, A.stale, none, (P.reverse ? 1 : 0) | (x32_ok(A) ? 2 : 0), P.cache_ends, static_cast<const int4v *>(P.digest), nullptr);
+                       P.xcd_chunk, P.needs_fixup ? 0 : kFlatFinish, P.tile0, A.guard, A.stale, none, (P.reverse ? 1 : 0) | (x32_ok(A) ? 2 : 0), P.cache_ends, static_cast<const int4v *>(P.digest), nullptr, none.win);
   else
     SPMV_ACC_LAUNCH((flat_tile_kernel<NPT, NTC, NTV, false>), dim3(P.ntiles), dim3(kThreads), 0, stream, A.m, A.nnz,
                        P.ntiles, alpha, beta, A.rp, P.bp, A.ci, A.v, x, y, A.yin ? A.yin : y, P.head, P.tail, P.tail_row, P.tail_end,
-                       P.xcd_chunk, P.needs_fixup ? 0 : kFlatFinish, P.tile0, A.guard, A.stale, none, (P.reverse ? 1 : 0) | (x32_ok(A) ? 2 : 0), P.cache_ends, static_cast<const int4v *>(P.digest), nullptr);
+                       P.xcd_chunk, P.needs_fixup ? 0 : kFlatFinish, P.tile0, A.guard, A.stale, none, (P.reverse ? 1 : 0) | (x32_ok(A) ? 2 : 0), P.cache_ends, static_cast<const int4v *>(P.digest), nullptr, none.win);
 }
 template <bool NTC, bool NTV>
 void launch_flat_segsum(hipStream_t stream, const CsrDev &A, const FlatPlan &P, double alpha, double beta, const double *x,
@@ -317,7 +320,7 @@
   SPMV_ACC_LAUNCH((flat_tile_kernel<kNnzPerThread, NTC, NTV, false, false, true>), dim3(P.ntiles), dim3(kThreads), 0, stream, A.m,
                      A.nnz, P.ntiles, alpha, beta, A.rp, P.bp, A.ci, A.v, x, y, A.yin ? A.yin : y, P.head, P.tail, P.tail_row, P.tail_end,
                      P.xcd_chunk, P.needs_fixup ? 0 : kFlatFinish, P.tile0, A.guard, A.stale, none, (P.reverse ? 1 : 0) | (x32_ok(A) ? 2 : 0), P.cache_ends,
-                     static_cast<const int4v *>(P.digest), nullptr);
+                     static_cast<const int4v *>(P.digest), nullptr, none.win);
 }
 template <bool NTC, bool NTV>
 void launch_flat_hint(hipStream_t stream, const CsrDev &A, const FlatPlan &P, double alpha, double beta, const double *x, double *y) {
@@ -325,7 +328,7 @@
   SPMV_ACC_LAUNCH((flat_tile_kernel<kNnzPerThread, NTC, NTV, false, false, false, true>), dim3(P.ntiles), dim3(kThreads), 0, stream, A.m,
                      A.nnz, P.ntiles, alpha, beta, A.rp, P.bp, A.ci, A.v, x, y, A.yin ? A.yin : y, P.head, P.tail, P.tail_row, P.tail_end,
                      P.xcd_chunk, P.needs_fixup ? 0 : kFlatFinish, P.tile0, A.guard, A.stale, none, (P.reverse ? 1 : 0) | (x32_ok(A) ? 2 : 0), P.cache_ends,
-                     static_cast<const int4v *>(P.digest), A.cold);
+                     static_cast<const int4v *>(P.digest), A.cold, none.win);
 }
 template <bool NTC, bool NTV>
 void launch_flat_col16(hipStream_t stream, const CsrDev &A, const FlatPlan &P, double alpha, double beta, const double *x,
@@ -333,7 +336,7 @@
   const Col16Dev c = col16_dev(*P.col16, A);
   SPMV_ACC_LAUNCH((flat_tile_kernel<kNnzPerThread, NTC, NTV, false, true>), dim3(P.ntiles), dim3(kThreads), 0, stream, A.m,
                      A.nnz, P.ntiles, alpha, beta, A.rp, P.bp, A.ci, A.v, x, y, A.yin ? A.yin : y, P.head, P.tail, P.tail_row, P.tail_end,
-                     P.xcd_chunk, P.needs_fixup ? 0 : kFlatFinish, P.tile0, A.guard, A.stale, c, (P.reverse ? 1 : 0) | 2, P.cache_ends, static_cast<const int4v *>(P.digest), nullptr);
+                     P.xcd_chunk, P.needs_fixup ? 0 : kFlatFinish, P.tile0, A.guard, A.stale, c, (P.reverse ? 1 : 0) | 2, P.cache_ends, static_cast<const int4v *>(P.digest), nullptr, c.win);
 }
 template <int NPT>
 void launch_flat_policy(hipStream_t stream, const CsrDev &A, const FlatPlan &P, double alpha, double beta, const double *x,
diff --git a/spmv_acc_amd/csrc/k_rowblock.hip b/spmv_acc_amd/csrc/k_rowblock.hip
--- a/spmv_acc_amd/csrc/k_rowblock.hip
+++ b/spmv_acc_amd/csrc/k_rowblock.hip
@@ -32,7 +32,8 @@
                                                                    int *__restrict__ stale,
                                                                    const unsigned char *__restrict__ lens,
                                                                    const int *__restrict__ base, int cache_ends,
-                                                                   const unsigned char *__restrict__ cold, Col16Dev c16) {
+                                                                   const unsigned char *__restrict__ cold, Col16Dev c16,
+                                                                   const int *__restrict__ c16_blk, const int *__restrict__ c16_win) {
   check_plan_guard(rp, m, guard, stale);
   if (C16) check_ci_guard(ci, c16, stale);
   __shared__ int wave_tot[kThreads / kWave];
@@ -49,6 +50,8 @@
   const int row_end = (base_ll + rpb < m) ? row_base + rpb : m;
   int s0, s1;
   bool from_lens = false;
+  C16Window cw = {0, 0u};
+  if (C16 && c16_blk != nullptr) cw = c16_window_load(c16_blk, b);
   if (LENS) {
     const int b0 = base[b];
     s0 = b0 & 0x7fffffff;
@@ -81,8 +84,10 @@
   for (int off = off0; off < s1; off += kTile) {
     const bool cached_end = NTC && NTV && cache_ends > 0 && (b < cache_ends || b >= nblocks - cache_ends);
     if (C16 && c16_ok) {
-      if (cached_end) stage_products_c16<kThreads, kNnzPerThread, false, false>(lds, off, lo4 > off ? lo4 : off, s1, c16, v, x);
-      else stage_products_c16<kThreads, kNnzPerThread, NTC, NTV>(lds, off, lo4 > off ? lo4 : off, s1, c16, v, x);
+      if (c16_win == nullptr) cw = c16_window_fixed(off, c16.rec_ints);
+      else if (off != off0) cw = c16_window_load(c16_win, off >> 8);
+      if (cached_end) stage_products_c16<kThreads, kNnzPerThread, false, false>(lds, off, lo4 > off ? lo4 : off, s1, c16, cw, v, x);
+      else stage_products_c16<kThreads, kNnzPerThread, NTC, NTV>(lds, off, lo4 > off ? lo4 : off, s1, c16, cw, v, x);
     } else if (cached_end)
       stage_products<kThreads, kNnzPerThread, false, false, HINT>(lds, off, s1, nnz, ci, v, x, true, cold, (flags & 128) != 0);
     else
@@ -157,15 +162,16 @@
   SPMV_ACC_LAUNCH((rowblock_stream_kernel<VEC, NC, NV, LN, H, C>), dim3(nblocks), dim3(kThreads), 0, stream, A.m, A.nnz, nblocks, rpb, flags,
                      alpha, beta, A.rp, A.ci, A.v, x, y, A.yin ? A.yin : y, A.guard, A.stale,
                      LN ? D->lens : static_cast<const unsigned char *>(nullptr), LN ? D->base : static_cast<const int *>(nullptr), cache_ends,
-                     H ? A.cold : static_cast<const unsigned char *>(nullptr), c16);
+                     H ? A.cold : static_cast<const unsigned char *>(nullptr), c16, c16.blk, c16.win);
 }
 
 template <int VEC, bool NC, bool NV>
 void launch_policy(hipStream_t stream, const CsrDev &A, const RowDigest *D, const Col16 *C, int nblocks, int rpb, int flags, double alpha,
                    double beta, const double *x, double *y, int cache_ends) {
   const bool lens = VEC <= 2 && D && D->lens;
-  const bool c16 = C && C->state == 1 && A.cold == nullptr && x32_ok(A);
-  const Col16Dev cd = c16 ? col16_dev(*C, A) : Col16Dev{};
+  const bool c16 = C && C->state == 1 && A.cold == nullptr && x32_ok(A) && (!C->packed || (C->blk != nullptr && C->blk_rpb == rpb));
+  Col16Dev cd = c16 ? col16_dev(*C, A) : Col16Dev{};
+  if (c16 && C->packed) cd.blk = C->blk;
 #define SPMV_ACC_RB(LN, H, CC) launch_rb_instance<VEC, NC, NV, LN, H, CC>(stream, A, D, cd, nblocks, rpb, flags, alpha, beta, x, y, cache_ends)
   if constexpr (VEC <= 2) {
     if (lens) {
diff --git a/spmv_acc_amd/csrc/kernels.hpp b/spmv_acc_amd/csrc/kernels.hpp
--- a/spmv_acc_amd/csrc/kernels.hpp
+++ b/spmv_acc_amd/csrc/kernels.hpp
@@ -113,6 +113,10 @@
   unsigned char *d8 = nullptr;
   int *rec = nullptr;
   int *ovf = nullptr;
+  bool packed = false;
+  int *win = nullptr;
+  int *blk = nullptr;
+  int blk_rpb = 0;
   int *ci_guard = nullptr;
   long long escapes = 0;
   long long overflow = 0;
@@ -124,6 +128,8 @@
   const int *rec;
   const int *ovf;
   const int *ci_guard;
+  const int *win;
+  const int *blk;
   int rec_ints;
   int guard_lo, guard_span;
 };
@@ -131,10 +137,12 @@
   Col16Dev d;
   d.d16 = C.d16 ? C.d16 - static_cast<long long>(C.chunk0) * kCol16Chunk : nullptr;
   d.d8 = C.d8 ? C.d8 - static_cast<long long>(C.chunk0) * kCol16Chunk : nullptr;
-  d.rec = C.rec - static_cast<long long>(C.chunk0) * C.rec_ints;
+  d.rec = C.packed ? C.rec : C.rec - static_cast<long long>(C.chunk0) * C.rec_ints;
+  d.win = C.packed ? C.win - 2 * static_cast<long long>(C.chunk0) : nullptr;
+  d.blk = nullptr;
   d.ovf = C.ovf;
   d.ci_guard = C.ci_guard;
-  d.rec_ints = C.rec_ints;
+  d.rec_ints = C.packed ? 64 : C.rec_ints;
   d.guard_lo = A.nnz0;
   d.guard_span = A.count() > 0 ? A.count() - 1 : 0;
   return d;
@@ -149,9 +157,12 @@
 size_t col16_scan_bytes(int nchunks);
 void launch_col16_base(hipStream_t stream, const int *ci, int nnz, int chunk0, int nchunks, int *base, int *esc_count, unsigned long long *stats);
 void launch_col16_overflow(hipStream_t stream, int *cnt, int nchunks, int E);
+void launch_col16_granules(hipStream_t stream, const int *esc_count, int nchunks, int fixed_granules, int *granules);
+void launch_col16_windows(hipStream_t stream, const int *start, int nchunks, int *win);
+void launch_col16_blocks(hipStream_t stream, const int *rp, int m, int rpb, int nblocks, const int *win, int *blk);
 bool launch_col16_scan(hipStream_t stream, int nchunks, const int *esc_count, int *esc_start, void *tmp, size_t tmp_bytes);
 void launch_col16_encode(hipStream_t stream, const int *ci, int nnz, int chunk0, int nchunks, const int *base, const int *ovf_start, int R,
-                         int bits, void *codes, int *rec, int *ovf);
+                         int bits, void *codes, int *rec, int *ovf, const int *rec_start);
 void launch_col16_guard(hipStream_t stream, const int *ci, int lo, int span, int *out);
 
 struct FlatPlan {
diff --git a/spmv_acc_amd/csrc/plan.cpp b/spmv_acc_amd/csrc/plan.cpp
--- a/spmv_acc_amd/csrc/plan.cpp
+++ b/spmv_acc_amd/csrc/plan.cpp
@@ -504,6 +504,7 @@
       out->last_kernel = p.last_kernel;
       out->col16 = p.last_c16;
       out->col_bits = p.last_col_bits;
+      out->col_packed = p.last_col_packed;
       out->slab_passes = p.seg_state == 1 && (tun(kT_slab_segments) >= 1 || (tun(kT_slab_segments) < 0 && p.seg_choice == 1)) ? p.seg_slabs - (p.seg_rest_below > 0 ? 1 : 0) : 0;
       return true;
     }
diff --git a/spmv_acc_amd/csrc/tile_stage.hpp b/spmv_acc_amd/csrc/tile_stage.hpp
--- a/spmv_acc_amd/csrc/tile_stage.hpp
+++ b/spmv_acc_amd/csrc/tile_stage.hpp
@@ -213,8 +213,28 @@
   }
 };
 
+struct C16Window {
+  int off;
+  unsigned cls;
+};
+__device__ __forceinline__ int c16_granules_below(unsigned cls, int q) {
+  const unsigned m = cls & ((1u << (2 * q)) - 1u);
+  return q + __popc(m & 0x5555u) + 2 * __popc(m & 0xAAAAu);
+}
+__device__ __forceinline__ C16Window c16_window_load(const int *__restrict__ desc, long long i) {
+  const int2 d = *reinterpret_cast<const int2 *>(desc + 2 * i);
+  return C16Window{d.x, static_cast<unsigned>(d.y)};
+}
+__device__ __forceinline__ void c16_record(const C16Window &W, int q, int *first, int *ints) {
+  *first = 16 * (W.off + c16_granules_below(W.cls, q));
+  *ints = 16 * (static_cast<int>((W.cls >> (2 * q)) & 3u) + 1);
+}
+__device__ __forceinline__ C16Window c16_window_fixed(int a0, int R) {
+  return C16Window{(a0 >> 8) * (R >> 4), static_cast<unsigned>((R >> 4) - 1) * 0x5555u};
+}
+
 template <int BITS>
-__device__ __forceinline__ void c16_decode(int (&c)[4], const Codes4<BITS> &d, int rv, int R, int lane, const int *__restrict__ ovf) {
+__device__ __forceinline__ void c16_decode(int (&c)[4], const Codes4<BITS> &d, int rv, int E, int lane, const int *__restrict__ ovf) {
   constexpr int ESC = Codes4<BITS>::escape;
   const int bs = __builtin_amdgcn_readlane(rv, 0);
   const int nesc = __builtin_amdgcn_readlane(rv, 1);
@@ -223,7 +243,6 @@
 #pragma unroll
   for (int q = 0; q < 4; ++q) c[q] = bs + dq[q];
   if (nesc > 0) {
-    const int E = R - 4;
     const unsigned long long lt = (1ull << lane) - 1ull;
     const bool e[4] = {dq[0] == ESC, dq[1] == ESC, dq[2] == ESC, dq[3] == ESC};
     const unsigned long long slot[4] = {__ballot(e[0]), __ballot(e[1]), __ballot(e[2]), __ballot(e[3])};
@@ -241,19 +260,22 @@
 
 template <int THREADS, int NPT, bool NTC, bool NTV, int BITS>
 __device__ __forceinline__ void stage_products_c16_all(double *__restrict__ lds, int a0, int lo4, int hi, const Col16Dev &C,
-                                                       const double *__restrict__ v, const double *__restrict__ x) {
+                                                       const C16Window &W, const double *__restrict__ v, const double *__restrict__ x) {
   constexpr int K = NPT / 4;
   Codes4<BITS> d[K];
   double2v va[K], vb[K];
   int rv[K];
   const int lane = threadIdx.x & (kWave - 1);
   const int R = C.rec_ints;
-  const int rl = lane < R ? lane : 0;
+  const int E = R - 4;
 #pragma unroll
   for (int k = 0; k < K; ++k) {
     const int wave_j = __builtin_amdgcn_readfirstlane(a0 + 4 * ((threadIdx.x & ~(kWave - 1)) + k * THREADS));
-    rv[k] = C.rec[static_cast<long long>(wave_j >> 8) * R + rl];
-  }
+    int first, ints;
+    c16_record(W, (wave_j - a0) >> 8, &first, &ints);
+    rv[k] = C.rec[first + (lane < ints ? lane : 0)];
+  }
+  __builtin_amdgcn_sched_barrier(0x387);
 #pragma unroll
   for (int k = 0; k < K; ++k) d[k].template load<NTC>(C, a0 + 4 * (threadIdx.x + k * THREADS));
 #pragma unroll
@@ -268,7 +290,7 @@
   for (int k = 0; k < K; ++k) {
     const int j = a0 + 4 * (threadIdx.x + k * THREADS);
     int c[4];
-    c16_decode(c, d[k], rv[k], R, lane, C.ovf);
+    c16_decode(c, d[k], rv[k], E, lane, C.ovf);
     const bool mine = j >= lo4 && j < hi;
     const int bs = __builtin_amdgcn_readlane(rv[k], 0);
 #pragma unroll
@@ -290,23 +312,25 @@
 
 template <int THREADS, int NPT, bool NTC, bool NTV, int BITS>
 __device__ __forceinline__ void stage_products_c16_tail(double *__restrict__ lds, int a0, int lo4, int hi, const Col16Dev &C,
-                                                        const double *__restrict__ v, const double *__restrict__ x) {
+                                                        const C16Window &W, const double *__restrict__ v, const double *__restrict__ x) {
   const int lane = threadIdx.x & (kWave - 1);
   const int R = C.rec_ints;
-  const int rl = lane < R ? lane : 0;
+  const int E = R - 4;
 #pragma nounroll
   for (int k = 0; k < NPT / 4 - 1; ++k) {
     const int wave_j = __builtin_amdgcn_readfirstlane(a0 + 4 * ((threadIdx.x & ~(kWave - 1)) + k * THREADS));
     if (wave_j >= hi) break;
     const int g = threadIdx.x + k * THREADS;
     const int j = a0 + 4 * g;
-    const int rv = C.rec[static_cast<long long>(wave_j >> 8) * R + rl];
+    int first, ints;
+    c16_record(W, (wave_j - a0) >> 8, &first, &ints);
+    const int rv = C.rec[first + (lane < ints ? lane : 0)];
     Codes4<BITS> d;
     d.template load<NTC>(C, j);
     const int jv = (j >= lo4 && j < hi) ? j : lo4;
     const double2v va = load_stream_d2<NTV>(v + jv), vb = load_stream_d2<NTV>(v + jv + 2);
     int c[4];
-    c16_decode(c, d, rv, R, lane, C.ovf);
+    c16_decode(c, d, rv, E, lane, C.ovf);
     const bool mine = j >= lo4 && j < hi;
     const int bs = __builtin_amdgcn_readlane(rv, 0);
     double xg[4];
@@ -324,15 +348,15 @@
 }
 
 template <int THREADS, int NPT, bool NTC, bool NTV>
-__device__ __forceinline__ void stage_products_c16(double *__restrict__ lds, int a0, int lo4, int hi, const Col16Dev &C,
+__device__ __forceinline__ void stage_products_c16(double *__restrict__ lds, int a0, int lo4, int hi, const Col16Dev &C, const C16Window &W,
                                                    const double *__restrict__ v, const double *__restrict__ x) {
   const int last_j = __builtin_amdgcn_readfirstlane(a0 + 4 * ((threadIdx.x & ~(kWave - 1)) + (NPT / 4 - 1) * THREADS));
   if (C.d8 != nullptr) {
-    if (last_j < hi) stage_products_c16_all<THREADS, NPT, NTC, NTV, 8>(lds, a0, lo4, hi, C, v, x);
-    else stage_products_c16_tail<THREADS, NPT, NTC, NTV, 8>(lds, a0, lo4, hi, C, v, x);
+    if (last_j < hi) stage_products_c16_all<THREADS, NPT, NTC, NTV, 8>(lds, a0, lo4, hi, C, W, v, x);
+    else stage_products_c16_tail<THREADS, NPT, NTC, NTV, 8>(lds, a0, lo4, hi, C, W, v, x);
   } else {
-    if (last_j < hi) stage_products_c16_all<THREADS, NPT, NTC, NTV, 16>(lds, a0, lo4, hi, C, v, x);
-    else stage_products_c16_tail<THREADS, NPT, NTC, NTV, 16>(lds, a0, lo4, hi, C, v, x);
+    if (last_j < hi) stage_products_c16_all<THREADS, NPT, NTC, NTV, 16>(lds, a0, lo4, hi, C, W, v, x);
+    else stage_products_c16_tail<THREADS, NPT, NTC, NTV, 16>(lds, a0, lo4, hi, C, W, v, x);
   }
 }
 
diff --git a/spmv_acc_amd/csrc/tuner.cpp b/spmv_acc_amd/csrc/tuner.cpp
--- a/spmv_acc_amd/csrc/tuner.cpp
+++ b/spmv_acc_amd/csrc/tuner.cpp
@@ -56,7 +56,7 @@
 
 int flat_stride_for(const Plan &p) {
   if (flat_segment_sum()) return kThreads * kNnzPerThread;
-  if (tun(kT_col16) > 0) return kThreads * kNnzPerThread;
+  if (col16_mode() > 0) return kThreads * kNnzPerThread;
   int npt = tun(kT_flat_npt);
   if (npt < 0) npt = p.flat_npt_choice > 0 ? p.flat_npt_choice : kNnzPerThread;
   return kThreads * ((npt == 4 || npt == 16) ? npt : kNnzPerThread);
@@ -276,7 +276,7 @@
     return true;
   }
   ++t_plan_work;
-  int *base = nullptr, *cnt = nullptr, *ovf_start = nullptr;
+  int *base = nullptr, *cnt = nullptr, *ovf_start = nullptr, *rec_start = nullptr;
   unsigned long long *stats = nullptr;
   void *tmp = nullptr;
   const size_t tmp_bytes = col16_scan_bytes(nchunks);
@@ -290,7 +290,8 @@
             hip_ok(hipMemsetAsync(cnt + n1 + nchunks, 0, sizeof(int), st), "memset col16") &&
             hip_ok(hipMemsetAsync(stats, 0, sizeof(unsigned long long) * 8, st), "memset col16 statistics");
   unsigned long long h_stats[8] = {0, 0, 0, 0, 0, 0, 0, 0};
-  int R = 0, total = 0, bits = 16;
+  int R = 0, total = 0, bits = 16, granules = 0;
+  bool packed = false;
   if (ok) {
     launch_col16_base(st, A.ci, A.nnz, chunk0, nchunks, base, cnt, stats);
     ok = hip_ok(hipMemcpyAsync(h_stats, stats, sizeof(h_stats), hipMemcpyDeviceToHost, st), "read col16 statistics") &&
@@ -301,24 +302,47 @@
     R = h_stats[1] <= limit ? 16 : (h_stats[2] <= limit ? 32 : (h_stats[3] <= limit ? 64 : 0));
     const int R8 = h_stats[5] <= limit ? 16 : (h_stats[6] <= limit ? 32 : (h_stats[7] <= limit ? 64 : 0));
     const long long extra8 = static_cast<long long>(h_stats[4]) - static_cast<long long>(h_stats[0]);
-    const int mode = tun(kT_col16);
+    const int mode = col16_mode();
     bits = mode == 8 || (mode != 2 && R > 0 && R8 > 0 && R8 <= R && 200 * extra8 <= static_cast<long long>(A.count())) ? 8 : 16;
     if (bits == 8) R = R8;
-    const int forced = tun(kT_col16) > 1 ? tun(kT_col16) : 0;
+    const int forced = col16_mode() > 1 ? col16_mode() : 0;
     if (forced == 16 || forced == 32 || forced == 64) R = forced;
     tune_log("m %d nnz %d 16-bit columns: %llu escapes in %d chunks, %llu / %llu / %llu chunks above 12 / 28 / 60 -> %s", A.m, A.nnz, h_stats[0], nchunks,
              h_stats[1], h_stats[2], h_stats[3], R ? (R == 16 ? "16-int records" : (R == 32 ? "32-int records" : "64-int records")) : "not encoded");
     tune_log("m %d nnz %d 8-bit columns: %llu escapes (%+lld), %llu / %llu / %llu chunks above 12 / 28 / 60 -> %d-bit codes", A.m, A.nnz, h_stats[4], extra8,
              h_stats[5], h_stats[6], h_stats[7], bits);
   }
+  const size_t cofs = bits == 8 ? n1 : 0;
+  const int pack_mode = col16_pack_mode();
   if (ok && R > 0) {
-    const size_t cofs = bits == 8 ? n1 : 0;
-    launch_col16_overflow(st, cnt + cofs, nchunks, R - 4);
+    ok = hip_ok(hipMalloc(reinterpret_cast<void **>(&rec_start), sizeof(int) * n1), "hipMalloc col16 record offsets") &&
+         hip_ok(hipMemsetAsync(ovf_start + nchunks, 0, sizeof(int), st), "memset col16");
+    auto place = [&](int fixed_granules) {
+      launch_col16_granules(st, cnt + cofs, nchunks, fixed_granules, ovf_start);
+      return launch_col16_scan(st, nchunks, ovf_start, rec_start, tmp, tmp_bytes) &&
+             hip_ok(hipMemcpyAsync(&granules, rec_start + nchunks, sizeof(int), hipMemcpyDeviceToHost, st), "read col16 record total") &&
+             hip_ok(hipStreamSynchronize(st), "sync col16 record sizes");
+    };
+    if (ok && (pack_mode > 0 || (pack_mode < 0 && R > 16))) {
+      ok = place(0);
+      const long long saved = 4LL * R * nchunks - 64LL * granules;
+      packed = ok && (pack_mode > 0 || saved >= 32LL * nchunks);
+      if (ok)
+        tune_log("m %d nnz %d chunk records: fixed %d ints = %.1f B per chunk, packed %.1f B per chunk -> %s", A.m, A.nnz, R, 4.0 * R, 64.0 * granules / nchunks,
+                 packed ? "packed" : "fixed");
+    } else if (ok) {
+      tune_log("m %d nnz %d chunk records: fixed %d ints -> fixed", A.m, A.nnz, R);
+    }
+    if (ok && !packed) ok = place(R / 16);
+  }
+  if (ok && R > 0) {
+    launch_col16_overflow(st, cnt + cofs, nchunks, packed ? 60 : R - 4);
     ok = launch_col16_scan(st, nchunks, cnt + cofs, ovf_start, tmp, tmp_bytes) &&
          hip_ok(hipMemcpyAsync(&total, ovf_start + nchunks, sizeof(int), hipMemcpyDeviceToHost, st), "read col16 overflow total") &&
          hip_ok(hipStreamSynchronize(st), "sync col16");
     const size_t code_bytes = static_cast<size_t>(bits / 8) * static_cast<size_t>(nchunks) * kCol16Chunk;
-    const size_t rec_bytes = sizeof(int) * static_cast<size_t>(nchunks) * R;
+    const size_t rec_bytes = 64 * (static_cast<size_t>(granules) + 4);
+    const size_t win_bytes = sizeof(int) * 2 * (static_cast<size_t>(nchunks) + 8);
     const size_t ovf_bytes = sizeof(int) * (static_cast<size_t>(total) + 64);
     void *codes = nullptr;
     ok = ok && hip_ok(hipMalloc(&codes, code_bytes), "hipMalloc col16 offsets") &&
@@ -326,16 +350,19 @@
          hip_ok(hipMalloc(reinterpret_cast<void **>(&C.ovf), ovf_bytes), "hipMalloc col16 overflow list") &&
          hip_ok(hipMalloc(reinterpret_cast<void **>(&C.ci_guard), sizeof(int) * kGuardSamples), "hipMalloc col16 guard") &&
          hip_ok(hipMemsetAsync(C.rec, 0, rec_bytes, st), "memset col16 records") && hip_ok(hipMemsetAsync(C.ovf, 0, ovf_bytes, st), "memset col16 overflow");
+    ok = ok && hip_ok(hipMalloc(reinterpret_cast<void **>(&C.win), win_bytes), "hipMalloc col16 record windows") &&
+         hip_ok(hipMemsetAsync(C.win, 0, win_bytes, st), "memset col16 record windows");
     if (bits == 8) C.d8 = static_cast<unsigned char *>(codes);
     else C.d16 = static_cast<unsigned short *>(codes);
     if (ok) {
-      launch_col16_encode(st, A.ci, A.nnz, chunk0, nchunks, base + cofs, ovf_start, R, bits, codes, C.rec, C.ovf);
+      launch_col16_windows(st, rec_start, nchunks, C.win);
+      launch_col16_encode(st, A.ci, A.nnz, chunk0, nchunks, base + cofs, ovf_start, packed ? 64 : R, bits, codes, C.rec, C.ovf, rec_start);
       launch_col16_guard(st, A.ci, A.nnz0, A.count() > 0 ? A.count() - 1 : 0, C.ci_guard);
       ok = hip_ok(hipStreamSynchronize(st), "sync col16 encode");
     }
-    C.bytes = code_bytes + rec_bytes + ovf_bytes;
-  }
-  for (void *q : {static_cast<void *>(base), static_cast<void *>(cnt), static_cast<void *>(ovf_start), static_cast<void *>(stats), tmp})
+    C.bytes = code_bytes + rec_bytes + ovf_bytes + win_bytes;
+  }
+  for (void *q : {static_cast<void *>(base), static_cast<void *>(cnt), static_cast<void *>(ovf_start), static_cast<void *>(rec_start), static_cast<void *>(stats), tmp})
     if (q) (void)hipFree(q);
   if (!ok) {
     p.free_col16();
@@ -351,8 +378,28 @@
   C.nchunks = nchunks;
   C.rec_ints = R;
   C.bits = bits;
+  C.packed = packed;
   C.escapes = static_cast<long long>(h_stats[bits == 8 ? 4 : 0]);
   C.overflow = total;
+  return true;
+}
+
+bool ensure_col16_blocks(Plan &p, int rpb, hipStream_t st) {
+  Col16 &C = p.col16;
+  if (C.state != 1 || !C.packed || (C.blk && C.blk_rpb == rpb) || t_capturing || stream_capturing(st)) return true;
+  ++t_plan_work;
+  if (C.blk) (void)hipFree(C.blk);
+  C.blk = nullptr;
+  C.blk_rpb = 0;
+  const size_t nblocks = (static_cast<size_t>(p.A.m) + rpb - 1) / rpb;
+  if (!hip_ok(hipMalloc(reinterpret_cast<void **>(&C.blk), sizeof(int) * 2 * (nblocks + 1)), "hipMalloc col16 block descriptors")) return false;
+  launch_col16_blocks(st, p.A.rp, p.A.m, rpb, static_cast<int>(nblocks), C.win - 2 * static_cast<long long>(C.chunk0), C.blk);
+  if (!hip_ok(hipStreamSynchronize(st), "build the col16 block descriptors")) {
+    (void)hipFree(C.blk);
+    C.blk = nullptr;
+    return false;
+  }
+  C.blk_rpb = rpb;
   return true;
 }
 
@@ -419,7 +466,7 @@
 }
 
 bool autotune_flat_geometry(Plan &p, hipStream_t st, const double *x) {
-  if (p.flat_geometry_tuned || tun(kT_col16) > 0 || flat_segment_sum() || t_capturing || by_rule()) return true;
+  if (p.flat_geometry_tuned || col16_mode() > 0 || flat_segment_sum() || t_capturing || by_rule()) return true;
   if (p.A.count() >= flat_small_nnz() || p.flat.ntiles <= 1) {
     p.flat_geometry_tuned = true;
     return true;
```

After: 578.1, median of 6. +1.4%, better.
